# mttga/purejaxql

Measured on NVIDIA H100. Metric: MinAtar-Breakout env steps/sec @4096 envs x128 seeds, higher is better.
Workload: dtype f32

## Files before the change

### include/pqn_b200.h

```cpp
#ifndef PQN_B200_H
#define PQN_B200_H

#include <stdint.h>

#ifdef __cplusplus
extern "C" {
#endif

#define PQN_OK 0
#define PQN_E_INVALID (-1)
#define PQN_E_CUDA (-2)
#define PQN_E_UNSUPPORTED (-3)

#define PQN_ENV_BREAKOUT 0
#define PQN_ENV_ASTERIX 1
#define PQN_ENV_SPACE_INVADERS 2
#define PQN_ENV_FREEWAY 3
#define PQN_ENV_SEAQUEST 4
#define PQN_ENV_CARTPOLE 16
#define PQN_ENV_ACROBOT 17
#define PQN_ENV_MOUNTAIN_CAR 18
#define PQN_ENV_MEMORY_CHAIN 32
#define PQN_ENV_CATCH 33
#define PQN_ENV_DEEP_SEA 34
// ... 58 lines not shown
int pqn_rollout_act_step(int env_id, const uint32_t* step_keys, const float* q, const float* eps,
                         uint32_t* state, void* obs_next, int64_t obs_seed_stride, int32_t* action,
                         float* reward, uint8_t* done, float* maxq, int64_t tr_seed_stride, double* info_sums,
                         int info_done_only, int32_t S, int32_t E, int32_t env_total, int32_t env_offset, int max_steps,
                         float rew_scale, int rng_mode, void* stream);
int pqn_rollout_keys(uint32_t* rng_inout, uint32_t* keys_out, int32_t S, int32_t T, int rng_mode, void* stream);

int pqn_qlambda(const float* reward, const uint8_t* done, const float* maxq, const float* q_last,
                float* targets, int32_t T, int32_t S, int32_t E, int32_t A, float gamma, float lambda,
                void* stream);

#define PQN_NET_MINATAR_CNN 0
#define PQN_NET_MLP 1
#define PQN_NET_RNN 2
#define PQN_NET_MLP_BITS 3

typedef struct pqn_net_desc_t {
  int32_t kind;
  int32_t in_c;
  int32_t hidden;
  int32_t layers;
  int32_t num_actions;
  int32_t norm_type;
  int32_t norm_input;
} pqn_net_desc_t;
#define PQN_MAX_LAYERS 8
#define PQN_NORM_LAYER 0
#define PQN_NORM_BATCH 1
#define PQN_NORM_NONE 2

typedef struct pqn_net_layout_t {
  int64_t total;
  int64_t bn_scale, bn_bias;
  int64_t conv_w, conv_b;
  int64_t ln0_scale, ln0_bias;
  int64_t d0_w, d0_b;
  int64_t ln1_scale, ln1_bias;
  int64_t d1_w, d1_b;
  int64_t head_w, head_b;
  int64_t gru_ir_w, gru_ir_b, gru_iz_w, gru_iz_b, gru_in_w, gru_in_b, gru_hr_w, gru_hz_w, gru_hn_w, gru_hn_b;
} pqn_net_layout_t;

int pqn_net_layout(const pqn_net_desc_t* desc_host, pqn_net_layout_t* out_host);
int pqn_net_dense_layer(const pqn_net_desc_t* desc_host, int32_t layer, int64_t* offsets_host);
int64_t pqn_net_stats_floats(const pqn_net_desc_t* desc_host);
int64_t pqn_net_workspace_bytes(const pqn_net_desc_t* desc_host, int32_t S, int64_t rows);

int pqn_net_init(const pqn_net_desc_t* desc_host, const uint32_t* keys, float* params, int32_t S, void* stream);

int pqn_qnet_forward(const pqn_net_desc_t* desc_host, const float* params, const float* batch_stats, const void* obs,
                     const int32_t* gather, int64_t obs_rows_per_seed, float* q, int32_t S, int64_t rows,
                     void* workspace, void* stream);

int pqn_qnet_loss_grad(const pqn_net_desc_t* desc_host, const float* params, float* batch_stats, const void* obs,
                       const int32_t* gather, int64_t obs_rows_per_seed, const int32_t* action,
                       const float* target, int64_t tr_rows_per_seed, float* grads, float* loss_sum,
                       float* qsa_sum, float* bn_sums, int32_t S, int64_t rows, void* workspace, void* stream);

int pqn_rnn_step(const pqn_net_desc_t* desc_host, const float* params, float* hs, const float* obs,
                 int64_t obs_rows_per_seed, const uint8_t* last_done, const int32_t* last_action, float* q, int32_t S,
                 int32_t E, void* workspace, void* stream);
int pqn_rnn_loss_grad(const pqn_net_desc_t* desc_host, const float* params, const float* hs0, const float* obs,
                      const uint8_t* last_done, const int32_t* last_action, const int32_t* action, const float* reward,
                      const uint8_t* done, float* grads, float* loss_sum, float* qsa_sum, int32_t S, int32_t T, int32_t B,
                      float gamma, float lambda, void* workspace, void* stream);
int pqn_rnn_step_stats(const pqn_net_desc_t* desc_host, const float* params, const float* batch_stats, float* hs,
                       const float* obs, int64_t obs_rows_per_seed, const uint8_t* last_done, const int32_t* last_action,
                       float* q, int32_t S, int32_t E, void* workspace, void* stream);
int pqn_rnn_loss_grad_stats(const pqn_net_desc_t* desc_host, const float* params, float* batch_stats, const float* hs0,
                            const float* obs, const uint8_t* last_done, const int32_t* last_action,
                            const int32_t* action, const float* reward, const uint8_t* done, float* grads,
                            float* loss_sum, float* qsa_sum, int32_t S, int32_t T, int32_t B, float gamma, float lambda,
                            void* workspace, void* stream);

int pqn_radam_clip_step(float* params, const float* grads, float* mu, float* nu, const float* sched,
                        int32_t* step_counter, float* gnorm_scratch , int32_t S, int64_t P,
                        float max_norm, float b1, float b2, float eps, void* stream);

int pqn_bn_stats_update(float* batch_stats, float* bn_sums, int32_t S, int32_t F, int64_t stats_seed_stride,
                        float count, float momentum, void* stream);

int pqn_set_tensor_core_path(int on);
int pqn_set_conv_mma_path(int on);

int pqn_tc_split_lo(const float* x, float* lo, int64_t n, void* stream);
int pqn_tc_gemm_test(const float* a, const float* a_lo, const float* b, const float* b_lo, float* d, int32_t S,
                     int32_t M, int32_t N, int32_t K, int a_mn, int b_mn, int split3, void* stream);

int pqn_tc_split16(const float* x, void* hi, void* lo, int64_t n, float scale, void* stream);
int pqn_tc_gemm16_test(const void* a_hi, const void* a_lo, const void* b_hi, const void* b_lo, float* d, int32_t S,
                       int32_t M, int32_t N, int32_t K, int a_mn, int b_mn, float out_scale, void* stream);
int pqn_tc_dgrad16_test(const void* a_hi, const void* a_lo, const void* b_hi, const void* b_lo, const float* mask,
                        const uint32_t* relu_bits, float* d, int32_t S, int32_t M, int32_t N, int32_t K, int epi,
                        float out_scale, void* stream);

#ifdef __cplusplus
}
#endif
#endif
```

### purejaxql_b200/_lib.py

```python
from __future__ import annotations

import ctypes
import os
from ctypes import POINTER, Structure, c_char_p, c_double, c_float, c_int, c_int32, c_int64, c_longlong, c_void_p

HERE = os.path.dirname(os.path.abspath(__file__))
LIB_PATH = os.path.join(HERE, "libpqn_b200.so")


class EnvInfo(Structure):
    _fields_ = [("state_words", c_int32), ("obs_dim", c_int32), ("obs_shape", c_int32 * 3),
                ("num_actions", c_int32), ("max_steps", c_int32), ("binary_obs", c_int32),
                ("packed_obs_words", c_int32)]


class EnvParams(Structure):
    _fields_ = [("max_steps", c_int32), ("memory_length", c_int32)]


class NetDesc(Structure):
    _fields_ = [("kind", c_int32), ("in_c", c_int32), ("hidden", c_int32), ("layers", c_int32),
                ("num_actions", c_int32), ("norm_type", c_int32), ("norm_input", c_int32)]


NORM_TYPES = {"layer_norm": 0, "batch_norm": 1}


class NetLayout(Structure):
    _fields_ = [(n, c_int64) for n in (
        "total", "bn_scale", "bn_bias", "conv_w", "conv_b", "ln0_scale", "ln0_bias", "d0_w", "d0_b",
        "ln1_scale", "ln1_bias", "d1_w", "d1_b", "head_w", "head_b",
        "gru_ir_w", "gru_ir_b", "gru_iz_w", "gru_iz_b", "gru_in_w", "gru_in_b", "gru_hr_w", "gru_hz_w", "gru_hn_w",
        "gru_hn_b")]


class PqnError(RuntimeError):
    pass


_SIGS = {
    "pqn_last_error": (c_char_p, []),
    "pqn_version": (c_int, []),
    "pqn_launch_count": (c_longlong, []),
    "pqn_num_kernels": (c_int, []),
    "pqn_kernel_name": (c_char_p, [c_int]),
    "pqn_profile_enable": (c_int, [c_int]),
    "pqn_profile_read": (c_int, [POINTER(c_double), POINTER(c_longlong), c_int]),
    "pqn_env_info": (c_int, [c_int, POINTER(EnvInfo)]),
    "pqn_rng_split": (c_int, [c_void_p, c_int64, c_int32, c_void_p, c_int, c_void_p]),
    "pqn_threefry2x32": (c_int, [c_void_p, c_void_p, c_void_p, c_int64, c_void_p]),
    "pqn_rng_bits": (c_int, [c_void_p, c_int64, c_int64, c_void_p, c_int, c_void_p]),
    "pqn_random_normal": (c_int, [c_void_p, c_void_p, c_int64, c_int, c_void_p]),
    "pqn_normal_from_bits": (c_int, [c_void_p, c_void_p, c_int64, c_void_p]),
    "pqn_set_permutation_bucket_log2": (c_int, [c_int]),
    "pqn_permutation_workspace_bytes": (c_int64, [c_int64, c_int]),
    "pqn_permutation": (c_int, [c_void_p, c_int64, c_int, c_int, c_void_p, c_int64, c_void_p, c_void_p]),
    "pqn_env_reset": (c_int, [c_int, c_void_p, c_void_p, c_void_p, c_int64, c_int, c_int, c_void_p]),
    "pqn_env_reset_params": (c_int, [c_int, c_void_p, c_void_p, c_void_p, c_int64, POINTER(EnvParams), c_int, c_void_p]),
    "pqn_env_step": (c_int, [c_int, c_void_p, c_void_p, c_void_p, c_void_p, c_void_p, c_void_p, c_void_p,
                             c_void_p, c_void_p, c_void_p, c_int64, c_int, c_int, c_void_p]),
    "pqn_env_obs_packed": (c_int, [c_int, c_void_p, c_void_p, c_int64, c_void_p]),
    "pqn_env_obs": (c_int, [c_int, c_void_p, c_void_p, c_int64, c_void_p]),
    "pqn_eps_greedy": (c_int, [c_void_p, c_void_p, c_void_p, c_void_p, c_int64, c_int32, c_int, c_void_p]),
    "pqn_rollout_act_step": (c_int, [c_int, c_void_p, c_void_p, c_void_p, c_void_p, c_void_p, c_int64, c_void_p,
                                     c_void_p, c_void_p, c_void_p, c_int64, c_void_p, c_int, c_int32, c_int32,
                                     c_int32, c_int32, c_int, c_float, c_int, c_void_p]),
    "pqn_rollout_keys": (c_int, [c_void_p, c_void_p, c_int32, c_int32, c_int, c_void_p]),
    "pqn_qlambda": (c_int, [c_void_p, c_void_p, c_void_p, c_void_p, c_void_p, c_int32, c_int32, c_int32, c_int32,
                            c_float, c_float, c_void_p]),
    "pqn_net_layout": (c_int, [POINTER(NetDesc), POINTER(NetLayout)]),
    "pqn_net_dense_layer": (c_int, [POINTER(NetDesc), c_int32, POINTER(c_int64)]),
    "pqn_net_stats_floats": (c_int64, [POINTER(NetDesc)]),
    "pqn_net_workspace_bytes": (c_int64, [POINTER(NetDesc), c_int32, c_int64]),
    "pqn_net_init": (c_int, [POINTER(NetDesc), c_void_p, c_void_p, c_int32, c_void_p]),
    "pqn_qnet_forward": (c_int, [POINTER(NetDesc), c_void_p, c_void_p, c_void_p, c_void_p, c_int64, c_void_p, c_int32,
                                 c_int64, c_void_p, c_void_p]),
    "pqn_qnet_loss_grad": (c_int, [POINTER(NetDesc), c_void_p, c_void_p, c_void_p, c_void_p, c_int64, c_void_p,
                                   c_void_p, c_int64, c_void_p, c_void_p, c_void_p, c_void_p, c_int32, c_int64,
                                   c_void_p, c_void_p]),
    "pqn_rnn_step": (c_int, [POINTER(NetDesc), c_void_p, c_void_p, c_void_p, c_int64, c_void_p, c_void_p, c_void_p,
                             c_int32, c_int32, c_void_p, c_void_p]),
    "pqn_rnn_loss_grad": (c_int, [POINTER(NetDesc), c_void_p, c_void_p, c_void_p, c_void_p, c_void_p, c_void_p, c_void_p,
                                  c_void_p, c_void_p, c_void_p, c_void_p, c_int32, c_int32, c_int32, c_float, c_float,
                                  c_void_p, c_void_p]),
    "pqn_rnn_step_stats": (c_int, [POINTER(NetDesc), c_void_p, c_void_p, c_void_p, c_void_p, c_int64, c_void_p, c_void_p,
                                   c_void_p, c_int32, c_int32, c_void_p, c_void_p]),
    "pqn_rnn_loss_grad_stats": (c_int, [POINTER(NetDesc), c_void_p, c_void_p, c_void_p, c_void_p, c_void_p, c_void_p,
                                        c_void_p, c_void_p, c_void_p, c_void_p, c_void_p, c_void_p, c_int32, c_int32,
                                        c_int32, c_float, c_float, c_void_p, c_void_p]),
    "pqn_radam_clip_step": (c_int, [c_void_p, c_void_p, c_void_p, c_void_p, c_void_p, c_void_p, c_void_p, c_int32,
                                    c_int64, c_float, c_float, c_float, c_float, c_void_p]),
    "pqn_bn_stats_update": (c_int, [c_void_p, c_void_p, c_int32, c_int32, c_int64, c_float, c_float, c_void_p]),
    "pqn_set_tensor_core_path": (c_int, [c_int]),
    "pqn_set_conv_mma_path": (c_int, [c_int]),
    "pqn_tc_split_lo": (c_int, [c_void_p, c_void_p, c_int64, c_void_p]),
    "pqn_tc_split16": (c_int, [c_void_p, c_void_p, c_void_p, c_int64, c_float, c_void_p]),
    "pqn_tc_gemm_test": (c_int, [c_void_p, c_void_p, c_void_p, c_void_p, c_void_p, c_int32, c_int32, c_int32,
                                 c_int32, c_int, c_int, c_int, c_void_p]),
    "pqn_tc_gemm16_test": (c_int, [c_void_p, c_void_p, c_void_p, c_void_p, c_void_p, c_int32, c_int32, c_int32,
                                   c_int32, c_int, c_int, c_float, c_void_p]),
    "pqn_tc_dgrad16_test": (c_int, [c_void_p, c_void_p, c_void_p, c_void_p, c_void_p, c_void_p, c_void_p, c_int32,
                                    c_int32, c_int32, c_int32, c_int, c_float, c_void_p]),
}

EXPORTS = tuple(_SIGS)
_lib = None


def lib():
    global _lib
    if _lib is None:
        if not os.path.exists(LIB_PATH):
            raise PqnError(
                f"{LIB_PATH} is not built. Run `python -m purejaxql_b200.build` (needs nvcc). "
                "purejaxql_b200 has no CPU fallback.")
        l = ctypes.CDLL(LIB_PATH)
        for name, (res, args) in _SIGS.items():
            fn = getattr(l, name)
            fn.restype = res
            fn.argtypes = args
        _lib = l
    return _lib


def check(rc: int, what: str = ""):
    if rc != 0:
        msg = lib().pqn_last_error().decode("utf-8", "replace")
        raise PqnError(f"{what or 'libpqn_b200'} failed (rc={rc}): {msg}")


def p(t):
    if t is None:
        return None
    if not t.is_cuda:
        raise PqnError("libpqn_b200 takes CUDA tensors only (no CPU fallback); got a CPU tensor")
    if not t.is_contiguous():
        raise PqnError("libpqn_b200 takes contiguous tensors")
    return c_void_p(t.data_ptr())


def raw(t):
    if t is None:
        return None
    if not t.is_cuda:
        raise PqnError("libpqn_b200 takes CUDA tensors only (no CPU fallback); got a CPU tensor")
    return c_void_p(t.data_ptr())


def stream_ptr():
    import torch
    return c_void_p(torch.cuda.current_stream().cuda_stream)


def profile_read(reset=True):
    l = lib()
    n = l.pqn_num_kernels()
    ms = (c_double * n)()
    cnt = (c_longlong * n)()
    check(l.pqn_profile_read(ms, cnt, 1 if reset else 0), "pqn_profile_read")
    return {l.pqn_kernel_name(i).decode(): (ms[i], int(cnt[i])) for i in range(n) if cnt[i]}
```

### purejaxql_b200/csrc/pqn_net.cu

```cuda
#include <cuda_runtime.h>
#include <stdint.h>

#include "../../include/pqn_b200.h"
#include "api_common.h"
#include "tc_common.cuh"

namespace pqn {

constexpr int GT = 256;
constexpr int BK = 16;
constexpr float LN_EPS = 1e-6f;
constexpr int CONV_O = 16;
constexpr int CONV_PIX = 64;
constexpr int HID_CNN = 128;
constexpr int FLAT_CNN = CONV_PIX * CONV_O;

static int g_use_tc = 2;
static int g_conv_mma = 1;

__host__ __device__ static inline int64_t align4(int64_t x) { return (x + 3) & ~(int64_t)3; }

static int make_layout(const pqn_net_desc_t* d, pqn_net_layout_t* L) {
  int64_t off = 0;
  auto take = [&](int64_t n) { int64_t o = off; off += align4(n); return o; };
  L->d1_w = L->d1_b = L->ln1_scale = L->ln1_bias = L->conv_w = L->conv_b = -1;
  L->gru_ir_w = L->gru_ir_b = L->gru_iz_w = L->gru_iz_b = L->gru_in_w = L->gru_in_b = -1;
  L->gru_hr_w = L->gru_hz_w = L->gru_hn_w = L->gru_hn_b = -1;
  const int A = d->num_actions;
  const bool has_norm = d->norm_type != PQN_NORM_NONE;
  if (d->kind == PQN_NET_MINATAR_CNN) {
    const int C = d->in_c;
    L->bn_scale = take(C); L->bn_bias = take(C);
    L->conv_w = take(9 * C * CONV_O); L->conv_b = take(CONV_O);
    L->ln0_scale = L->ln0_bias = -1;
    if (has_norm) { L->ln0_scale = take(CONV_O); L->ln0_bias = take(CONV_O); }
    L->d0_w = take((int64_t)FLAT_CNN * HID_CNN); L->d0_b = take(HID_CNN);
    if (has_norm) { L->ln1_scale = take(HID_CNN); L->ln1_bias = take(HID_CNN); }
    L->head_w = take((int64_t)HID_CNN * A); L->head_b = take(A);
  } else if (d->kind == PQN_NET_MLP || d->kind == PQN_NET_RNN || d->kind == PQN_NET_MLP_BITS) {
    const int D = d->in_c, H = d->hidden;
    L->bn_scale = take(D); L->bn_bias = take(D);
    L->d0_w = take((int64_t)D * H); L->d0_b = take(H);
    L->ln0_scale = L->ln0_bias = -1;
    if (has_norm) { L->ln0_scale = take(H); L->ln0_bias = take(H); }
    for (int l = 1; l < d->layers; ++l) {
      const int64_t w = take((int64_t)H * H), b = take(H);
      const int64_t sc = has_norm ? take(H) : -1, bi = has_norm ? take(H) : -1;
      if (l == 1) { L->d1_w = w; L->d1_b = b; L->ln1_scale = sc; L->ln1_bias = bi; }
    }
    if (d->kind == PQN_NET_RNN) {
      L->gru_ir_w = take((int64_t)(H + A) * H); L->gru_ir_b = take(H);
      L->gru_iz_w = take((int64_t)(H + A) * H); L->gru_iz_b = take(H);
      L->gru_in_w = take((int64_t)(H + A) * H); L->gru_in_b = take(H);
      L->gru_hr_w = take((int64_t)H * H); L->gru_hz_w = take((int64_t)H * H);
      L->gru_hn_w = take((int64_t)H * H); L->gru_hn_b = take(H);
    }
    L->head_w = take((int64_t)H * A); L->head_b = take(A);
  } else {
    return -1;
  }
  L->total = off;
  return 0;
}

struct DenseOff { int64_t w, b, g, bi; };
__host__ __device__ inline DenseOff dense_off(const pqn_net_layout_t& L, int H, int l) {
  if (l == 0) return DenseOff{L.d0_w, L.d0_b, L.ln0_scale, L.ln0_bias};
  if (l == 1) return DenseOff{L.d1_w, L.d1_b, L.ln1_scale, L.ln1_bias};
  const bool norm = L.ln1_scale >= 0;
  const int64_t stride = align4((int64_t)H * H) + (norm ? 3 : 1) * align4(H);
  const int64_t w = (norm ? L.ln1_bias : L.d1_b) + align4(H) + (l - 2) * stride;
  const int64_t b = w + align4((int64_t)H * H);
  return DenseOff{w, b, norm ? b + align4(H) : -1, norm ? b + 2 * align4(H) : -1};
}

static int check_desc(const pqn_net_desc_t* d, const char* who) {
  if (!d) return set_error(PQN_E_INVALID, "%s: desc is NULL", who);
  if (d->num_actions < 1 || d->num_actions > 32) return set_error(PQN_E_INVALID, "%s: num_actions=%d out of [1,32]", who, d->num_actions);
  if (d->norm_type < 0 || d->norm_type > 2 || d->norm_input < 0 || d->norm_input > 1)
    return set_error(PQN_E_INVALID, "%s: norm_type=%d norm_input=%d", who, d->norm_type, d->norm_input);
  if (d->kind == PQN_NET_MLP || d->kind == PQN_NET_RNN || d->kind == PQN_NET_MLP_BITS) {
    const int H = d->hidden;
    if (H != 64 && H != 128 && H != 256 && H != 512)
      return set_error(PQN_E_UNSUPPORTED, "%s: hidden=%d (64, 128, 256 or 512 built)", who, H);
    if (d->layers < 1 || d->layers > PQN_MAX_LAYERS)
      return set_error(PQN_E_UNSUPPORTED, "%s: layers=%d (1 to %d built)", who, d->layers, PQN_MAX_LAYERS);
  }
  {
    const int Nh = d->kind == PQN_NET_MINATAR_CNN ? 128 : d->hidden;
    const size_t need = (size_t)(24 * Nh + 9 * d->num_actions * Nh + 8 * d->num_actions + 16) * sizeof(float);
    if (need > 227u * 1024u)
      return set_error(PQN_E_UNSUPPORTED, "%s: hidden=%d with num_actions=%d needs %zu B of shared memory for the head "
                       "backward (limit 227 KB)", who, Nh, d->num_actions, need);
  }
  if (d->kind == PQN_NET_MINATAR_CNN) {
    if (d->in_c != 4 && d->in_c != 6 && d->in_c != 7 && d->in_c != 10)
      return set_error(PQN_E_UNSUPPORTED, "%s: CNN in_c=%d (MinAtar uses 4/6/7/10)", who, d->in_c);
    return PQN_OK;
  }
  if (d->kind == PQN_NET_MLP_BITS) {
    if (d->in_c != 400 && d->in_c != 600 && d->in_c != 700)
// ... 494 lines not shown
      if (DZLO != nullptr) {
        float lo[V];
#pragma unroll
        for (int k = 0; k < V; ++k) lo[k] = tc::tf32_lo(dz[V * c + k]);
        st_feat<V>(DZLO + e, lo);
      }
    }
  }
#pragma unroll
  for (int j = 0; j < F; ++j) {
    const int f = (j / V) * CW + lane * V + (j % V);
    s_red3[warp * 3 * N + f] = a_dsc[j];
    s_red3[warp * 3 * N + N + f] = a_dbi[j];
    s_red3[warp * 3 * N + 2 * N + f] = a_db[j];
  }
  if (HEAD && lane == 0) { s_ls[warp * 2] = a_loss; s_ls[warp * 2 + 1] = a_qsa; }
  __syncthreads();
  const int stride = 3 * N + (HEAD ? A * N + A + 2 : 0);
  float* __restrict__ o = part + ((int64_t)seed * gridDim.x + blockIdx.x) * stride;
  for (int i = tid; i < 3 * N; i += 256) {
    float v = 0.f;
#pragma unroll
    for (int wv = 0; wv < 8; ++wv) v += s_red3[wv * 3 * N + i];
    o[i] = v;
  }
  if (HEAD) {
    for (int i = tid; i < A * N; i += 256) {
      float v = 0.f;
#pragma unroll
      for (int wv = 0; wv < 8; ++wv) v += s_dhw[wv * A * N + i];
      o[3 * N + i] = v;
    }
    if (tid < A + 2) {
      float v = 0.f;
      for (int wv = 0; wv < 8; ++wv) v += tid < A ? s_dhb[wv * A + tid] : s_ls[wv * 2 + (tid - A)];
      o[3 * N + A * N + tid] = v;
    }
  }
}

template <int SL>
__device__ __forceinline__ float ordered_partial_sum(const float* __restrict__ p, int count, int64_t stride, bool valid) {
  constexpr int COLS = 256 / SL;
  __shared__ float slice_sum[SL][COLS];
  const int col = threadIdx.x % COLS, sl = threadIdx.x / COLS;
  float v = 0.f;
  if (valid) {
#pragma unroll 4
    for (int c = sl; c < count; c += SL) v += p[(int64_t)c * stride];
  }
  slice_sum[sl][col] = v;
  __syncthreads();
  float r = 0.f;
  if (sl == 0) {
#pragma unroll
    for (int k = 0; k < SL; ++k) r += slice_sum[k][col];
  }
  return r;
}
static inline int final_slices(int count) { return count > 48 ? 32 : 8; }

template <int SL>
__global__ void row_bwd_final_kernel(const float* __restrict__ part, int nctas, int N, int A, int head,
                                     float* __restrict__ grads, int64_t P, int64_t off_dscale, int64_t off_dbias,
                                     int64_t off_db, int64_t off_hw, int64_t off_hb, float* __restrict__ loss_sum,
                                     float* __restrict__ qsa_sum) {
  const int seed = blockIdx.y;
  const int stride = 3 * N + (head ? A * N + A + 2 : 0);
  const int i = blockIdx.x * (256 / SL) + threadIdx.x % (256 / SL);
  const float v = ordered_partial_sum<SL>(part + (int64_t)seed * nctas * stride + i, nctas, stride, i < stride);
  if (i >= stride || threadIdx.x >= 256 / SL) return;
  float* __restrict__ g = grads + (int64_t)seed * P;
  if (i < N) g[off_dscale + i] = v;
  else if (i < 2 * N) g[off_dbias + (i - N)] = v;
  else if (i < 3 * N) g[off_db + (i - 2 * N)] = v;
  else if (i < 3 * N + A * N) {
    const int j = i - 3 * N, a = j / N, f = j - a * N;
    g[off_hw + (int64_t)f * A + a] = v;
  } else if (i < 3 * N + A * N + A) g[off_hb + (i - 3 * N - A * N)] = v;
  else if (i == 3 * N + A * N + A) loss_sum[seed] += v;
  else qsa_sum[seed] += v;
}

template <int C>
struct ConvCfg {
  static constexpr int TAPS = 9 * C;
  static constexpr int OBS_BITS = 100 * C;
  static constexpr int OBS_WORDS = (OBS_BITS + 31) / 32;
  static constexpr int PW = (OBS_WORDS + 3) / 4 * 4;
  static constexpr int SW = PW + 1;
};

template <int C>
__device__ __forceinline__ uint32_t pixel_bits(const uint32_t* __restrict__ so, int p) {
  const int f0 = p * C;
  const uint32_t lo = so[f0 >> 5], hi = so[(f0 >> 5) + 1];
  return __funnelshift_r(lo, hi, f0 & 31) & ((1u << C) - 1u);
}

template <int C>
__device__ __forceinline__ void conv_pixel(const uint32_t* __restrict__ so, const float* __restrict__ ws,
                                           const float* __restrict__ cb, int y, int x, float (&acc)[CONV_O]) {
#pragma unroll
  for (int o = 0; o < CONV_O; ++o) acc[o] = cb[o];
#pragma unroll
  for (int di = 0; di < 3; ++di)
#pragma unroll
    for (int dj = 0; dj < 3; ++dj) {
      const uint32_t nib = pixel_bits<C>(so, (y + di) * 10 + (x + dj));
      if (__ballot_sync(0xffffffffu, nib != 0u) == 0u) continue;
#pragma unroll
      for (int c = 0; c < C; ++c) {
        const bool bit = (nib >> c) & 1u;
        if (__ballot_sync(0xffffffffu, bit) == 0u) continue;
        const float* __restrict__ w = ws + ((di * 3 + dj) * C + c) * CONV_O;
#pragma unroll
        for (int o4 = 0; o4 < CONV_O / 4; ++o4) {
          const float4 wv = *reinterpret_cast<const float4*>(w + 4 * o4);
          if (bit) {
            acc[4 * o4] += wv.x; acc[4 * o4 + 1] += wv.y; acc[4 * o4 + 2] += wv.z; acc[4 * o4 + 3] += wv.w;
          }
        }
      }
    }
}

__device__ __forceinline__ void ln16(const float (&z)[CONV_O], float& mean, float& rstd) {
  float s1 = 0.f, s2 = 0.f;
#pragma unroll
  for (int o = 0; o < CONV_O; ++o) { s1 += z[o]; s2 = fmaf(z[o], z[o], s2); }
  mean = s1 * (1.0f / CONV_O);
  const float var = fmaxf(s2 * (1.0f / CONV_O) - mean * mean, 0.f);
  rstd = 1.0f / sqrtf(var + LN_EPS);
}

template <int C>
__device__ __forceinline__ void conv_load_consts(const float* __restrict__ prm, const pqn_net_layout_t& L, float* ws,
                                                 float* cb, float* sc, float* bi) {
  const float inv255 = 1.0f / 255.0f;
  for (int i = threadIdx.x; i < ConvCfg<C>::TAPS * CONV_O; i += blockDim.x) ws[i] = __ldg(prm + L.conv_w + i) * inv255;
  if (threadIdx.x < CONV_O) {
    cb[threadIdx.x] = __ldg(prm + L.conv_b + threadIdx.x);
    sc[threadIdx.x] = __ldg(prm + L.ln0_scale + threadIdx.x);
    bi[threadIdx.x] = __ldg(prm + L.ln0_bias + threadIdx.x);
  }
}

template <int C, bool TRAIN>
__global__ void __launch_bounds__(256) conv_fwd_kernel(const uint32_t* __restrict__ obs, int64_t obs_rows_per_seed,
                                                       const int32_t* __restrict__ gather,
                                                       const float* __restrict__ params, int64_t P,
                                                       pqn_net_layout_t L, float* __restrict__ H1,
                                                       float* __restrict__ H1LO, float* __restrict__ bn_sums,
                                                       int rows) {
  using Cfg = ConvCfg<C>;
  __shared__ __align__(16) float ws[Cfg::TAPS * CONV_O];
  __shared__ float cb[CONV_O], sc[CONV_O], bi[CONV_O];
  __shared__ uint32_t so[4][Cfg::SW];
  __shared__ float s_cnt[C];
  const int tid = threadIdx.x, sl = tid >> 6, pix = tid & 63;
  const int seed = blockIdx.y;
  const int row = blockIdx.x * 4 + sl;
  const bool valid = row < rows;
  conv_load_consts<C>(params + (int64_t)seed * P, L, ws, cb, sc, bi);
  if (TRAIN && tid < C) s_cnt[tid] = 0.f;
  if (pix < Cfg::SW) {
    uint32_t w = 0u;
    if (valid && pix < Cfg::PW) {
      const int64_t src = gather ? gather[(int64_t)seed * rows + row] : row;
      w = __ldg(obs + ((int64_t)seed * obs_rows_per_seed + src) * Cfg::PW + pix);
    }
    so[sl][pix] = w;
  }
  __syncthreads();
// ... 120 lines not shown
      for (int o4 = 0; o4 < CONV_O / 4; ++o4) {
        float4 dz;
        dz.x = rstd * (dy[4 * o4] - m1 - acc[4 * o4] * m2);
        dz.y = rstd * (dy[4 * o4 + 1] - m1 - acc[4 * o4 + 1] * m2);
        dz.z = rstd * (dy[4 * o4 + 2] - m1 - acc[4 * o4 + 2] * m2);
        dz.w = rstd * (dy[4 * o4 + 3] - m1 - acc[4 * o4 + 3] * m2);
        *reinterpret_cast<float4*>(&my_dz[pix * SDZ_LD + 4 * o4]) = dz;
      }
    }
    __syncwarp();
#pragma unroll 8
    for (int p = tpar; p < CONV_PIX; p += 2) a_dcb += my_dz[p * SDZ_LD + o_b];
#pragma unroll
    for (int c = 0; c < C; ++c) {
      for (int wi = 0; wi < Cfg::OBS_WORDS; ++wi) {
        uint32_t bits = my_so[wi];
        if (C == 4) bits &= 0x11111111u << c;
        if (bits == 0u) continue;
        while (bits) {
          const int b = __ffs(bits) - 1;
          bits &= bits - 1u;
          const int f = wi * 32 + b;
          const int q = f / C;
          if (f - q * C != c) continue;
          const int qy = q / 10, qx = q - qy * 10;
#pragma unroll
          for (int it = 0; it < 5; ++it) {
            const int py = qy - t_di[it], px = qx - t_dj[it];
            if ((unsigned)py < 8u && (unsigned)px < 8u) wacc[c][it] += my_dz[(py * 8 + px) * SDZ_LD + o_b];
          }
        }
      }
    }
  }
  __syncthreads();
  for (int i = tid; i < TAPS * CONV_O; i += blockDim.x) s_w[i] = 0.f;
  __syncthreads();
  const float inv255 = 1.0f / 255.0f;
#pragma unroll
  for (int c = 0; c < C; ++c)
#pragma unroll
    for (int it = 0; it < 5; ++it) {
      const int tap = it * 2 + tpar;
      if (tap < 9) atomicAdd(&s_w[(tap * C + c) * CONV_O + o_b], wacc[c][it] * inv255);
    }
  atomicAdd(&s_red[2 * CONV_O + o_b], a_dcb);
#pragma unroll
  for (int o = 0; o < CONV_O; ++o) {
    float v0 = a_dsc[o], v1 = a_dbi[o];
#pragma unroll
    for (int sft = 16; sft > 0; sft >>= 1) {
      v0 += __shfl_xor_sync(0xffffffffu, v0, sft);
      v1 += __shfl_xor_sync(0xffffffffu, v1, sft);
    }
    if (lane == 0) {
      atomicAdd(&s_red[o], v0);
      atomicAdd(&s_red[CONV_O + o], v1);
    }
  }
  __syncthreads();
  float* __restrict__ g = grads + (int64_t)seed * P;
  for (int i = tid; i < TAPS * CONV_O; i += blockDim.x) atomicAdd(g + L.conv_w + i, s_w[i]);
  if (tid < CONV_O) {
    atomicAdd(g + L.ln0_scale + tid, s_red[tid]);
    atomicAdd(g + L.ln0_bias + tid, s_red[CONV_O + tid]);
    atomicAdd(g + L.conv_b + tid, s_red[2 * CONV_O + tid]);
  }
}

__device__ __forceinline__ void mma_tf32_16n8k8(float (&d)[4], const uint32_t (&a)[4], uint32_t b0, uint32_t b1) {
  asm volatile(
      "mma.sync.aligned.m16n8k8.row.col.f32.tf32.tf32.f32 {%0,%1,%2,%3}, {%4,%5,%6,%7}, {%8,%9}, {%0,%1,%2,%3};"
      : "+f"(d[0]), "+f"(d[1]), "+f"(d[2]), "+f"(d[3])
      : "r"(a[0]), "r"(a[1]), "r"(a[2]), "r"(a[3]), "r"(b0), "r"(b1));
}

template <int C>
struct ConvMma {
  static constexpr int TAPS = 9 * C;
  static constexpr int KS = (TAPS + 7) / 8;
  static constexpr int MT = (TAPS + 15) / 16;
};

template <int C>
struct PatchCfg {
  static constexpr int WORDS = (9 * C + 31) / 32;
};

template <int C>
__device__ __forceinline__ void patch_bits(const uint32_t* __restrict__ so, int pix, uint32_t (&w)[PatchCfg<C>::WORDS]) {
  constexpr int W = PatchCfg<C>::WORDS;
#pragma unroll
  for (int k = 0; k < W; ++k) w[k] = 0u;
  const int y = pix >> 3, x = pix & 7;
#pragma unroll
  for (int di = 0; di < 3; ++di) {
    const int f0 = ((y + di) * 10 + x) * C;
    const uint32_t r = __funnelshift_r(so[f0 >> 5], so[(f0 >> 5) + 1], f0 & 31) & ((1u << (3 * C)) - 1u);
    const int o = 3 * C * di;
    w[o >> 5] |= r << (o & 31);
    if ((o & 31) + 3 * C > 32) w[min((o >> 5) + 1, W - 1)] |= r >> (32 - (o & 31));
  }
}

template <int C>
__device__ __forceinline__ void build_patch(const uint32_t* __restrict__ so, int pix, uint32_t* __restrict__ out) {
  constexpr int W = PatchCfg<C>::WORDS;
  uint32_t w[W];
  patch_bits<C>(so, pix, w);
#pragma unroll
  for (int k = 0; k < W; ++k) out[k] = w[k];
}

template <int C>
__device__ __forceinline__ void build_patches(const uint32_t* __restrict__ so, uint32_t* __restrict__ patch, int lane) {
  build_patch<C>(so, lane, patch + lane * PatchCfg<C>::WORDS);
  build_patch<C>(so, lane + 32, patch + (lane + 32) * PatchCfg<C>::WORDS);
}

__device__ __forceinline__ uint32_t bit_f32(uint32_t word, int shift) {
  return ((word >> shift) & 1u) ? 0x3F800000u : 0u;
}

template <int C, bool EXPC = false>
__device__ __forceinline__ void conv_mma_load_weights(const float* __restrict__ prm, const pqn_net_layout_t& L,
                                                      float2* wb_hi, float2* wb_lo, float* cb, float* sc, float* bi) {
  using M = ConvMma<C>;
  const float inv255 = 1.0f / 255.0f;
  for (int i = threadIdx.x; i < M::KS * 2 * 32; i += blockDim.x) {
    const int ln = i & 31, h = (i >> 5) & 1, ks = i >> 6;
    const int o = h * 8 + (ln >> 2);
    const int t0 = ks * 8 + (ln & 3), t1 = t0 + 4;
    float w0 = t0 < M::TAPS ? __ldg(prm + L.conv_w + t0 * CONV_O + o) * inv255 : 0.f;
    float w1 = t1 < M::TAPS ? __ldg(prm + L.conv_w + t1 * CONV_O + o) * inv255 : 0.f;
    if (EXPC) {
      w0 *= __uint_as_float((254u - (1u << (t0 & 7))) << 23);
      w1 *= __uint_as_float((254u - (1u << (t1 & 7))) << 23);
    }
    const float h0 = __uint_as_float(__float_as_uint(w0) & 0xFFFFE000u), h1 = __uint_as_float(__float_as_uint(w1) & 0xFFFFE000u);
    wb_hi[i] = make_float2(h0, h1);
    wb_lo[i] = make_float2(w0 - h0, w1 - h1);
  }
  if (threadIdx.x < CONV_O) {
    cb[threadIdx.x] = __ldg(prm + L.conv_b + threadIdx.x);
    sc[threadIdx.x] = __ldg(prm + L.ln0_scale + threadIdx.x);
    bi[threadIdx.x] = __ldg(prm + L.ln0_bias + threadIdx.x);
  }
}

template <int C>
struct ExpPatch {
  static constexpr int KS = ConvMma<C>::KS;
  static constexpr int LD = KS | 1;
};

template <int C>
__device__ __forceinline__ void build_exp_patch(const uint32_t* __restrict__ so, int pix, uint32_t* __restrict__ out) {
  constexpr int W = PatchCfg<C>::WORDS;
  uint32_t w[W];
  patch_bits<C>(so, pix, w);
#pragma unroll
  for (int ks = 0; ks < ExpPatch<C>::KS; ++ks)
    out[ks] = ((w[(8 * ks) >> 5] >> ((8 * ks) & 31)) & 0xFFu) << 23;
}

template <int C>
__device__ __forceinline__ void conv_mma_block2_exp(const uint32_t* __restrict__ xp, const float2* __restrict__ wb_hi,
                                                    const float2* __restrict__ wb_lo, const float* __restrict__ cb,
                                                    int mbp, int lane, float (&z)[2][2][4]) {
  using E = ExpPatch<C>;
  const int g = lane >> 2, t = lane & 3;
  const uint32_t m_lo = 1u << (23 + t), m_hi = 1u << (27 + t);
#pragma unroll
  for (int i = 0; i < 2; ++i)
#pragma unroll
    for (int h = 0; h < 2; ++h) {
      z[i][h][0] = z[i][h][2] = cb[8 * h + 2 * t];
      z[i][h][1] = z[i][h][3] = cb[8 * h + 2 * t + 1];
    }
  const uint32_t* r00 = xp + (32 * mbp + g) * E::LD;
#pragma unroll
  for (int ks = 0; ks < E::KS; ++ks) {
    uint32_t a[2][4];
#pragma unroll
    for (int i = 0; i < 2; ++i) {
      const uint32_t w0 = r00[(16 * i) * E::LD + ks], w1 = r00[(16 * i + 8) * E::LD + ks];
      a[i][0] = w0 & m_lo; a[i][1] = w1 & m_lo; a[i][2] = w0 & m_hi; a[i][3] = w1 & m_hi;
    }
    float2 bl[2], bh[2];
#pragma unroll
    for (int h = 0; h < 2; ++h) {
      bl[h] = wb_lo[(ks * 2 + h) * 32 + lane];
      bh[h] = wb_hi[(ks * 2 + h) * 32 + lane];
    }
#pragma unroll
    for (int h = 0; h < 2; ++h)
#pragma unroll
      for (int i = 0; i < 2; ++i) mma_tf32_16n8k8(z[i][h], a[i], __float_as_uint(bl[h].x), __float_as_uint(bl[h].y));
#pragma unroll
    for (int h = 0; h < 2; ++h)
#pragma unroll
      for (int i = 0; i < 2; ++i) mma_tf32_16n8k8(z[i][h], a[i], __float_as_uint(bh[h].x), __float_as_uint(bh[h].y));
  }
}

__device__ __forceinline__ void ln16_quad(const float (&z)[2][4], float& mean0, float& rstd0, float& mean1,
                                          float& rstd1) {
  float s0 = z[0][0] + z[0][1] + z[1][0] + z[1][1];
  float q0 = fmaf(z[1][1], z[1][1], fmaf(z[1][0], z[1][0], fmaf(z[0][0], z[0][0], __fmul_rn(z[0][1], z[0][1]))));
  float s1 = z[0][2] + z[0][3] + z[1][2] + z[1][3];
  float q1 = fmaf(z[1][3], z[1][3], fmaf(z[1][2], z[1][2], fmaf(z[0][2], z[0][2], __fmul_rn(z[0][3], z[0][3]))));
#pragma unroll
  for (int o = 1; o <= 2; o <<= 1) {
    s0 += __shfl_xor_sync(0xffffffffu, s0, o); q0 += __shfl_xor_sync(0xffffffffu, q0, o);
    s1 += __shfl_xor_sync(0xffffffffu, s1, o); q1 += __shfl_xor_sync(0xffffffffu, q1, o);
  }
  mean0 = __fmul_rn(s0, 1.0f / CONV_O); mean1 = __fmul_rn(s1, 1.0f / CONV_O);
  rstd0 = rsqrtf(fmaxf(fmaf(q0, 1.0f / CONV_O, -__fmul_rn(mean0, mean0)), 0.f) + LN_EPS);
  rstd1 = rsqrtf(fmaxf(fmaf(q1, 1.0f / CONV_O, -__fmul_rn(mean1, mean1)), 0.f) + LN_EPS);
}

constexpr int CONV_MMA_WARPS = 8;

template <int C, bool TRAIN, bool H16 = false>
__global__ void __launch_bounds__(CONV_MMA_WARPS * 32, 3)
    conv_fwd_mma_kernel(const uint32_t* __restrict__ obs, int64_t obs_rows_per_seed, const int32_t* __restrict__ gather,
                        const float* __restrict__ params, int64_t P, pqn_net_layout_t L, float* __restrict__ H1,
                        float* __restrict__ H1LO, float* __restrict__ XH1, float* __restrict__ RS1,
                        uint32_t* __restrict__ RB, float* __restrict__ bn_sums, int rows) {
  using Cfg = ConvCfg<C>;
  using M = ConvMma<C>;
  __shared__ float2 wb_hi[M::KS * 2 * 32], wb_lo[M::KS * 2 * 32];
  __shared__ float cb[CONV_O], sc[CONV_O], bi[CONV_O];
  __shared__ uint32_t so[CONV_MMA_WARPS][Cfg::SW];
  __shared__ uint32_t sxp[CONV_MMA_WARPS][CONV_PIX * ExpPatch<C>::LD];
  __shared__ float s_cnt[C];
  const int tid = threadIdx.x, warp = tid >> 5, lane = tid & 31;
  const int g = lane >> 2, t = lane & 3;
  const int seed = blockIdx.y;
  conv_mma_load_weights<C, true>(params + (int64_t)seed * P, L, wb_hi, wb_lo, cb, sc, bi);
  if (TRAIN && tid < C) s_cnt[tid] = 0.f;
  __syncthreads();
  int cnt[C];
  uint32_t cmask[C];
#pragma unroll
  for (int c = 0; c < C; ++c) {
    cnt[c] = 0;
    cmask[c] = 0u;
    if (TRAIN) {
      for (int b = 0; b < 32; ++b) {
        const int f = lane * 32 + b;
        if (f < Cfg::OBS_BITS && f % C == c) cmask[c] |= 1u << b;
      }
    }
  }
  uint32_t* __restrict__ my_so = so[warp];
  static_assert(Cfg::PW <= 32, "one packed observation word per lane");
  if (lane == 0) my_so[Cfg::PW] = 0u;
  const int row_stride = gridDim.x * CONV_MMA_WARPS;
  auto fetch = [&](int r) -> uint32_t {
    if (r >= rows || lane >= Cfg::PW) return 0u;
    const int64_t src = gather ? gather[(int64_t)seed * rows + r] : r;
    return __ldg(obs + ((int64_t)seed * obs_rows_per_seed + src) * Cfg::PW + lane);
  };
  uint32_t pre = fetch(blockIdx.x * CONV_MMA_WARPS + warp);
  for (int row = blockIdx.x * CONV_MMA_WARPS + warp; row < rows; row += row_stride) {
    __syncwarp();
    if (lane < Cfg::PW) my_so[lane] = pre;
    if (TRAIN && bn_sums != nullptr) {
#pragma unroll
      for (int c = 0; c < C; ++c) cnt[c] += __popc(pre & cmask[c]);
    }
    __syncwarp();
    pre = fetch(row + row_stride);
    build_exp_patch<C>(my_so, lane, sxp[warp] + lane * ExpPatch<C>::LD);
    build_exp_patch<C>(my_so, lane + 32, sxp[warp] + (lane + 32) * ExpPatch<C>::LD);
    __syncwarp();
    float* __restrict__ hrow = H16 ? nullptr : H1 + ((int64_t)seed * rows + row) * FLAT_CNN;
    float* __restrict__ lrow = (!H16 && H1LO) ? H1LO + ((int64_t)seed * rows + row) * FLAT_CNN : nullptr;
    __half* __restrict__ hrow16 = H16 ? reinterpret_cast<__half*>(H1) + ((int64_t)seed * rows + row) * FLAT_CNN : nullptr;
    __half* __restrict__ lrow16 = H16 ? reinterpret_cast<__half*>(H1LO) + ((int64_t)seed * rows + row) * FLAT_CNN : nullptr;
    float* __restrict__ xrow = (TRAIN && XH1) ? XH1 + ((int64_t)seed * rows + row) * FLAT_CNN : nullptr;
    float* __restrict__ rrow = (TRAIN && RS1) ? RS1 + ((int64_t)seed * rows + row) * CONV_PIX : nullptr;
    uint16_t* __restrict__ brow =
        (TRAIN && RB) ? reinterpret_cast<uint16_t*>(RB + ((int64_t)seed * rows + row) * (FLAT_CNN / 32)) : nullptr;
#pragma unroll 1
    for (int mbp = 0; mbp < 2; ++mbp) {
     float z2[2][2][4];
     conv_mma_block2_exp<C>(sxp[warp], wb_hi, wb_lo, cb, mbp, lane, z2);
#pragma unroll
     for (int mi = 0; mi < 2; ++mi) {
      const int mb = 2 * mbp + mi;
      float (&z)[2][4] = z2[mi];
      float mean0, rstd0, mean1, rstd1;
      ln16_quad(z, mean0, rstd0, mean1, rstd1);
      uint32_t rb0 = 0u, rb1 = 0u;
#pragma unroll
      for (int h = 0; h < 2; ++h) {
        const int o = 8 * h + 2 * t;
        float2 v0, v1;
        v0.x = fmaxf((z[h][0] - mean0) * rstd0 * sc[o] + bi[o], 0.f);
        v0.y = fmaxf((z[h][1] - mean0) * rstd0 * sc[o + 1] + bi[o + 1], 0.f);
        v1.x = fmaxf((z[h][2] - mean1) * rstd1 * sc[o] + bi[o], 0.f);
        v1.y = fmaxf((z[h][3] - mean1) * rstd1 * sc[o + 1] + bi[o + 1], 0.f);
        const int p0 = 16 * mb + g, p1 = p0 + 8;
        if (H16) {
          __half2 h0, l0, h1v, l1;
          tc::split16x2<false>(fminf(v0.x, 65000.f), fminf(v0.y, 65000.f), h0, l0);
          tc::split16x2<false>(fminf(v1.x, 65000.f), fminf(v1.y, 65000.f), h1v, l1);
          *reinterpret_cast<__half2*>(hrow16 + p0 * CONV_O + o) = h0;
          *reinterpret_cast<__half2*>(lrow16 + p0 * CONV_O + o) = l0;
          *reinterpret_cast<__half2*>(hrow16 + p1 * CONV_O + o) = h1v;
          *reinterpret_cast<__half2*>(lrow16 + p1 * CONV_O + o) = l1;
        } else {
          *reinterpret_cast<float2*>(hrow + p0 * CONV_O + o) = v0;
          *reinterpret_cast<float2*>(hrow + p1 * CONV_O + o) = v1;
        }
        if (TRAIN) {
          rb0 |= ((v0.x > 0.f ? 1u : 0u) | (v0.y > 0.f ? 2u : 0u)) << o;
          rb1 |= ((v1.x > 0.f ? 1u : 0u) | (v1.y > 0.f ? 2u : 0u)) << o;
        }
        if (xrow) {
          *reinterpret_cast<float2*>(xrow + p0 * CONV_O + o) =
              make_float2((z[h][0] - mean0) * rstd0, (z[h][1] - mean0) * rstd0);
          *reinterpret_cast<float2*>(xrow + p1 * CONV_O + o) =
              make_float2((z[h][2] - mean1) * rstd1, (z[h][3] - mean1) * rstd1);
          if (h == 0 && t == 0) { rrow[p0] = rstd0; rrow[p1] = rstd1; }
        }
        if (lrow) {
          *reinterpret_cast<float2*>(lrow + p0 * CONV_O + o) = make_float2(tc::tf32_lo(v0.x), tc::tf32_lo(v0.y));
          *reinterpret_cast<float2*>(lrow + p1 * CONV_O + o) = make_float2(tc::tf32_lo(v1.x), tc::tf32_lo(v1.y));
        }
      }
      if (TRAIN && brow) {
        rb0 |= __shfl_xor_sync(0xffffffffu, rb0, 1); rb1 |= __shfl_xor_sync(0xffffffffu, rb1, 1);
        rb0 |= __shfl_xor_sync(0xffffffffu, rb0, 2); rb1 |= __shfl_xor_sync(0xffffffffu, rb1, 2);
        if (t == 0) { brow[16 * mb + g] = (uint16_t)rb0; brow[16 * mb + g + 8] = (uint16_t)rb1; }
      }
     }
    }
  }
  if (TRAIN && bn_sums != nullptr) {
#pragma unroll
    for (int c = 0; c < C; ++c) {
      int v = cnt[c];
#pragma unroll
      for (int o = 16; o > 0; o >>= 1) v += __shfl_xor_sync(0xffffffffu, v, o);
      if (lane == 0 && v) atomicAdd(&s_cnt[c], (float)v);
    }
    __syncthreads();
    if (tid < C && s_cnt[tid] != 0.f) {
      atomicAdd(bn_sums + (int64_t)seed * 2 * C + tid, s_cnt[tid]);
      atomicAdd(bn_sums + (int64_t)seed * 2 * C + C + tid, s_cnt[tid]);
    }
  }
}

__device__ __forceinline__ void mma_f16_16n8k16(float (&d)[4], const uint32_t (&a)[4], uint32_t b0, uint32_t b1) {
  asm volatile(
      "mma.sync.aligned.m16n8k16.row.col.f32.f16.f16.f32 {%0,%1,%2,%3}, {%4,%5,%6,%7}, {%8,%9}, {%0,%1,%2,%3};"
      : "+f"(d[0]), "+f"(d[1]), "+f"(d[2]), "+f"(d[3])
      : "r"(a[0]), "r"(a[1]), "r"(a[2]), "r"(a[3]), "r"(b0), "r"(b1));
}

template <int C>
struct Conv16 {
  static constexpr int TAPS = 9 * C;
  static constexpr int KS = (TAPS + 15) / 16;
  static constexpr int ROW = 2 * KS < 8 ? 8 : 2 * KS;
};

__host__ __device__ constexpr int conv16_channel(int h, int n) { return 4 * (n >> 1) + 2 * h + (n & 1); }

__host__ __device__ constexpr int conv16_tap(int s, int kk) {
  return 16 * s + (kk < 8 ? 0 : 8) + ((kk & 1) ? 4 : 0) + ((kk & 7) >> 1);
}

template <int C>
__device__ __forceinline__ void conv16_load_weights(const float* __restrict__ prm, const pqn_net_layout_t& L, uint4* wb,
                                                    float* cb, float* sc, float* bi) {
  using M = Conv16<C>;
  const float inv255 = 1.0f / 255.0f;
  for (int i = threadIdx.x; i < M::KS * 2 * 32; i += blockDim.x) {
    const int ln = i & 31, h = (i >> 5) & 1, s = i >> 6;
    const int gg = ln >> 2, tt = ln & 3;
    const int o = conv16_channel(h, gg);
    const float scale = __uint_as_float((uint32_t)(127 + 15 - (1 << tt)) << 23);
    float v[4];
#pragma unroll
    for (int q = 0; q < 4; ++q) {
      const int tap = conv16_tap(s, 2 * tt + (q & 1) + (q >> 1) * 8);
      v[q] = tap < M::TAPS ? __ldg(prm + L.conv_w + tap * CONV_O + o) * inv255 * scale : 0.f;
      v[q] = fminf(fmaxf(v[q], -65000.f), 65000.f);
    }
    const __half2 h0 = __floats2half2_rn(v[0], v[1]), h1 = __floats2half2_rn(v[2], v[3]);
    const float2 f0 = __half22float2(h0), f1 = __half22float2(h1);
    const __half2 l0 = __floats2half2_rn(v[0] - f0.x, v[1] - f0.y), l1 = __floats2half2_rn(v[2] - f1.x, v[3] - f1.y);
    wb[i] = make_uint4(*reinterpret_cast<const uint32_t*>(&h0), *reinterpret_cast<const uint32_t*>(&h1),
                       *reinterpret_cast<const uint32_t*>(&l0), *reinterpret_cast<const uint32_t*>(&l1));
  }
  if (threadIdx.x < CONV_O) {
    cb[threadIdx.x] = __ldg(prm + L.conv_b + threadIdx.x);
    sc[threadIdx.x] = __ldg(prm + L.ln0_scale + threadIdx.x);
    bi[threadIdx.x] = __ldg(prm + L.ln0_bias + threadIdx.x);
  }
}

template <int C>
__device__ __forceinline__ void build_patch16(const uint32_t* __restrict__ so, int pix, uint32_t* __restrict__ out) {
  constexpr int W = PatchCfg<C>::WORDS;
  uint32_t w[W];
  patch_bits<C>(so, pix, w);
#pragma unroll
  for (int b = 0; b < 2 * Conv16<C>::KS; ++b) {
    const int o = 8 * b;
    uint32_t v = (o >> 5) < W ? w[(o >> 5) < W ? (o >> 5) : 0] : 0u;
    const int sh = o & 31;
    const uint32_t lo = sh >= 10 ? v >> (sh - 10) : v << (10 - sh);
    const uint32_t hi = sh + 4 <= 26 ? v << (26 - sh - 4) : v >> (sh + 4 - 26);
    out[b] = __byte_perm(lo, hi, 0x7610);
  }
}

template <int C>
__device__ __forceinline__ void store_patch16(const uint32_t* __restrict__ so, int pix, uint32_t* __restrict__ row) {
  using M = Conv16<C>;
  uint32_t w[M::ROW];
#pragma unroll
  for (int k = 0; k < M::ROW; ++k) w[k] = 0u;
  build_patch16<C>(so, pix, w);
#pragma unroll
  for (int q = 0; q < M::ROW / 4; ++q)
    *reinterpret_cast<uint4*>(row + 4 * q) = make_uint4(w[4 * q], w[4 * q + 1], w[4 * q + 2], w[4 * q + 3]);
}

template <int C, int NB>
__device__ __forceinline__ void conv16_blocks(const uint32_t* __restrict__ xp, const uint4* __restrict__ wb,
                                              const float* __restrict__ cb, int mb0, int lane, float (&z)[NB][2][4]) {
  using M = Conv16<C>;
  const int g = lane >> 2, t = lane & 3;
  const uint32_t mask = (1u << (10 + t)) | (1u << (26 + t));
#pragma unroll
  for (int i = 0; i < NB; ++i)
#pragma unroll
    for (int h = 0; h < 2; ++h) {
      z[i][h][0] = z[i][h][2] = cb[4 * t + 2 * h];
      z[i][h][1] = z[i][h][3] = cb[4 * t + 2 * h + 1];
    }
  const uint32_t* r00 = xp + (16 * mb0 + g) * M::ROW;
#pragma unroll
  for (int s = 0; s < M::KS; ++s) {
    uint32_t a[NB][4];
#pragma unroll
    for (int i = 0; i < NB; ++i) {
      const uint2 w0 = *reinterpret_cast<const uint2*>(r00 + (16 * i) * M::ROW + 2 * s);
      const uint2 w1 = *reinterpret_cast<const uint2*>(r00 + (16 * i + 8) * M::ROW + 2 * s);
      a[i][0] = w0.x & mask; a[i][1] = w1.x & mask; a[i][2] = w0.y & mask; a[i][3] = w1.y & mask;
    }
    uint4 b[2];
#pragma unroll
    for (int h = 0; h < 2; ++h) b[h] = wb[(s * 2 + h) * 32 + lane];
#pragma unroll
    for (int h = 0; h < 2; ++h)
#pragma unroll
      for (int i = 0; i < NB; ++i) mma_f16_16n8k16(z[i][h], a[i], b[h].z, b[h].w);
#pragma unroll
    for (int h = 0; h < 2; ++h)
#pragma unroll
      for (int i = 0; i < NB; ++i) mma_f16_16n8k16(z[i][h], a[i], b[h].x, b[h].y);
  }
}

__device__ __forceinline__ void conv16_xhat(const float (&z)[2][4], float (&x0)[4], float (&x1)[4], float& rstd0,
                                            float& rstd1) {
  float mean0, mean1;
  ln16_quad(z, mean0, rstd0, mean1, rstd1);
  const float nm0 = -__fmul_rn(mean0, rstd0), nm1 = -__fmul_rn(mean1, rstd1);
#pragma unroll
  for (int h = 0; h < 2; ++h)
#pragma unroll
    for (int c = 0; c < 2; ++c) {
      x0[2 * h + c] = fmaf(z[h][c], rstd0, nm0);
      x1[2 * h + c] = fmaf(z[h][2 + c], rstd1, nm1);
    }
}

__device__ __forceinline__ uint32_t cvt_f16x2_satfinite(float lo, float hi) {
  uint32_t r;
  asm("cvt.rn.satfinite.f16x2.f32 %0, %1, %2;" : "=r"(r) : "f"(hi), "f"(lo));
  return r;
}

constexpr int CONV16_WARPS = 4;
constexpr int CONV16_CTAS_PER_SM = 5;

template <int C, bool TRAIN, bool H16>
__global__ void __launch_bounds__(CONV16_WARPS * 32, CONV16_CTAS_PER_SM)
    conv_fwd_mma16_kernel(const uint32_t* __restrict__ obs, int64_t obs_rows_per_seed, const int32_t* __restrict__ gather,
                          const float* __restrict__ params, int64_t P, pqn_net_layout_t L, float* __restrict__ H1,
                          float* __restrict__ H1LO, uint32_t* __restrict__ RB, float* __restrict__ bn_sums, int rows) {
  using Cfg = ConvCfg<C>;
  using M = Conv16<C>;
  __shared__ __align__(16) uint4 wb[M::KS * 2 * 32];
  __shared__ float cb[CONV_O], sc[CONV_O], bi[CONV_O];
  __shared__ uint32_t so[CONV16_WARPS][Cfg::SW];
  __shared__ __align__(16) uint32_t sxp[CONV16_WARPS][CONV_PIX * M::ROW];
  __shared__ float s_cnt[C];
  const int tid = threadIdx.x, warp = tid >> 5, lane = tid & 31;
  const int g = lane >> 2, t = lane & 3;
  const int seed = blockIdx.y;
  conv16_load_weights<C>(params + (int64_t)seed * P, L, wb, cb, sc, bi);
  if (TRAIN && tid < C) s_cnt[tid] = 0.f;
  __syncthreads();
  int cnt[C];
  uint32_t cmask[C];
#pragma unroll
  for (int c = 0; c < C; ++c) {
    cnt[c] = 0;
    cmask[c] = 0u;
    if (TRAIN) {
      for (int b = 0; b < 32; ++b) {
        const int f = lane * 32 + b;
        if (f < Cfg::OBS_BITS && f % C == c) cmask[c] |= 1u << b;
      }
    }
  }
  uint32_t* __restrict__ my_so = so[warp];
  static_assert(Cfg::PW <= 32, "one packed observation word per lane");
  if (lane == 0) my_so[Cfg::PW] = 0u;
  const int row_stride = gridDim.x * CONV16_WARPS;
  auto fetch_index = [&](int r) -> int {
    const int rc = r < rows ? r : rows - 1;
    return gather ? __ldg(gather + (int64_t)seed * rows + rc) : rc;
  };
  auto fetch_obs = [&](int src) -> uint32_t {
    return __ldg(obs + ((int64_t)seed * obs_rows_per_seed + src) * Cfg::PW + (lane < Cfg::PW ? lane : 0));
  };
  const int row0 = blockIdx.x * CONV16_WARPS + warp;
  uint32_t pre = fetch_obs(fetch_index(row0));
  int src_next = fetch_index(row0 + row_stride);
  for (int row = row0; row < rows; row += row_stride) {
    __syncwarp();
    if (lane < Cfg::PW) my_so[lane] = pre;
    if (TRAIN && bn_sums != nullptr) {
#pragma unroll
      for (int c = 0; c < C; ++c) cnt[c] += __popc(pre & cmask[c]);
    }
    __syncwarp();
    pre = fetch_obs(src_next);
    src_next = fetch_index(row + 2 * row_stride);
    store_patch16<C>(my_so, lane, sxp[warp] + lane * M::ROW);
    store_patch16<C>(my_so, lane + 32, sxp[warp] + (lane + 32) * M::ROW);
    __syncwarp();
    const int64_t grow = (int64_t)seed * rows + row;
    float* __restrict__ hrow = H16 ? nullptr : H1 + grow * FLAT_CNN;
    __half* __restrict__ hrow16 = H16 ? reinterpret_cast<__half*>(H1) + grow * FLAT_CNN : nullptr;
    __half* __restrict__ lrow16 = H16 ? reinterpret_cast<__half*>(H1LO) + grow * FLAT_CNN : nullptr;
    uint16_t* __restrict__ brow = (TRAIN && RB) ? reinterpret_cast<uint16_t*>(RB + grow * (FLAT_CNN / 32)) : nullptr;
    uint32_t keep_rb = 0u;
#pragma unroll 1
    for (int mbp = 0; mbp < 2; ++mbp) {
      float z2[2][2][4];
      conv16_blocks<C, 2>(sxp[warp], wb, cb, 2 * mbp, lane, z2);
#pragma unroll
      for (int mi = 0; mi < 2; ++mi) {
        const int mb = 2 * mbp + mi;
        float x0[4], x1[4], rstd0, rstd1;
        conv16_xhat(z2[mi], x0, x1, rstd0, rstd1);
        uint32_t rb0 = 0u, rb1 = 0u;
        const int p0 = 16 * mb + g, p1 = p0 + 8, o4 = 4 * t;
        float v0[4], v1[4];
#pragma unroll
        for (int c = 0; c < 4; ++c) {
          v0[c] = fmaxf(fmaf(x0[c], sc[o4 + c], bi[o4 + c]), 0.f);
          v1[c] = fmaxf(fmaf(x1[c], sc[o4 + c], bi[o4 + c]), 0.f);
        }
        if (H16) {
          uint32_t hw0[2], hw1[2], lw0[2], lw1[2];
#pragma unroll
          for (int h = 0; h < 2; ++h) {
            hw0[h] = cvt_f16x2_satfinite(v0[2 * h], v0[2 * h + 1]);
            hw1[h] = cvt_f16x2_satfinite(v1[2 * h], v1[2 * h + 1]);
            const float2 f0 = __half22float2(*reinterpret_cast<const __half2*>(&hw0[h]));
            const float2 f1 = __half22float2(*reinterpret_cast<const __half2*>(&hw1[h]));
            const __half2 l0 = __floats2half2_rn((v0[2 * h] - f0.x) * tc::TC_LO_SCALE, (v0[2 * h + 1] - f0.y) * tc::TC_LO_SCALE);
            const __half2 l1 = __floats2half2_rn((v1[2 * h] - f1.x) * tc::TC_LO_SCALE, (v1[2 * h + 1] - f1.y) * tc::TC_LO_SCALE);
            lw0[h] = *reinterpret_cast<const uint32_t*>(&l0); lw1[h] = *reinterpret_cast<const uint32_t*>(&l1);
          }
          *reinterpret_cast<uint2*>(hrow16 + p0 * CONV_O + o4) = make_uint2(hw0[0], hw0[1]);
          *reinterpret_cast<uint2*>(lrow16 + p0 * CONV_O + o4) = make_uint2(lw0[0], lw0[1]);
          *reinterpret_cast<uint2*>(hrow16 + p1 * CONV_O + o4) = make_uint2(hw1[0], hw1[1]);
          *reinterpret_cast<uint2*>(lrow16 + p1 * CONV_O + o4) = make_uint2(lw1[0], lw1[1]);
        } else {
          *reinterpret_cast<float4*>(hrow + p0 * CONV_O + o4) = make_float4(v0[0], v0[1], v0[2], v0[3]);
          *reinterpret_cast<float4*>(hrow + p1 * CONV_O + o4) = make_float4(v1[0], v1[1], v1[2], v1[3]);
        }
        if (TRAIN) {
#pragma unroll
          for (int c = 0; c < 4; ++c) {
            rb0 |= (v0[c] > 0.f ? 1u : 0u) << (o4 + c);
            rb1 |= (v1[c] > 0.f ? 1u : 0u) << (o4 + c);
          }
        }
        if (TRAIN && brow) {
          uint32_t rb = rb0 | (rb1 << 16);
          rb |= __shfl_xor_sync(0xffffffffu, rb, 1);
          rb |= __shfl_xor_sync(0xffffffffu, rb, 2);
          if (t == mb) keep_rb = rb;
        }
      }
    }
    if (TRAIN && brow) { brow[16 * t + g] = (uint16_t)keep_rb; brow[16 * t + g + 8] = (uint16_t)(keep_rb >> 16); }
  }
  if (TRAIN && bn_sums != nullptr) {
#pragma unroll
    for (int c = 0; c < C; ++c) {
      int v = cnt[c];
#pragma unroll
      for (int o = 16; o > 0; o >>= 1) v += __shfl_xor_sync(0xffffffffu, v, o);
      if (lane == 0 && v) atomicAdd(&s_cnt[c], (float)v);
    }
    __syncthreads();
    if (tid < C && s_cnt[tid] != 0.f) {
      atomicAdd(bn_sums + (int64_t)seed * 2 * C + tid, s_cnt[tid]);
      atomicAdd(bn_sums + (int64_t)seed * 2 * C + C + tid, s_cnt[tid]);
    }
  }
}

constexpr int CDZ_LD = 16;
__device__ __forceinline__ int cswz(int p, int col) { return col ^ (((p >> 1) & 1) << 3); }

__device__ __forceinline__ void cp_async16(void* smem_dst, const void* gsrc) {
  asm volatile("cp.async.cg.shared.global [%0], [%1], 16;" ::"r"((uint32_t)__cvta_generic_to_shared(smem_dst)), "l"(gsrc)
               : "memory");
}
__device__ __forceinline__ void cp_async_commit() { asm volatile("cp.async.commit_group;" ::: "memory"); }
__device__ __forceinline__ void cp_async_wait_all() { asm volatile("cp.async.wait_group 0;" ::: "memory"); }

template <int C>
struct ConvBwdSmem {
  static constexpr int DY = 0;
  static constexpr int XH = DY + FLAT_CNN;
  static constexpr int RS = XH + FLAT_CNN;
  static constexpr int DZ = RS + CONV_PIX;
  static constexpr int PATCH = DZ + CONV_PIX * CDZ_LD;
  static constexpr int WARP_FLOATS = (PATCH + CONV_PIX * PatchCfg<C>::WORDS + 3) / 4 * 4;
  static constexpr int WARPS = 8;
  static constexpr int BYTES = (WARPS * WARP_FLOATS + 4 * CONV_O) * 4;
};

template <int C>
__global__ void __launch_bounds__(ConvBwdSmem<C>::WARPS * 32, 2)
    conv_bwd_mma_kernel(const uint32_t* __restrict__ obs, int64_t obs_rows_per_seed, const int32_t* __restrict__ gather,
                        const float* __restrict__ params, int64_t P, pqn_net_layout_t L, const float* __restrict__ DY1,
                        const float* __restrict__ XH1, const float* __restrict__ RS1, float* __restrict__ part,
                        int rows) {
  using Cfg = ConvCfg<C>;
  using M = ConvMma<C>;
  using SM = ConvBwdSmem<C>;
  constexpr int PWD = PatchCfg<C>::WORDS;
  extern __shared__ __align__(16) float smem_bwd[];
  const int tid = threadIdx.x, warp = tid >> 5, lane = tid & 31;
  const int g = lane >> 2, t = lane & 3;
  const int seed = blockIdx.y;
  float* my = smem_bwd + warp * SM::WARP_FLOATS;
  float* my_dy = my + SM::DY;
  float* my_xh = my + SM::XH;
  float* my_rs = my + SM::RS;
  float* my_dz = my + SM::DZ;
  uint32_t* my_so = reinterpret_cast<uint32_t*>(my + SM::DZ);
// ... 164 lines not shown
  for (int col = 0; col < 4; ++col) {
    float v0 = a_dsc[col], v1 = a_dbi[col], v2 = a_dcb[col];
#pragma unroll
    for (int sft = 4; sft <= 16; sft <<= 1) {
      v0 += __shfl_xor_sync(0xffffffffu, v0, sft);
      v1 += __shfl_xor_sync(0xffffffffu, v1, sft);
      v2 += __shfl_xor_sync(0xffffffffu, v2, sft);
    }
    a_dsc[col] = v0; a_dbi[col] = v1; a_dcb[col] = v2;
  }
  for (int w = 0; w < SM::WARPS; ++w) {
    if (warp == w && g == 0) {
#pragma unroll
      for (int col = 0; col < 4; ++col) {
        const int o = 8 * (col >> 1) + 2 * t + (col & 1);
        s_red[o] = (w == 0 ? 0.f : s_red[o]) + a_dsc[col];
        s_red[CONV_O + o] = (w == 0 ? 0.f : s_red[CONV_O + o]) + a_dbi[col];
        s_red[2 * CONV_O + o] = (w == 0 ? 0.f : s_red[2 * CONV_O + o]) + a_dcb[col];
      }
    }
    __syncthreads();
  }
  float* __restrict__ o = part + ((int64_t)seed * gridDim.x + blockIdx.x) * (M::TAPS * CONV_O + 3 * CONV_O);
  for (int i = tid; i < M::TAPS * CONV_O; i += blockDim.x) o[i] = s_w[i] * (1.0f / 255.0f);
  if (tid < 3 * CONV_O) o[M::TAPS * CONV_O + tid] = s_red[tid];
}

template <int C>
struct ConvBwd16 {
  static constexpr int MT = ConvMma<C>::MT;
  static constexpr int NG = 4 * MT;
  static constexpr int NGP = (NG % 8 == 4) ? NG : NG + 4;
  static constexpr int DY = 0;
  static constexpr int XH = DY + FLAT_CNN;
  static constexpr int RS = XH + 16 * CONV_O;
  static constexpr int DZT = RS + 16;
  static constexpr int PW = DZT + 2 * CONV_O * 32;
  static constexpr int XP = PW + 32 * NGP;
  static constexpr int WARP_FLOATS = (XP + CONV_PIX * Conv16<C>::ROW + 3) / 4 * 4;
  static constexpr int WARPS = (C == 4) ? 8 : 6;
  static constexpr int WB = WARPS * WARP_FLOATS;
  static constexpr int BYTES = (WB + Conv16<C>::KS * 2 * 32 * 4 + 6 * CONV_O) * 4;
};

__device__ __forceinline__ int cswz16(int p, int col) {
  return ((p ^ ((p >> 2) & 1)) << 4) + (col ^ (((p >> 1) & 1) << 3));
}
__device__ __forceinline__ int dzt_word(int ch, int ks, int pos) {
  const int c7 = ch & 7;
  return (ch << 5) + ((ks ^ ((c7 + (c7 >> 2)) & 3)) << 3) + pos;
}

template <int C>
__global__ void __launch_bounds__(ConvBwd16<C>::WARPS * 32, 2)
    conv_bwd_mma16_kernel(const uint32_t* __restrict__ obs, int64_t obs_rows_per_seed, const int32_t* __restrict__ gather,
                          const float* __restrict__ params, int64_t P, pqn_net_layout_t L, const float* __restrict__ DY1,
                          float* __restrict__ part, int rows, float gs) {
  using Cfg = ConvCfg<C>;
  using M = ConvMma<C>;
  using SM = ConvBwd16<C>;
  constexpr int PWD = PatchCfg<C>::WORDS;
  extern __shared__ __align__(16) float smem_bwd[];
  const int tid = threadIdx.x, warp = tid >> 5, lane = tid & 31;
  const int g = lane >> 2, t = lane & 3;
  const int seed = blockIdx.y;
  float* my = smem_bwd + warp * SM::WARP_FLOATS;
  float* my_dy = my + SM::DY;
  float* my_xh = my + SM::XH;
  float* my_rs = my + SM::RS;
  uint32_t* my_dzt = reinterpret_cast<uint32_t*>(my + SM::DZT);
  uint32_t* my_so = reinterpret_cast<uint32_t*>(my + SM::DZT);
  uint32_t* my_pw = reinterpret_cast<uint32_t*>(my + SM::PW);
  uint32_t* my_xp = reinterpret_cast<uint32_t*>(my + SM::XP);
  uint4* wb = reinterpret_cast<uint4*>(smem_bwd + SM::WB);
  float* cb = smem_bwd + SM::WB + Conv16<C>::KS * 2 * 32 * 4;
  float* sc = cb + CONV_O;
  float* bi = sc + CONV_O;
  float* s_red = bi + CONV_O;
  float* s_w = smem_bwd;
  static_assert(Cfg::SW <= 2 * CONV_O * 32, "obs staging aliases the dz planes");
  static_assert(M::MT * 16 * CONV_O <= SM::WARP_FLOATS * SM::WARPS, "dW reduction buffer aliases the warp slices");
  static_assert(Cfg::PW <= 32, "one packed observation word per lane");
  static_assert(SM::XP % 4 == 0 && SM::WB % 4 == 0, "16-byte aligned patch rows and weight fragments");
  conv16_load_weights<C>(params + (int64_t)seed * P, L, wb, cb, sc, bi);
  if (tid < 3 * CONV_O) s_red[tid] = 0.f;
  __syncthreads();
  float a_dsc[4] = {0.f, 0.f, 0.f, 0.f}, a_dbi[4] = {0.f, 0.f, 0.f, 0.f}, a_dcb[4] = {0.f, 0.f, 0.f, 0.f};
  float wrun[M::MT][2][4];
#pragma unroll
  for (int mt = 0; mt < M::MT; ++mt)
#pragma unroll
    for (int h = 0; h < 2; ++h)
#pragma unroll
      for (int j = 0; j < 4; ++j) wrun[mt][h][j] = 0.f;
  const uint32_t amask = (1u << (10 + (g & 3))) | (1u << (26 + (g & 3)));
  const int pos_g = g < 4 ? 2 * g : 2 * (g - 4) + 1;

  const int row_stride = gridDim.x * SM::WARPS;
  auto fetch_index = [&](int r) -> int {
    const int rc = r < rows ? r : rows - 1;
    return gather ? __ldg(gather + (int64_t)seed * rows + rc) : rc;
  };
  auto fetch_obs = [&](int src) -> uint32_t {
    return __ldg(obs + ((int64_t)seed * obs_rows_per_seed + src) * Cfg::PW + (lane < Cfg::PW ? lane : 0));
  };
  auto fetch_dy = [&](int r) {
    if (r < rows) {
      const float* dsrc = DY1 + ((int64_t)seed * rows + r) * FLAT_CNN;
#pragma unroll
      for (int i = 0; i < FLAT_CNN / 4 / 32; ++i) {
        const int q = i * 32 + lane, prow = q >> 2;
        cp_async16(my_dy + cswz16(prow, (q & 3) * 4), dsrc + q * 4);
      }
    }
    cp_async_commit();
  };
  int row = blockIdx.x * SM::WARPS + warp;
  uint32_t pre = fetch_obs(fetch_index(row));
  int src_next = fetch_index(row + row_stride);
  fetch_dy(row);
  for (; row < rows; row += row_stride) {
    __syncwarp();
    if (lane < Cfg::PW) my_so[lane] = pre;
    if (lane == 0) my_so[Cfg::PW] = 0u;
    __syncwarp();
    pre = fetch_obs(src_next);
    src_next = fetch_index(row + 2 * row_stride);
    store_patch16<C>(my_so, lane, my_xp + lane * Conv16<C>::ROW);
    store_patch16<C>(my_so, lane + 32, my_xp + (lane + 32) * Conv16<C>::ROW);
    {
      uint32_t w0[PWD], w1[PWD];
      patch_bits<C>(my_so, 2 * lane, w0);
      patch_bits<C>(my_so, 2 * lane + 1, w1);
      uint32_t pw[SM::NGP];
#pragma unroll
      for (int k = 0; k < SM::NGP; ++k) pw[k] = 0u;
#pragma unroll
      for (int q = 0; q < SM::NG; ++q) {
        const int ql = q & 3, slot = (q & ~3) + (ql == 1 ? 2 : (ql == 2 ? 1 : ql));
        const int bit = 4 * q, wi = bit >> 5, sh = bit & 31;
        if (wi < PWD) {
          const uint32_t v0 = w0[wi < PWD ? wi : 0], v1 = w1[wi < PWD ? wi : 0];
          const uint32_t lo = sh >= 10 ? v0 >> (sh >= 10 ? sh - 10 : 0) : v0 << (sh < 10 ? 10 - sh : 0);
          const uint32_t hi = sh <= 26 ? v1 << (sh <= 26 ? 26 - sh : 0) : v1 >> (sh > 26 ? sh - 26 : 0);
          pw[slot] = __byte_perm(lo, hi, 0x7610);
        }
      }
      uint32_t* dstw = my_pw + lane * SM::NGP;
#pragma unroll
      for (int k = 0; k < SM::NGP / 4; ++k)
        *reinterpret_cast<uint4*>(dstw + 4 * k) = make_uint4(pw[4 * k], pw[4 * k + 1], pw[4 * k + 2], pw[4 * k + 3]);
    }
    cp_async_wait_all();
    __syncwarp();
#pragma unroll 1
    for (int mb = 0; mb < 4; ++mb) {
      {
        float zc[1][2][4], x0[4], x1[4], rs0, rs1;
        conv16_blocks<C, 1>(my_xp, wb, cb, mb, lane, zc);
        conv16_xhat(zc[0], x0, x1, rs0, rs1);
        __syncwarp();
        *reinterpret_cast<float4*>(my_xh + cswz16(g, 4 * t)) = make_float4(x0[0], x0[1], x0[2], x0[3]);
        *reinterpret_cast<float4*>(my_xh + cswz16(g + 8, 4 * t)) = make_float4(x1[0], x1[1], x1[2], x1[3]);
        if (t == 0) { my_rs[g] = rs0; my_rs[g + 8] = rs1; }
        __syncwarp();
      }
      const int p0 = 16 * mb + 2 * g, p1 = p0 + 1;
// ... 521 lines not shown
  if (per_seed < 1) per_seed = 1;
  return (unsigned)per_seed;
}

static int wgrad_splits(int tiles, int S, int rows) {
  int s = (2 * device_sm_count() + tiles * S - 1) / (tiles * S);
  const int maxs = (rows + 255) / 256;
  if (s > maxs) s = maxs;
  if (s < 1) s = 1;
  return s;
}

__global__ void split_lo_strided_kernel(const float* __restrict__ src, int64_t src_seed_stride, float* __restrict__ lo,
                                        int64_t n_per_seed) {
  const int seed = blockIdx.y;
  const int64_t i4 = (int64_t)blockIdx.x * blockDim.x + threadIdx.x;
  if (i4 * 4 >= n_per_seed) return;
  const float4 v = __ldg(reinterpret_cast<const float4*>(src + (int64_t)seed * src_seed_stride) + i4);
  reinterpret_cast<float4*>(lo + (int64_t)seed * n_per_seed)[i4] =
      make_float4(tc::tf32_lo(v.x), tc::tf32_lo(v.y), tc::tf32_lo(v.z), tc::tf32_lo(v.w));
}

static void launch_split_w1(const float* params, int64_t P, int64_t off_w, float* w1_lo, int S, cudaStream_t st) {
  const int64_t n = (int64_t)FLAT_CNN * HID_CNN;
  LaunchScope _ls(K_TC_SPLIT, st);
  split_lo_strided_kernel<<<dim3(cdiv(n / 4, 256), S), 256, 0, st>>>(params + off_w, P, w1_lo, n);
}

struct Planes16 { __half *h1_hi, *h1_lo, *dz_hi, *dz_lo, *w1_hi, *w1_lo; };
static Planes16 planes16(const Workspace& w, int S, int64_t rows) {
  const int64_t R = (int64_t)S * rows;
  Planes16 p;
  p.h1_hi = reinterpret_cast<__half*>(w.h1_lo); p.h1_lo = p.h1_hi + R * FLAT_CNN;
  p.dz_hi = reinterpret_cast<__half*>(w.dz2_lo); p.dz_lo = p.dz_hi + R * HID_CNN;
  p.w1_hi = reinterpret_cast<__half*>(w.w1_lo); p.w1_lo = p.w1_hi + (int64_t)S * FLAT_CNN * HID_CNN;
  return p;
}
static float grad_scale(int64_t rows) {
  float s = 16.f;
  while (rows > 1) { s *= 2.f; rows = (rows + 1) >> 1; }
  return s;
}

__global__ void split16_strided_kernel(const float* __restrict__ src, int64_t src_seed_stride, __half* __restrict__ hi,
                                       __half* __restrict__ lo, int64_t n_per_seed) {
  const int seed = blockIdx.y;
  const int64_t i4 = (int64_t)blockIdx.x * blockDim.x + threadIdx.x;
  if (i4 * 4 >= n_per_seed) return;
  const float4 v = __ldg(reinterpret_cast<const float4*>(src + (int64_t)seed * src_seed_stride) + i4);
  __half2 h0, h1, l0, l1;
  tc::split16x2(v.x, v.y, h0, l0);
  tc::split16x2(v.z, v.w, h1, l1);
  reinterpret_cast<uint2*>(hi + (int64_t)seed * n_per_seed)[i4] =
      make_uint2(*reinterpret_cast<uint32_t*>(&h0), *reinterpret_cast<uint32_t*>(&h1));
  reinterpret_cast<uint2*>(lo + (int64_t)seed * n_per_seed)[i4] =
      make_uint2(*reinterpret_cast<uint32_t*>(&l0), *reinterpret_cast<uint32_t*>(&l1));
}

static void launch_split16_w1(const float* params, int64_t P, int64_t off_w, const Planes16& pl, int S, cudaStream_t st) {
  const int64_t n = (int64_t)FLAT_CNN * HID_CNN;
  LaunchScope _ls(K_TC_SPLIT, st);
  split16_strided_kernel<<<dim3(cdiv(n / 4, 256), S), 256, 0, st>>>(params + off_w, P, pl.w1_hi, pl.w1_lo, n);
}
static void launch_split16_h1(const float* h1, const Planes16& pl, int64_t n, cudaStream_t st) {
  LaunchScope _ls(K_TC_SPLIT, st);
  split16_strided_kernel<<<dim3(cdiv(n / 4, 256), 1), 256, 0, st>>>(h1, 0, pl.h1_hi, pl.h1_lo, n);
}

static int tc16_dense_fwd(int epi, const float* params, int64_t P, const pqn_net_layout_t& L, const Workspace& w,
                          const Planes16& pl, int A, float* q, int S, int rows, cudaStream_t st) {
  CUtensorMap t[4];
  int rc;
  if ((rc = tc::make_tmap16(&t[0], pl.h1_hi, FLAT_CNN, rows, S, FLAT_CNN, (uint64_t)rows * FLAT_CNN, 128))) return rc;
  if ((rc = tc::make_tmap16(&t[1], pl.h1_lo, FLAT_CNN, rows, S, FLAT_CNN, (uint64_t)rows * FLAT_CNN, 128))) return rc;
  if ((rc = tc::make_tmap16(&t[2], pl.w1_hi, HID_CNN, FLAT_CNN, S, HID_CNN, (uint64_t)FLAT_CNN * HID_CNN, 64))) return rc;
  if ((rc = tc::make_tmap16(&t[3], pl.w1_lo, HID_CNN, FLAT_CNN, S, HID_CNN, (uint64_t)FLAT_CNN * HID_CNN, 64))) return rc;
  tc::GemmShape gs = {};
  gs.S = S; gs.M = rows; gs.m_tiles = (rows + 127) / 128; gs.n_tiles = 1; gs.k_blocks = FLAT_CNN / tc::TC_BK16;
  tc::EpiParams ep = {};
  ep.params = params; ep.P = P; ep.off_b = L.d0_b; ep.off_scale = L.ln1_scale; ep.off_bias = L.ln1_bias;
  ep.off_hw = L.head_w; ep.off_hb = L.head_b; ep.A = A; ep.rows = rows;
  ep.H = w.h2; ep.XHAT = w.xhat2; ep.RSTD = w.rstd2; ep.Q = q;
  return tc::launch_gemm16(0, 1, epi, t, gs, ep, st, epi == tc::EPI_LN_HEAD ? K_TC_FWD_HEAD : K_TC_FWD);
}

static int tc16_wgrad(float* grads, int64_t P, const pqn_net_layout_t& L, const Planes16& pl, int S, int rows,
                      float gscale, float* wg_part, cudaStream_t st) {
  CUtensorMap t[4];
  int rc;
  if ((rc = tc::make_tmap16(&t[0], pl.h1_hi, FLAT_CNN, rows, S, FLAT_CNN, (uint64_t)rows * FLAT_CNN, 64))) return rc;
  if ((rc = tc::make_tmap16(&t[1], pl.h1_lo, FLAT_CNN, rows, S, FLAT_CNN, (uint64_t)rows * FLAT_CNN, 64))) return rc;
  if ((rc = tc::make_tmap16(&t[2], pl.dz_hi, HID_CNN, rows, S, HID_CNN, (uint64_t)rows * HID_CNN, 64))) return rc;
  if ((rc = tc::make_tmap16(&t[3], pl.dz_lo, HID_CNN, rows, S, HID_CNN, (uint64_t)rows * HID_CNN, 64))) return rc;
  tc::GemmShape gs = {};
  gs.S = S; gs.M = FLAT_CNN; gs.m_tiles = FLAT_CNN / 128; gs.n_tiles = 1;
  gs.k_blocks = (rows + tc::TC_BK16 - 1) / tc::TC_BK16;
  gs.k_split = wgrad_ksplit(S * gs.m_tiles * gs.n_tiles, gs.k_blocks);
  tc::EpiParams ep = {};
  ep.ld_out = HID_CNN; ep.out_scale = 1.0f / gscale;
  const int64_t n = (int64_t)FLAT_CNN * HID_CNN;
  if (gs.k_split > 1) { ep.out = wg_part; ep.out_seed_stride = n; ep.split_stride = (int64_t)S * n; }
  else { ep.out = grads + L.d0_w; ep.out_seed_stride = P; }
  if ((rc = tc::launch_gemm16(1, 1, tc::EPI_STORE, t, gs, ep, st, K_TC_WGRAD))) return rc;
  if (gs.k_split > 1) {
    launch_split_reduce(wg_part, gs.k_split, (int64_t)S * n, n, S, grads + L.d0_w, P, st);
  }
  return 0;
}

static int tc16_dgrad(const Workspace& w, const Planes16& pl, int S, int rows, bool have_bits, float gscale,
                      cudaStream_t st) {
  CUtensorMap t[4];
  int rc;
  if ((rc = tc::make_tmap16(&t[0], pl.dz_hi, HID_CNN, rows, S, HID_CNN, (uint64_t)rows * HID_CNN, 128))) return rc;
  if ((rc = tc::make_tmap16(&t[1], pl.dz_lo, HID_CNN, rows, S, HID_CNN, (uint64_t)rows * HID_CNN, 128))) return rc;
  if ((rc = tc::make_tmap16(&t[2], pl.w1_hi, HID_CNN, FLAT_CNN, S, HID_CNN, (uint64_t)FLAT_CNN * HID_CNN, 128))) return rc;
  if ((rc = tc::make_tmap16(&t[3], pl.w1_lo, HID_CNN, FLAT_CNN, S, HID_CNN, (uint64_t)FLAT_CNN * HID_CNN, 128))) return rc;
  tc::GemmShape gs = {};
  gs.S = S; gs.M = rows; gs.m_tiles = (rows + 127) / 128; gs.n_tiles = FLAT_CNN / 128; gs.k_blocks = HID_CNN / tc::TC_BK16;
 
  tc::EpiParams ep = {};
  ep.out = w.h1; ep.mask = w.h1; ep.ld_out = FLAT_CNN; ep.out_seed_stride = (int64_t)rows * FLAT_CNN;
  ep.relu_bits = w.relu_bits; ep.rows = rows; ep.out_scale = 1.0f / gscale;
  return tc::launch_gemm16(0, 0, have_bits ? tc::EPI_RELU_BITS : tc::EPI_RELU_MASK, t, gs, ep, st, K_TC_DGRAD);
}

static int tc16_mm_store(const __half* a, int64_t a_plane, const __half* b, int64_t b_plane, float* out, int S, int rows, int K,
                         int N, cudaStream_t st, int kid) {
  CUtensorMap t[4];
  int rc;
  if ((rc = tc::make_tmap16(&t[0], a, K, rows, S, K, (uint64_t)rows * K, 128))) return rc;
  if ((rc = tc::make_tmap16(&t[1], a + a_plane, K, rows, S, K, (uint64_t)rows * K, 128))) return rc;
  if ((rc = tc::make_tmap16(&t[2], b, N, K, S, N, (uint64_t)K * N, 64))) return rc;
  if ((rc = tc::make_tmap16(&t[3], b + b_plane, N, K, S, N, (uint64_t)K * N, 64))) return rc;
  tc::GemmShape gs = {};
  gs.S = S; gs.M = rows; gs.m_tiles = (rows + 127) / 128; gs.n_tiles = N / 128; gs.k_blocks = (K + tc::TC_BK16 - 1) / tc::TC_BK16;
 
  tc::EpiParams ep = {};
  ep.out = out; ep.ld_out = N; ep.out_seed_stride = (int64_t)rows * N;
  return tc::launch_gemm16(0, 1, tc::EPI_STORE, t, gs, ep, st, kid);
}
static int tc16_mm_wgrad(const __half* a, int64_t a_plane, const __half* dz, int64_t dz_plane, float* out, int64_t out_seed_stride,
                         int S, int rows, int M, int N, float out_scale, float* wg_part, cudaStream_t st) {
  CUtensorMap t[4];
  int rc;
  if ((rc = tc::make_tmap16(&t[0], a, M, rows, S, M, (uint64_t)rows * M, 64))) return rc;
  if ((rc = tc::make_tmap16(&t[1], a + a_plane, M, rows, S, M, (uint64_t)rows * M, 64))) return rc;
  if ((rc = tc::make_tmap16(&t[2], dz, N, rows, S, N, (uint64_t)rows * N, 64))) return rc;
  if ((rc = tc::make_tmap16(&t[3], dz + dz_plane, N, rows, S, N, (uint64_t)rows * N, 64))) return rc;
  tc::GemmShape gs = {};
  gs.S = S; gs.M = M; gs.m_tiles = M / 128; gs.n_tiles = N / 128; gs.k_blocks = (rows + tc::TC_BK16 - 1) / tc::TC_BK16;
  gs.k_split = wgrad_ksplit(S * gs.m_tiles * gs.n_tiles, gs.k_blocks);
  tc::EpiParams ep = {};
  ep.ld_out = N; ep.out_scale = out_scale;
  const int64_t n = (int64_t)M * N;
  if (gs.k_split > 1) { ep.out = wg_part; ep.out_seed_stride = n; ep.split_stride = (int64_t)S * n; }
  else { ep.out = out; ep.out_seed_stride = out_seed_stride; }
  if ((rc = tc::launch_gemm16(1, 1, tc::EPI_STORE, t, gs, ep, st, K_TC_WGRAD))) return rc;
  if (gs.k_split > 1) {
    launch_split_reduce(wg_part, gs.k_split, (int64_t)S * n, n, S, out, out_seed_stride, st);
  }
  return 0;
}
static int tc16_mm_dgrad(const __half* dz, int64_t dz_plane, const __half* wgt, int64_t w_plane, const float* mask, float* out,
                         int S, int rows, int N, int Kp, float out_scale, cudaStream_t st) {
  CUtensorMap t[4];
// ... 223 lines not shown
  if (rnn::modular_rnn(d)) {
    if ((rc = rnn::rnn_trunk_bwd_modular(d, L, params, obs, grads, S, rows, w, st))) return rc;
    return check_launch(who);
  }
  const dim3 rbg(conv_mma_ctas(S, rows, 4), S);
  float* dcur = w.dx;
  for (int l = d->layers - 1; l >= 0; --l) {
    const DenseOff o = dense_off(L, H, l);
    if ((rc = run_row_bwd(H, false, rbg, A, st, nullptr, w.xh[l], w.rs[l], dcur, dcur, nullptr, nullptr, nullptr, 1.0f, params,
                          grads, P, o.g, o.bi, o.b, 0, 0, nullptr, nullptr, nullptr, 0, nullptr, nullptr, w.rbp,
                          rows))) return rc;
    const float* xprev = l == 0 ? obs : w.h[l - 1];
    const int kin = l == 0 ? D : H;
    const int spl = wgrad_splits(ffma_tiles(kin, H), S, rows);
    run_wgrad_ffma(xprev, (int64_t)rows * kin, kin, dcur, (int64_t)rows * H, H, grads, P, o.w, rows, kin, S, spl, w.wgp, st);
    if (l > 0) {
      float* dnext = dcur == w.dhl ? w.dx : w.dhl;
      launch_dgrad(dcur, (int64_t)rows * H, H, params, P, o.w, w.h[l - 1], dnext, (int64_t)rows * H, rows, H, 0, S, st);
      dcur = dnext;
    }
  }
  return check_launch(who);
}

}

using namespace pqn;

extern "C" {

int64_t pqn_net_stats_floats(const pqn_net_desc_t* d) {
  if (check_desc(d, "pqn_net_stats_floats")) return -1;
  return nrm::stats_floats(d);
}

int pqn_rnn_step(const pqn_net_desc_t* d, const float* params, float* hs, const float* obs, int64_t obs_rows_per_seed,
                 const uint8_t* last_done, const int32_t* last_action, float* q, int32_t S, int32_t E, void* workspace,
                 void* stream) {
  int rc = check_desc(d, "pqn_rnn_step");
  if (rc) return rc;
  if ((rc = rnn::check_rnn(d, "pqn_rnn_step"))) return rc;
  return rnn_step(d, params, nullptr, hs, obs, obs_rows_per_seed, last_done, last_action, q, S, E, workspace, stream,
                  "pqn_rnn_step");
}

int pqn_rnn_step_stats(const pqn_net_desc_t* d, const float* params, const float* batch_stats, float* hs, const float* obs,
                       int64_t obs_rows_per_seed, const uint8_t* last_done, const int32_t* last_action, float* q, int32_t S,
                       int32_t E, void* workspace, void* stream) {
  int rc = check_desc(d, "pqn_rnn_step_stats");
  if (rc) return rc;
  if ((rc = rnn::check_rnn_stats(d, batch_stats, "pqn_rnn_step_stats"))) return rc;
  return rnn_step(d, params, batch_stats, hs, obs, obs_rows_per_seed, last_done, last_action, q, S, E, workspace, stream,
                  "pqn_rnn_step_stats");
}

int pqn_rnn_loss_grad(const pqn_net_desc_t* d, const float* params, const float* hs0, const float* obs,
                      const uint8_t* last_done, const int32_t* last_action, const int32_t* action, const float* reward,
                      const uint8_t* done, float* grads, float* loss_sum, float* qsa_sum, int32_t S, int32_t T, int32_t B,
                      float gamma, float lambda, void* workspace, void* stream) {
  int rc = check_desc(d, "pqn_rnn_loss_grad");
  if (rc) return rc;
  if ((rc = rnn::check_rnn(d, "pqn_rnn_loss_grad"))) return rc;
  return rnn_loss_grad(d, params, nullptr, hs0, obs, last_done, last_action, action, reward, done, grads, loss_sum, qsa_sum,
                       S, T, B, gamma, lambda, workspace, stream, "pqn_rnn_loss_grad");
}

int pqn_rnn_loss_grad_stats(const pqn_net_desc_t* d, const float* params, float* batch_stats, const float* hs0,
                            const float* obs, const uint8_t* last_done, const int32_t* last_action, const int32_t* action,
                            const float* reward, const uint8_t* done, float* grads, float* loss_sum, float* qsa_sum,
                            int32_t S, int32_t T, int32_t B, float gamma, float lambda, void* workspace, void* stream) {
  int rc = check_desc(d, "pqn_rnn_loss_grad_stats");
  if (rc) return rc;
  if ((rc = rnn::check_rnn_stats(d, batch_stats, "pqn_rnn_loss_grad_stats"))) return rc;
  return rnn_loss_grad(d, params, batch_stats, hs0, obs, last_done, last_action, action, reward, done, grads, loss_sum,
                       qsa_sum, S, T, B, gamma, lambda, workspace, stream, "pqn_rnn_loss_grad_stats");
}

int pqn_set_conv_mma_path(int on) {
  if (on != 0 && on != 1 && on != 3) return set_error(PQN_E_UNSUPPORTED, "pqn_set_conv_mma_path: no conv path %d", on);
  g_conv_mma = on;
  return PQN_OK;
}

int pqn_set_tensor_core_path(int on) {
  if (on < 0 || on > 2) return set_error(PQN_E_UNSUPPORTED, "pqn_set_tensor_core_path: no tensor-core path %d", on);
  g_use_tc = on;
  return PQN_OK;
}

int pqn_net_layout(const pqn_net_desc_t* d, pqn_net_layout_t* out) {
  int rc = check_desc(d, "pqn_net_layout");
  if (rc) return rc;
  if (!out) return set_error(PQN_E_INVALID, "pqn_net_layout: out is NULL");
  make_layout(d, out);
  return PQN_OK;
}

int pqn_net_dense_layer(const pqn_net_desc_t* d, int32_t layer, int64_t* offsets_host) {
  int rc = check_desc(d, "pqn_net_dense_layer");
  if (rc) return rc;
  if (d->kind != PQN_NET_MLP && d->kind != PQN_NET_RNN && d->kind != PQN_NET_MLP_BITS)
    return set_error(PQN_E_INVALID, "pqn_net_dense_layer: only the MLP and GRU networks have hidden dense layers");
  if (!offsets_host || layer < 0 || layer >= d->layers)
    return set_error(PQN_E_INVALID, "pqn_net_dense_layer: layer=%d out of [0,%d) or offsets NULL", layer, d->layers);
  pqn_net_layout_t L;
  make_layout(d, &L);
  const DenseOff o = dense_off(L, d->hidden, layer);
  offsets_host[0] = o.w; offsets_host[1] = o.b; offsets_host[2] = o.g; offsets_host[3] = o.bi;
  return PQN_OK;
}

int64_t pqn_net_workspace_bytes(const pqn_net_desc_t* d, int32_t S, int64_t rows) {
  if (check_desc(d, "pqn_net_workspace_bytes")) return -1;
  if (d->kind == PQN_NET_RNN) return rnn::carve_rnn(d, S, rows, nullptr, nullptr);
  if (modular_net(d)) return nrm::carve_norm(d, S, rows, nullptr, nullptr);
  return carve(d, S, rows, nullptr, nullptr) +
         (d->kind == PQN_NET_MLP_BITS ? bits::carve_bits(d, S, rows, nullptr, nullptr) : 0);
}

int pqn_qnet_forward(const pqn_net_desc_t* d, const float* params, const float* batch_stats, const void* obs,
                     const int32_t* gather, int64_t obs_rows_per_seed, float* q, int32_t S, int64_t rows, void* workspace,
                     void* stream) {
  int rc = check_desc(d, "pqn_qnet_forward");
  if (rc) return rc;
  if (!params || !obs || !q || !workspace || S <= 0 || rows <= 0 || S > 65535)
    return set_error(PQN_E_INVALID, "pqn_qnet_forward: bad argument");
  cudaStream_t st = (cudaStream_t)stream;
  pqn_net_layout_t L;
  make_layout(d, &L);
  if (modular_net(d)) {
    nrm::NormWs nw;
    nrm::carve_norm(d, S, rows, (char*)workspace, &nw);
    return nrm::norm_forward(d, L, params, const_cast<float*>(batch_stats), obs, gather, obs_rows_per_seed, q, S, (int)rows,
                            0, nullptr, nw, st);
  }
  Workspace w;
  carve(d, S, rows, (char*)workspace, &w);
  const int A = d->num_actions;
  if (d->kind == PQN_NET_MINATAR_CNN) {
    const bool use_tc = g_use_tc && A <= PQN_TC_MAX_A;
    const bool f16 = use_tc && g_use_tc == 2;
    const Planes16 pl = planes16(w, S, rows);
    const bool conv16 = f16 && g_conv_mma == 1;
    launch_conv_fwd<false>(d->in_c, dim3(cdiv(rows, 4), S), st, (const uint32_t*)obs, obs_rows_per_seed, gather, params,
                           L.total, L, conv16 ? (float*)pl.h1_hi : w.h1, conv16 ? (float*)pl.h1_lo : nullptr, nullptr,
                           (int)rows, nullptr, nullptr, nullptr, conv16);
    if (f16) {
      if (!conv16) launch_split16_h1(w.h1, pl, (int64_t)S * rows * FLAT_CNN, st);
      launch_split16_w1(params, L.total, L.d0_w, pl, S, st);
      if ((rc = tc16_dense_fwd(tc::EPI_LN_HEAD, params, L.total, L, w, pl, A, q, S, (int)rows, st))) return rc;
    } else if (use_tc) {
      launch_split_w1(params, L.total, L.d0_w, w.w1_lo, S, st);
      if ((rc = tc_dense_fwd(tc::EPI_LN_HEAD, params, L.total, L, w, A, q, S, (int)rows, st))) return rc;
    } else {
      if ((rc = launch_dense<2>(128, dim3(cdiv(rows, 128), S), st, w.h1, rows * FLAT_CNN, FLAT_CNN, params, L.total, L.d0_w,
                      L.d0_b, L.ln1_scale, L.ln1_bias, L.head_w, L.head_b, A, nullptr, nullptr, nullptr, q, (int)rows,
                      FLAT_CNN))) return rc;
    }
  } else {
    const int D = d->in_c, H = d->hidden;
    const bool bits = d->kind == PQN_NET_MLP_BITS, bits_tc = bits && g_use_tc == 2;
    const float* x = (const float*)obs;
    int64_t xss = obs_rows_per_seed * D;
    if (bits && !bits_tc) {
      bits::launch_expand((const uint32_t*)obs, obs_rows_per_seed, gather, (int)rows, D, w.xg, S, st);
      x = w.xg;
      xss = rows * D;
    } else if (gather && !bits) {
      { LaunchScope _ls(K_GATHER_ROWS, st); gather_rows_kernel<<<dim3(cdiv(rows * D, 256), S), 256, 0, st>>>(x, obs_rows_per_seed, gather, w.xg,
                                                                      (int)rows, D); }
      x = w.xg;
      xss = rows * D;
    }
    const int BM = (H == 128) ? 128 : 64;
    const dim3 grid(cdiv(rows, BM), S);
    const int last = d->layers - 1;
    if (bits_tc) {
      bits::BitsWs bw;
      bits::carve_bits(d, S, rows, (char*)workspace + carve(d, S, rows, nullptr, nullptr), &bw);
      if ((rc = bits_layer0_ln(d, L, params, (const uint32_t*)obs, obs_rows_per_seed, gather, S, (int)rows, w, bw, nullptr,
                               nullptr, st))) return rc;
      if (last == 0) {
        LaunchScope _ls(K_NORM_FWD, st);
        nrm::head_fwd_kernel<<<dim3(cdiv(rows, 8), S), 256, 0, st>>>(w.h[0], (int)rows, H, params, L.total, L.head_w, L.head_b, A, q);
      }
    } else if (last == 0) {
      if ((rc = dense_ln_fwd<2>(H, grid, st, x, xss, D, params, L.total, dense_off(L, H, 0), L.head_w, L.head_b, A, w.h[0], nullptr,
                      nullptr, q, (int)rows, D))) return rc;
    } else {
      if ((rc = dense_ln_fwd<0>(H, grid, st, x, xss, D, params, L.total, dense_off(L, H, 0), 0, 0, A, w.h[0], nullptr, nullptr, nullptr,
                      (int)rows, D))) return rc;
    }
    {
      for (int l = 1; l <= last; ++l) {
        if (mlp_hidden_tc(H)) {
          if ((rc = mlp_hidden_tc_fwd(w, L, params, L.total, H, l, S, (int)rows, nullptr, nullptr,
                                      l == last ? K_TC_FWD_HEAD : K_TC_FWD, st))) return rc;
          if (l == last) {
            LaunchScope _ls(K_NORM_FWD, st);
            nrm::head_fwd_kernel<<<dim3(cdiv(rows, 8), S), 256, 0, st>>>(w.h[l], (int)rows, H, params, L.total, L.head_w, L.head_b, A, q);
          }
        } else if (l == last) {
          if ((rc = dense_ln_fwd<2>(H, grid, st, w.h[l - 1], rows * H, H, params, L.total, dense_off(L, H, l), L.head_w, L.head_b, A,
                          w.h[l], nullptr, nullptr, q, (int)rows, H))) return rc;
        } else {
          if ((rc = dense_ln_fwd<0>(H, grid, st, w.h[l - 1], rows * H, H, params, L.total, dense_off(L, H, l), 0, 0, A, w.h[l], nullptr,
                          nullptr, nullptr, (int)rows, H))) return rc;
        }
      }
    }
  }
  return check_launch("pqn_qnet_forward");
}

int pqn_qnet_loss_grad(const pqn_net_desc_t* d, const float* params, float* batch_stats, const void* obs,
                       const int32_t* gather, int64_t obs_rows_per_seed, const int32_t* action, const float* target,
                       int64_t tr_rows_per_seed, float* grads, float* loss_sum, float* qsa_sum, float* bn_sums,
                       int32_t S, int64_t rows, void* workspace, void* stream) {
  int rc = check_desc(d, "pqn_qnet_loss_grad");
  if (rc) return rc;
  if (!params || !obs || !action || !target || !grads || !loss_sum || !qsa_sum || !workspace || S <= 0 || rows <= 0 ||
      S > 65535)
    return set_error(PQN_E_INVALID, "pqn_qnet_loss_grad: bad argument");
  cudaStream_t st = (cudaStream_t)stream;
  pqn_net_layout_t L;
  make_layout(d, &L);
  const int64_t P = L.total;
  Workspace w;
  carve(d, S, rows, (char*)workspace, &w);
  const int A = d->num_actions;
// ... 148 lines not shown
```

### purejaxql_b200/csrc/pqn_tc.cu

```cuda
#include <cuda.h>
#include <cuda_runtime.h>
#include <stdint.h>

#include "../../include/pqn_b200.h"
#include "api_common.h"
#include "tc_common.cuh"

namespace pqn {
namespace tc {

constexpr int STG_LD = 36;

__device__ __forceinline__ void store_chunk_coalesced(float* stage, const float (&vals)[32], int lane, float* dst,
                                                      int64_t ld, int m_base, int M) {
#pragma unroll
  for (int j = 0; j < 8; ++j)
    *reinterpret_cast<float4*>(stage + lane * STG_LD + 4 * j) =
        make_float4(vals[4 * j], vals[4 * j + 1], vals[4 * j + 2], vals[4 * j + 3]);
  __syncwarp();
  const int r_in = lane >> 3, c4 = lane & 7;
#pragma unroll
  for (int it = 0; it < 8; ++it) {
    const int r = it * 4 + r_in;
    if (m_base + r < M)
      *reinterpret_cast<float4*>(dst + (int64_t)r * ld + 4 * c4) = *reinterpret_cast<const float4*>(stage + r * STG_LD + 4 * c4);
  }
  __syncwarp();
}

constexpr int SP_B = 0, SP_SC = 128, SP_BI = 256, SP_HW = 384 ,
              SP_HB = SP_HW + PQN_TC_MAX_A * 128, SP_FLOATS = SP_HB + PQN_TC_MAX_A;
static_assert(SP_FLOATS == TC_SP_FLOATS, "matches the TC_SMEM_BYTES budget in tc_common.cuh");

__device__ __forceinline__ void epi_bar_sync() { asm volatile("bar.sync 1, 128;" ::: "memory"); }
__device__ __forceinline__ void consumer_bar_sync() { asm volatile("bar.sync 2, 256;" ::: "memory"); }

template <int EPI>
__device__ __forceinline__ void stage_epi_params(const EpiParams& ep, float* sp, int seed, int et ) {
  const float* __restrict__ prm = ep.params + (int64_t)seed * ep.P;
  epi_bar_sync();
  sp[SP_B + et] = __ldg(prm + ep.off_b + et);
  sp[SP_SC + et] = __ldg(prm + ep.off_scale + et);
  sp[SP_BI + et] = __ldg(prm + ep.off_bias + et);
  if constexpr (EPI == EPI_LN_HEAD) {
    for (int a = 0; a < ep.A; ++a) sp[SP_HW + a * 128 + et] = __ldg(prm + ep.off_hw + (int64_t)et * ep.A + a);
    if (et < ep.A) sp[SP_HB + et] = __ldg(prm + ep.off_hb + et);
  }
  epi_bar_sync();
}

template <int EPI>
__device__ __forceinline__ void epilogue_ln_row(const EpiParams& ep, float (&acc)[128], float* stage, const float* sp,
                                                int lane, int seed, int m_base, int M) {
  const int m = m_base + lane;
  const bool row_ok = m < M;
  float s1 = 0.f, s2 = 0.f;
#pragma unroll
  for (int j4 = 0; j4 < 32; ++j4) {
    const float4 b = *reinterpret_cast<const float4*>(sp + SP_B + 4 * j4);
    const float bb[4] = {b.x, b.y, b.z, b.w};
#pragma unroll
    for (int e = 0; e < 4; ++e) {
      const int j = 4 * j4 + e;
      acc[j] += bb[e];
      s1 += acc[j];
      s2 = fmaf(acc[j], acc[j], s2);
    }
  }
  const float mean = s1 * (1.0f / 128.f);
  const float var = fmaxf(s2 * (1.0f / 128.f) - mean * mean, 0.f);
  const float rstd = 1.0f / sqrtf(var + 1e-6f);
  const int64_t grow = (int64_t)seed * ep.rows + m;
  if constexpr (EPI == EPI_LN_TRAIN) {
    float* hbase = ep.H + ((int64_t)seed * ep.rows + m_base) * 128;
    float* xbase = ep.XHAT + ((int64_t)seed * ep.rows + m_base) * 128;
#pragma unroll
    for (int c = 0; c < 4; ++c) {
      float xh[32], h[32];
#pragma unroll
      for (int j4 = 0; j4 < 8; ++j4) {
        const float4 s4 = *reinterpret_cast<const float4*>(sp + SP_SC + c * 32 + 4 * j4);
        const float4 b4 = *reinterpret_cast<const float4*>(sp + SP_BI + c * 32 + 4 * j4);
        const float ss[4] = {s4.x, s4.y, s4.z, s4.w}, bb[4] = {b4.x, b4.y, b4.z, b4.w};
#pragma unroll
        for (int e = 0; e < 4; ++e) {
          const int j = 4 * j4 + e;
          xh[j] = (acc[c * 32 + j] - mean) * rstd;
          h[j] = fmaxf(xh[j] * ss[e] + bb[e], 0.f);
        }
// ... 53 lines not shown
  const int wr = (warp & 3) * 32, wc = (warp >> 2) * 64;
  float mainacc[2][8][4], corr[2][8][4];
#pragma unroll
  for (int mi = 0; mi < 2; ++mi)
#pragma unroll
    for (int ni = 0; ni < 8; ++ni)
#pragma unroll
      for (int e = 0; e < 4; ++e) { mainacc[mi][ni][e] = 0.f; corr[mi][ni][e] = 0.f; }
  for (int kb = 0; kb < kbn; ++kb) {
    mbar_wait(&full[stage], phase);
    const uint8_t* sb = smem_al + stage * TC_STAGE_BYTES;
    if (kb % TC_PROMOTE == 0) {
#pragma unroll
      for (int mi = 0; mi < 2; ++mi)
#pragma unroll
        for (int ni = 0; ni < 8; ++ni)
#pragma unroll
          for (int e = 0; e < 4; ++e) mainacc[mi][ni][e] = 0.f;
    }
#pragma unroll
    for (int ks = 0; ks < TC_BK / 8; ++ks) {
      const int k = ks * 8 + tq;
      uint32_t ahi[2][4], alo[2][4];
#pragma unroll
      for (int mi = 0; mi < 2; ++mi) {
        const int r0 = wr + mi * 16 + g;
        const int rr[4] = {r0, r0 + 8, r0, r0 + 8}, kk[4] = {k, k, k + 4, k + 4};
#pragma unroll
        for (int e = 0; e < 4; ++e) {
          const float x = lds_tf32<A_MN>(sb + TC_A_HI, rr[e], kk[e]);
          ahi[mi][e] = tf32_trunc_bits(x);
          const float lo = split3 == 1 ? lds_tf32<A_MN>(sb + TC_A_LO, rr[e], kk[e]) : x - __uint_as_float(ahi[mi][e]);
          alo[mi][e] = tf32_trunc_bits(lo);
        }
      }
#pragma unroll
      for (int ni = 0; ni < 8; ++ni) {
        const int n = wc + ni * 8 + g;
        const uint32_t bh0 = tf32_trunc_bits(lds_tf32<B_MN>(sb + TC_B_HI, n, k));
        const uint32_t bh1 = tf32_trunc_bits(lds_tf32<B_MN>(sb + TC_B_HI, n, k + 4));
        if (split3) {
          const uint32_t bl0 = tf32_trunc_bits(lds_tf32<B_MN>(sb + TC_B_LO, n, k));
          const uint32_t bl1 = tf32_trunc_bits(lds_tf32<B_MN>(sb + TC_B_LO, n, k + 4));
#pragma unroll
          for (int mi = 0; mi < 2; ++mi) {
            mma_tf32_16x8x8(corr[mi][ni], alo[mi], bh0, bh1);
            mma_tf32_16x8x8(corr[mi][ni], ahi[mi], bl0, bl1);
          }
        }
#pragma unroll
        for (int mi = 0; mi < 2; ++mi) mma_tf32_16x8x8(mainacc[mi][ni], ahi[mi], bh0, bh1);
      }
    }
    __syncwarp();
    if (lane == 0) mbar_arrive(&empty[stage]);
    if (++stage == TC_STAGES) { stage = 0; phase ^= 1u; }
    if ((kb + 1) % TC_PROMOTE == 0 || kb == kbn - 1) {
      const bool first = kb < TC_PROMOTE;
#pragma unroll
      for (int mi = 0; mi < 2; ++mi)
#pragma unroll
        for (int ni = 0; ni < 8; ++ni)
#pragma unroll
          for (int h = 0; h < 2; ++h) {
            float2* p = reinterpret_cast<float2*>(tile_s + (wr + mi * 16 + g + 8 * h) * TC_ACC_LD + wc + ni * 8 + 2 * tq);
            const float2 v = make_float2(mainacc[mi][ni][2 * h], mainacc[mi][ni][2 * h + 1]);
            if (first) *p = v;
            else { const float2 o = *p; *p = make_float2(o.x + v.x, o.y + v.y); }
          }
    }
  }
#pragma unroll
  for (int mi = 0; mi < 2; ++mi)
#pragma unroll
    for (int ni = 0; ni < 8; ++ni)
#pragma unroll
      for (int h = 0; h < 2; ++h) {
        float2* p = reinterpret_cast<float2*>(tile_s + (wr + mi * 16 + g + 8 * h) * TC_ACC_LD + wc + ni * 8 + 2 * tq);
        float2 o = kbn > 0 ? *p : make_float2(0.f, 0.f);
        o.x += corr[mi][ni][2 * h];
        o.y += corr[mi][ni][2 * h + 1];
        *p = make_float2(o.x * osc, o.y * osc);
      }
}

template <int EPI, bool F16>
__host__ __device__ constexpr bool tma_store_epilogue() { return F16 && (EPI == EPI_RELU_MASK || EPI == EPI_RELU_BITS); }

__device__ __forceinline__ void wg_bar_sync(int wg) { asm volatile("bar.sync %0, 128;" ::"r"(3 + wg) : "memory"); }

template <int A_MN, int B_MN, int EPI, bool F16 = true>
__global__ void __launch_bounds__(TC_THREADS, 1)
    tc_gemm_kernel(const __grid_constant__ CUtensorMap tm_a_hi, const __grid_constant__ CUtensorMap tm_a_lo,
                   const __grid_constant__ CUtensorMap tm_b_hi, const __grid_constant__ CUtensorMap tm_b_lo,
                   const __grid_constant__ CUtensorMap tm_out, const GemmShape gs, const EpiParams ep) {
  constexpr bool TMA_EPI = tma_store_epilogue<EPI, F16>();
  extern __shared__ __align__(1024) uint8_t smem_raw[];
  const uint32_t smem_base = (smem_u32(smem_raw) + 1023u) & ~1023u;
  uint8_t* smem_al = smem_raw + (smem_base - smem_u32(smem_raw));
  float* tile_s = reinterpret_cast<float*>(smem_al + TC_STAGES * TC_STAGE_BYTES);
  float* sp_all = tile_s + 128 * TC_ACC_LD;
  uint64_t* full = reinterpret_cast<uint64_t*>(sp_all + TC_SP_FLOATS);
  uint64_t* empty = full + TC_STAGES;

  const int warp = threadIdx.x >> 5, lane = threadIdx.x & 31;

  if (warp == 8 && lane == 0) {
    prefetch_tmap(&tm_a_hi); prefetch_tmap(&tm_a_lo); prefetch_tmap(&tm_b_hi); prefetch_tmap(&tm_b_lo);
    if (TMA_EPI) prefetch_tmap(&tm_out);
    for (int i = 0; i < TC_STAGES; ++i) { mbar_init(&full[i], 1); mbar_init(&empty[i], TC_CONSUMERS / 32); }
    fence_barrier_init();
  }
  __syncthreads();

  const int ksplit = gs.k_split > 1 ? gs.k_split : 1;
  const int kb_per = (gs.k_blocks + ksplit - 1) / ksplit;
  const int tiles_per_seed = gs.m_tiles * gs.n_tiles * ksplit;
  const int num_tiles = tiles_per_seed * gs.S;
  auto decode = [&](int tile, int& seed, int& m0, int& n0, int& kb0, int& kbn) {
    seed = tile / tiles_per_seed;
    const int rem = tile - seed * tiles_per_seed;
    const int ks = rem % ksplit, mn = rem / ksplit;
    m0 = (mn / gs.n_tiles) * 128; n0 = (mn % gs.n_tiles) * 128;
    kb0 = ks * kb_per;
    kbn = min(kb_per, gs.k_blocks - kb0);
    if (kbn < 0) kbn = 0;
    return ks;
  };

  constexpr int BKE = F16 ? TC_BK16 : TC_BK;
  constexpr int MNB = F16 ? 2 : 4;
  constexpr int MNB_ELEMS = F16 ? 64 : 32, MNB_BYTES = F16 ? 8192 : 4096;
  const bool a_lo_tma = F16 || gs.split3 == 1, b_lo_tma = F16 || gs.split3 != 0;
  if (warp == 8) {
    if (lane == 0) {
      int stage = 0;
      uint32_t phase = 0;
      for (int tile = blockIdx.x; tile < num_tiles; tile += gridDim.x) {
        int seed, m0, n0, kb0, kbn;
        decode(tile, seed, m0, n0, kb0, kbn);
        for (int kb = kb0; kb < kb0 + kbn; ++kb) {
          mbar_wait(&empty[stage], phase ^ 1u);
          const uint32_t sb = smem_base + stage * TC_STAGE_BYTES;
          mbar_expect_tx(&full[stage], (2 + (a_lo_tma ? 1 : 0) + (b_lo_tma ? 1 : 0)) * TC_TILE_BYTES);
          const int k0 = kb * BKE;
          if (A_MN) {
#pragma unroll
            for (int j = 0; j < MNB; ++j) {
              tma_load_3d(sb + TC_A_HI + j * MNB_BYTES, &tm_a_hi, &full[stage], m0 + MNB_ELEMS * j, k0, seed);
              if (a_lo_tma) tma_load_3d(sb + TC_A_LO + j * MNB_BYTES, &tm_a_lo, &full[stage], m0 + MNB_ELEMS * j, k0, seed);
            }
          } else {
            tma_load_3d(sb + TC_A_HI, &tm_a_hi, &full[stage], k0, m0, seed);
            if (a_lo_tma) tma_load_3d(sb + TC_A_LO, &tm_a_lo, &full[stage], k0, m0, seed);
          }
          if (B_MN) {
#pragma unroll
            for (int j = 0; j < MNB; ++j) {
              tma_load_3d(sb + TC_B_HI + j * MNB_BYTES, &tm_b_hi, &full[stage], n0 + MNB_ELEMS * j, k0, seed);
              if (b_lo_tma) tma_load_3d(sb + TC_B_LO + j * MNB_BYTES, &tm_b_lo, &full[stage], n0 + MNB_ELEMS * j, k0, seed);
            }
          } else {
            tma_load_3d(sb + TC_B_HI, &tm_b_hi, &full[stage], k0, n0, seed);
            if (b_lo_tma) tma_load_3d(sb + TC_B_LO, &tm_b_lo, &full[stage], k0, n0, seed);
          }
          if (++stage == TC_STAGES) { stage = 0; phase ^= 1u; }
// ... 114 lines not shown
              x = mk.x > 0.f ? x : 0.f; y = mk.y > 0.f ? y : 0.f;
            }
          }
        }
      if (et == 0) bulk_wait_read_all();
      wg_bar_sync(wg);
      const int rl = fr - 64 * wg;
#pragma unroll
      for (int j = 0; j < 16; ++j)
#pragma unroll
        for (int h = 0; h < 2; ++h) {
          const int chunk = 2 * (j & 3) + (fc >> 2);
          const int off = (j >> 2) * TC_OUT_BOX_BYTES + (rl + 8 * h) * 128 + ((chunk ^ (lane >> 2)) << 4) + (fc & 3) * 4;
          *reinterpret_cast<float2*>(out_stage + off) = make_float2(mainacc[4 * j + 2 * h], mainacc[4 * j + 2 * h + 1]);
        }
      fence_proxy_async_smem();
      wg_bar_sync(wg);
      if (et == 0) {
#pragma unroll
        for (int b = 0; b < 4; ++b)
          tma_store_3d(&tm_out, smem_u32(out_stage + b * TC_OUT_BOX_BYTES), n0 + 32 * b, m0 + 64 * wg, seed);
        bulk_commit();
      }
      continue;
    }
    {
      const float osc = ep.out_scale != 0.f ? ep.out_scale : 1.0f;
#pragma unroll
      for (int j = 0; j < 16; ++j)
#pragma unroll
        for (int h = 0; h < 2; ++h) {
          float2* p = reinterpret_cast<float2*>(tile_s + (fr + 8 * h) * TC_ACC_LD + 8 * j + fc);
          float2 o = kbn > 0 ? *p : make_float2(0.f, 0.f);
          if (kbn > 0) {
            o.x = fmaf(corr[4 * j + 2 * h], TC_LO_INV, o.x);
            o.y = fmaf(corr[4 * j + 2 * h + 1], TC_LO_INV, o.y);
          }
          *p = make_float2(o.x * osc, o.y * osc);
        }
    }
    }
    consumer_bar_sync();

    if constexpr (EPI == EPI_LN_TRAIN || EPI == EPI_LN_HEAD) {
      if (t < 128) {
        stage_epi_params<EPI>(ep, sp_all, seed, t);
        float acc[128];
        const float* row = tile_s + t * TC_ACC_LD;
#pragma unroll
        for (int j = 0; j < 32; ++j) {
          const float4 v = *reinterpret_cast<const float4*>(row + 4 * j);
          acc[4 * j] = v.x; acc[4 * j + 1] = v.y; acc[4 * j + 2] = v.z; acc[4 * j + 3] = v.w;
        }
        __syncwarp();
        epilogue_ln_row<EPI>(ep, acc, tile_s + warp * 32 * TC_ACC_LD, sp_all, lane, seed, m0 + warp * 32, gs.M);
      }
    } else {
      const int64_t base = (int64_t)seed * ep.out_seed_stride + n0;
      float* out = ep.out + (EPI == EPI_STORE ? (int64_t)ks_idx * ep.split_stride : 0) + base;
      for (int i = t; i < 128 * 32; i += TC_CONSUMERS) {
        const int r = i >> 5, c4 = i & 31, m = m0 + r;
        if (m >= gs.M) break;
        float4 v = *reinterpret_cast<const float4*>(tile_s + r * TC_ACC_LD + 4 * c4);
        if constexpr (EPI == EPI_RELU_MASK) {
          const float4 mk = *reinterpret_cast<const float4*>(ep.mask + base + (int64_t)m * ep.ld_out + 4 * c4);
          v.x = mk.x > 0.f ? v.x : 0.f; v.y = mk.y > 0.f ? v.y : 0.f;
          v.z = mk.z > 0.f ? v.z : 0.f; v.w = mk.w > 0.f ? v.w : 0.f;
        }
        if constexpr (EPI == EPI_RELU_BITS) {
          const uint32_t wd = __ldg(ep.relu_bits + ((int64_t)seed * ep.rows + m) * (ep.ld_out >> 5) + ((n0 >> 5) + (c4 >> 3)));
          const uint32_t b = wd >> (4 * (c4 & 7));
          v.x = (b & 1u) ? v.x : 0.f; v.y = (b & 2u) ? v.y : 0.f;
          v.z = (b & 4u) ? v.z : 0.f; v.w = (b & 8u) ? v.w : 0.f;
        }
        *reinterpret_cast<float4*>(out + (int64_t)m * ep.ld_out + 4 * c4) = v;
      }
    }
  }
  if constexpr (TMA_EPI) {
    if (et == 0) bulk_wait_all();
  }
}

typedef CUresult (*EncodeTiledFn)(CUtensorMap*, CUtensorMapDataType, cuuint32_t, void*, const cuuint64_t*,
                                  const cuuint64_t*, const cuuint32_t*, const cuuint32_t*, CUtensorMapInterleave,
                                  CUtensorMapSwizzle, CUtensorMapL2promotion, CUtensorMapFloatOOBfill);

static EncodeTiledFn get_encode() {
  static EncodeTiledFn fn = nullptr;
  if (!fn) {
    void* p = nullptr;
    cudaDriverEntryPointQueryResult qres;
    if (cudaGetDriverEntryPoint("cuTensorMapEncodeTiled", &p, cudaEnableDefault, &qres) != cudaSuccess || !p) return nullptr;
    fn = reinterpret_cast<EncodeTiledFn>(p);
  }
  return fn;
}

static int num_sms() { return device_sm_count(); }

int make_tmap(CUtensorMap* tm, const float* base, uint64_t inner, uint64_t mid, uint64_t seeds, uint64_t mid_stride_elems,
              uint64_t seed_stride_elems, uint32_t box_mid) {
  EncodeTiledFn enc = get_encode();
  if (!enc) return set_error(PQN_E_CUDA, "cuTensorMapEncodeTiled entry point unavailable");
  cuuint64_t dims[3] = {inner, mid, seeds};
  cuuint64_t strides[2] = {mid_stride_elems * 4, seed_stride_elems * 4};
  cuuint32_t box[3] = {32, box_mid, 1};
  cuuint32_t estr[3] = {1, 1, 1};
  CUresult r = enc(tm, CU_TENSOR_MAP_DATA_TYPE_FLOAT32, 3, const_cast<float*>(base), dims, strides, box, estr,
                   CU_TENSOR_MAP_INTERLEAVE_NONE, CU_TENSOR_MAP_SWIZZLE_128B, CU_TENSOR_MAP_L2_PROMOTION_L2_256B,
                   CU_TENSOR_MAP_FLOAT_OOB_FILL_NONE);
  if (r != CUDA_SUCCESS) return set_error(PQN_E_CUDA, "cuTensorMapEncodeTiled failed (%d)", (int)r);
  return PQN_OK;
}

template <int A_MN, int B_MN, int EPI, bool F16>
static int launch_t(const CUtensorMap* t, const GemmShape& gs, const EpiParams& ep, cudaStream_t st, int kid) {
  auto kfn = tc_gemm_kernel<A_MN, B_MN, EPI, F16>;
  static_assert(TC_SMEM_BYTES <= 227 * 1024, "dynamic shared memory of the GEMM kernel exceeds the per-CTA limit");
  if (cudaFuncSetAttribute(kfn, cudaFuncAttributeMaxDynamicSharedMemorySize, TC_SMEM_BYTES) != cudaSuccess)
    return check_launch("tc_gemm(cudaFuncSetAttribute)");
  CUtensorMap tm_out = t[0];
  if (tma_store_epilogue<EPI, F16>()) {
    if (ep.ld_out != (int64_t)gs.n_tiles * 128 || gs.k_split > 1)
      return set_error(PQN_E_INVALID, "tc_gemm16: ReLU-mask epilogues need ld_out == N and no split-K");
    int rc = make_tmap(&tm_out, ep.out, (uint64_t)ep.ld_out, (uint64_t)gs.M, (uint64_t)gs.S, (uint64_t)ep.ld_out,
                       (uint64_t)ep.out_seed_stride, 64);
    if (rc) return rc;
  }
  const int tiles = gs.m_tiles * gs.n_tiles * gs.S * (gs.k_split > 1 ? gs.k_split : 1);
  const int grid = tiles < num_sms() ? tiles : num_sms();
  {
    LaunchScope _ls(kid < 0 ? (int)K_TC_GEMM : kid, st);
    kfn<<<grid, TC_THREADS, TC_SMEM_BYTES, st>>>(t[0], t[1], t[2], t[3], tm_out, gs, ep);
  }
  return check_launch("tc_gemm");
}

int launch_gemm(int a_mn, int b_mn, int epi, const CUtensorMap* t, const GemmShape& gs, const EpiParams& ep,
                cudaStream_t st, int kernel_id) {
#define PQN_TC_CASE(A, B, E) \
  if (a_mn == A && b_mn == B && epi == E) return launch_t<A, B, E, false>(t, gs, ep, st, kernel_id);
  PQN_TC_CASE(0, 1, EPI_STORE)
  PQN_TC_CASE(0, 1, EPI_LN_TRAIN)
  PQN_TC_CASE(0, 1, EPI_LN_HEAD)
  PQN_TC_CASE(1, 1, EPI_STORE)
  PQN_TC_CASE(0, 0, EPI_STORE)
  PQN_TC_CASE(0, 0, EPI_RELU_MASK)
  PQN_TC_CASE(0, 0, EPI_RELU_BITS)
#undef PQN_TC_CASE
  return set_error(PQN_E_UNSUPPORTED, "tc_gemm: combination a_mn=%d b_mn=%d epi=%d not instantiated", a_mn, b_mn, epi);
}

int launch_gemm16(int a_mn, int b_mn, int epi, const CUtensorMap* t, const GemmShape& gs, const EpiParams& ep,
                  cudaStream_t st, int kernel_id) {
#define PQN_TC_CASE(A, B, E) \
  if (a_mn == A && b_mn == B && epi == E) return launch_t<A, B, E, true>(t, gs, ep, st, kernel_id);
  PQN_TC_CASE(0, 1, EPI_STORE)
  PQN_TC_CASE(0, 1, EPI_LN_TRAIN)
  PQN_TC_CASE(0, 1, EPI_LN_HEAD)
  PQN_TC_CASE(1, 1, EPI_STORE)
  PQN_TC_CASE(0, 0, EPI_STORE)
  PQN_TC_CASE(0, 0, EPI_RELU_MASK)
  PQN_TC_CASE(0, 0, EPI_RELU_BITS)
#undef PQN_TC_CASE
  return set_error(PQN_E_UNSUPPORTED, "tc_gemm16: combination a_mn=%d b_mn=%d epi=%d not instantiated", a_mn, b_mn, epi);
}

int make_tmap16(CUtensorMap* tm, const void* base, uint64_t inner, uint64_t mid, uint64_t seeds, uint64_t mid_stride_elems,
                uint64_t seed_stride_elems, uint32_t box_mid) {
  EncodeTiledFn enc = get_encode();
  if (!enc) return set_error(PQN_E_CUDA, "cuTensorMapEncodeTiled entry point unavailable");
  cuuint64_t dims[3] = {inner, mid, seeds};
  cuuint64_t strides[2] = {mid_stride_elems * 2, seed_stride_elems * 2};
  cuuint32_t box[3] = {64, box_mid, 1};
  cuuint32_t estr[3] = {1, 1, 1};
  CUresult r = enc(tm, CU_TENSOR_MAP_DATA_TYPE_FLOAT16, 3, const_cast<void*>(base), dims, strides, box, estr,
                   CU_TENSOR_MAP_INTERLEAVE_NONE, CU_TENSOR_MAP_SWIZZLE_128B, CU_TENSOR_MAP_L2_PROMOTION_L2_256B,
                   CU_TENSOR_MAP_FLOAT_OOB_FILL_NONE);
  if (r != CUDA_SUCCESS) return set_error(PQN_E_CUDA, "cuTensorMapEncodeTiled(fp16) failed (%d)", (int)r);
  return PQN_OK;
}

__global__ void split_lo_kernel(const float* __restrict__ x, float* __restrict__ lo, int64_t n4) {
  const int64_t i = (int64_t)blockIdx.x * blockDim.x + threadIdx.x;
  if (i >= n4) return;
  const float4 v = __ldg(reinterpret_cast<const float4*>(x) + i);
  float4 o;
  o.x = tf32_lo(v.x); o.y = tf32_lo(v.y); o.z = tf32_lo(v.z); o.w = tf32_lo(v.w);
  reinterpret_cast<float4*>(lo)[i] = o;
}

__global__ void split16_kernel(const float* __restrict__ x, __half* __restrict__ hi, __half* __restrict__ lo, int64_t n4,
                               float scale) {
  const int64_t i = (int64_t)blockIdx.x * blockDim.x + threadIdx.x;
  if (i >= n4) return;
  const float4 v = __ldg(reinterpret_cast<const float4*>(x) + i);
  __half2 h0, h1, l0, l1;
  split16x2(v.x * scale, v.y * scale, h0, l0);
  split16x2(v.z * scale, v.w * scale, h1, l1);
  reinterpret_cast<uint2*>(hi)[i] = make_uint2(*reinterpret_cast<uint32_t*>(&h0), *reinterpret_cast<uint32_t*>(&h1));
  reinterpret_cast<uint2*>(lo)[i] = make_uint2(*reinterpret_cast<uint32_t*>(&l0), *reinterpret_cast<uint32_t*>(&l1));
}

}
}

using namespace pqn;
using namespace pqn::tc;

extern "C" {

int pqn_tc_split_lo(const float* x, float* lo, int64_t n, void* stream) {
  if (!x || !lo || n < 0 || (n & 3)) return set_error(PQN_E_INVALID, "pqn_tc_split_lo: bad argument (n %% 4 == 0)");
  if (n == 0) return PQN_OK;
  {
    LaunchScope _ls(K_TC_SPLIT, (cudaStream_t)stream);
    split_lo_kernel<<<(unsigned)((n / 4 + 255) / 256), 256, 0, (cudaStream_t)stream>>>(x, lo, n / 4);
  }
// ... 84 lines not shown
```

### purejaxql_b200/csrc/tc_common.cuh

```cuda
#pragma once
#include <cuda.h>
#include <cuda_fp16.h>
#include <stdint.h>

namespace pqn {
namespace tc {

constexpr int TC_CONSUMERS = 256;
constexpr int TC_THREADS = TC_CONSUMERS + 32;
constexpr int TC_BK16 = 64;
constexpr int TC_BK = 32;
constexpr int TC_STAGES = 2;
constexpr int TC_PROMOTE = 4;
constexpr int TC_TILE_BYTES = 128 * TC_BK16 * 2;
constexpr float TC_LO_SCALE = 2048.0f, TC_LO_INV = 1.0f / 2048.0f;
constexpr int TC_A_HI = 0, TC_A_LO = TC_TILE_BYTES, TC_B_HI = 2 * TC_TILE_BYTES, TC_B_LO = 3 * TC_TILE_BYTES;
constexpr int TC_STAGE_BYTES = 4 * TC_TILE_BYTES;
constexpr int TC_ACC_LD = 132;
constexpr int TC_SP_FLOATS = 384 + 8 * 128 + 8;
constexpr int TC_SMEM_BYTES = TC_STAGES * TC_STAGE_BYTES + 128 * TC_ACC_LD * 4 + TC_SP_FLOATS * 4 + 256  +
                              1024 ;
constexpr int TC_OUT_BOX_BYTES = 64 * 32 * 4;
constexpr int TC_OUT_STAGE_WG = 34 * 1024;
static_assert(TC_OUT_STAGE_WG >= 64 * TC_ACC_LD * 4 && TC_OUT_STAGE_WG + 4 * TC_OUT_BOX_BYTES <= 128 * TC_ACC_LD * 4,
// ... 23 lines not shown
  float *H, *XHAT, *RSTD, *Q;
};

__device__ __forceinline__ uint32_t smem_u32(const void* p) { return (uint32_t)__cvta_generic_to_shared(p); }

__device__ __forceinline__ float tf32_lo(float x) {
  const float hi = __uint_as_float(__float_as_uint(x) & 0xFFFFE000u);
  return x - hi;
}

__device__ __forceinline__ void mbar_init(uint64_t* bar, int count) {
  asm volatile("mbarrier.init.shared::cta.b64 [%0], %1;" ::"r"(smem_u32(bar)), "r"(count) : "memory");
}
__device__ __forceinline__ void fence_barrier_init() { asm volatile("fence.mbarrier_init.release.cluster;" ::: "memory"); }
__device__ __forceinline__ void mbar_expect_tx(uint64_t* bar, uint32_t bytes) {
  asm volatile("mbarrier.arrive.expect_tx.shared::cta.b64 _, [%0], %1;" ::"r"(smem_u32(bar)), "r"(bytes) : "memory");
}
__device__ __forceinline__ void mbar_arrive(uint64_t* bar) {
  asm volatile("mbarrier.arrive.shared::cta.b64 _, [%0];" ::"r"(smem_u32(bar)) : "memory");
}
__device__ __forceinline__ void mbar_wait(uint64_t* bar, uint32_t parity) {
  const uint32_t addr = smem_u32(bar);
  uint32_t ok;
  do {
    asm volatile(
        "{\n\t.reg .pred p;\n\t"
        "mbarrier.try_wait.parity.shared::cta.b64 p, [%1], %2;\n\t"
        "selp.u32 %0, 1, 0, p;\n\t}"
        : "=r"(ok)
        : "r"(addr), "r"(parity)
        : "memory");
  } while (!ok);
}

__device__ __forceinline__ void prefetch_tmap(const CUtensorMap* tm) {
  asm volatile("prefetch.tensormap [%0];" ::"l"(reinterpret_cast<uint64_t>(tm)) : "memory");
}
__device__ __forceinline__ void tma_load_3d(uint32_t smem_dst, const CUtensorMap* tm, uint64_t* bar, int c0, int c1, int c2) {
  asm volatile(
      "cp.async.bulk.tensor.3d.shared::cluster.global.mbarrier::complete_tx::bytes [%0], [%1, {%3, %4, %5}], [%2];"
      ::"r"(smem_dst), "l"(reinterpret_cast<uint64_t>(tm)), "r"(smem_u32(bar)), "r"(c0), "r"(c1), "r"(c2)
      : "memory");
}
__device__ __forceinline__ void tma_store_3d(const CUtensorMap* tm, uint32_t smem_src, int c0, int c1, int c2) {
  asm volatile("cp.async.bulk.tensor.3d.global.shared::cta.bulk_group [%0, {%2, %3, %4}], [%1];"
               ::"l"(reinterpret_cast<uint64_t>(tm)), "r"(smem_src), "r"(c0), "r"(c1), "r"(c2)
               : "memory");
}
__device__ __forceinline__ void bulk_commit() { asm volatile("cp.async.bulk.commit_group;" ::: "memory"); }
__device__ __forceinline__ void bulk_wait_read_all() { asm volatile("cp.async.bulk.wait_group.read 0;" ::: "memory"); }
__device__ __forceinline__ void bulk_wait_all() { asm volatile("cp.async.bulk.wait_group 0;" ::: "memory"); }
__device__ __forceinline__ void fence_proxy_async_smem() { asm volatile("fence.proxy.async.shared::cta;" ::: "memory"); }

__device__ __forceinline__ void wgmma_fence() { asm volatile("wgmma.fence.sync.aligned;" ::: "memory"); }
__device__ __forceinline__ void wgmma_commit() { asm volatile("wgmma.commit_group.sync.aligned;" ::: "memory"); }
template <int N>
__device__ __forceinline__ void wgmma_wait() { asm volatile("wgmma.wait_group.sync.aligned %0;" ::"n"(N) : "memory"); }
__device__ __forceinline__ void fence_operands(float (&d)[64]) {
#pragma unroll
  for (int i = 0; i < 64; ++i) asm volatile("" : "+f"(d[i])::"memory");
}

template <int TA, int TB>
__device__ __forceinline__ void wgmma_f16_m64n128(float (&d)[64], uint64_t desc_a, uint64_t desc_b, uint32_t scale_d) {
  asm volatile(
      "{\n\t.reg .pred p;\n\t"
      "setp.ne.b32 p, %66, 0;\n\t"
      "wgmma.mma_async.sync.aligned.m64n128k16.f32.f16.f16 "
      "{%0, %1, %2, %3, %4, %5, %6, %7, %8, %9, %10, %11, %12, %13, %14, %15, %16, %17, %18, %19, %20, %21, %22, %23, "
      "%24, %25, %26, %27, %28, %29, %30, %31, %32, %33, %34, %35, %36, %37, %38, %39, %40, %41, %42, %43, %44, %45, "
      "%46, %47, %48, %49, %50, %51, %52, %53, %54, %55, %56, %57, %58, %59, %60, %61, %62, %63}, "
      "%64, %65, p, 1, 1, %67, %68;\n\t}"
      : "+f"(d[0]), "+f"(d[1]), "+f"(d[2]), "+f"(d[3]), "+f"(d[4]), "+f"(d[5]), "+f"(d[6]), "+f"(d[7]), "+f"(d[8]),
        "+f"(d[9]), "+f"(d[10]), "+f"(d[11]), "+f"(d[12]), "+f"(d[13]), "+f"(d[14]), "+f"(d[15]), "+f"(d[16]),
        "+f"(d[17]), "+f"(d[18]), "+f"(d[19]), "+f"(d[20]), "+f"(d[21]), "+f"(d[22]), "+f"(d[23]), "+f"(d[24]),
        "+f"(d[25]), "+f"(d[26]), "+f"(d[27]), "+f"(d[28]), "+f"(d[29]), "+f"(d[30]), "+f"(d[31]), "+f"(d[32]),
        "+f"(d[33]), "+f"(d[34]), "+f"(d[35]), "+f"(d[36]), "+f"(d[37]), "+f"(d[38]), "+f"(d[39]), "+f"(d[40]),
        "+f"(d[41]), "+f"(d[42]), "+f"(d[43]), "+f"(d[44]), "+f"(d[45]), "+f"(d[46]), "+f"(d[47]), "+f"(d[48]),
        "+f"(d[49]), "+f"(d[50]), "+f"(d[51]), "+f"(d[52]), "+f"(d[53]), "+f"(d[54]), "+f"(d[55]), "+f"(d[56]),
        "+f"(d[57]), "+f"(d[58]), "+f"(d[59]), "+f"(d[60]), "+f"(d[61]), "+f"(d[62]), "+f"(d[63])
      : "l"(desc_a), "l"(desc_b), "r"(scale_d), "n"(TA), "n"(TB));
}

template <int MN>
__device__ __forceinline__ uint64_t make_gdesc16(uint32_t tile_addr, int ks) {
  const uint32_t addr = MN ? tile_addr + ks * 2048 : tile_addr + ks * 32;
  const uint64_t lbo = MN ? (8192u >> 4) : 1u;
  const uint64_t sbo = 1024u >> 4;
  return (uint64_t)((addr >> 4) & 0x3FFFu) | (lbo << 16) | (sbo << 32) | (1ull << 62);
}

__device__ __forceinline__ void split16(float x, __half& hi, __half& lo) {
  x = fminf(fmaxf(x, -65000.0f), 65000.0f);
  hi = __float2half_rn(x);
  lo = __float2half_rn((x - __half2float(hi)) * TC_LO_SCALE);
}
template <bool SAT = true>
__device__ __forceinline__ void split16x2(float x0, float x1, __half2& hi, __half2& lo) {
  if (SAT) {
    x0 = fminf(fmaxf(x0, -65000.0f), 65000.0f);
    x1 = fminf(fmaxf(x1, -65000.0f), 65000.0f);
  }
  hi = __floats2half2_rn(x0, x1);
  const float2 hf = __half22float2(hi);
  lo = __floats2half2_rn((x0 - hf.x) * TC_LO_SCALE, (x1 - hf.y) * TC_LO_SCALE);
}

int make_tmap(CUtensorMap* tm, const float* base, uint64_t inner, uint64_t mid, uint64_t seeds, uint64_t mid_stride_elems,
              uint64_t seed_stride_elems, uint32_t box_mid);
int launch_gemm(int a_mn, int b_mn, int epi, const CUtensorMap* t, const GemmShape& gs, const EpiParams& ep, cudaStream_t st,
                int kernel_id = -1);
int make_tmap16(CUtensorMap* tm, const void* base, uint64_t inner, uint64_t mid, uint64_t seeds, uint64_t mid_stride_elems,
                uint64_t seed_stride_elems, uint32_t box_mid);
int launch_gemm16(int a_mn, int b_mn, int epi, const CUtensorMap* t, const GemmShape& gs, const EpiParams& ep,
                  cudaStream_t st, int kernel_id = -1);

}
}
```

Measured before the change: 35.34 million.

## Fuse conv+LayerNorm into dense-layer WGMMA GEMM with register A operands

Adds a fused kernel that computes the bit-packed observation conv with mma.sync, applies LayerNorm and ReLU, splits the result into fp16 hi/lo, and feeds it straight into the dense-layer wgmma as register-sourced A fragments. This avoids writing and re-reading the conv activation tensor in global memory and drops the separate conv kernel launch. Observation tiles are prefetched with cp.async into double buffers, and weights are reloaded per seed. The cost is a more complex warp-specialised pipeline, extra register pressure and conv work repeated inside the GEMM, with a global toggle to fall back to the old path.

```diff
diff --git a/include/pqn_b200.h b/include/pqn_b200.h
--- a/include/pqn_b200.h
+++ b/include/pqn_b200.h
@@ -164,6 +164,7 @@
 
 int pqn_set_tensor_core_path(int on);
 int pqn_set_conv_mma_path(int on);
+int pqn_set_conv_fusion(int on);
 
 int pqn_tc_split_lo(const float* x, float* lo, int64_t n, void* stream);
 int pqn_tc_gemm_test(const float* a, const float* a_lo, const float* b, const float* b_lo, float* d, int32_t S,
diff --git a/purejaxql_b200/_lib.py b/purejaxql_b200/_lib.py
--- a/purejaxql_b200/_lib.py
+++ b/purejaxql_b200/_lib.py
@@ -93,6 +93,7 @@
     "pqn_bn_stats_update": (c_int, [c_void_p, c_void_p, c_int32, c_int32, c_int64, c_float, c_float, c_void_p]),
     "pqn_set_tensor_core_path": (c_int, [c_int]),
     "pqn_set_conv_mma_path": (c_int, [c_int]),
+    "pqn_set_conv_fusion": (c_int, [c_int]),
     "pqn_tc_split_lo": (c_int, [c_void_p, c_void_p, c_int64, c_void_p]),
     "pqn_tc_split16": (c_int, [c_void_p, c_void_p, c_void_p, c_int64, c_float, c_void_p]),
     "pqn_tc_gemm_test": (c_int, [c_void_p, c_void_p, c_void_p, c_void_p, c_void_p, c_int32, c_int32, c_int32,
diff --git a/purejaxql_b200/csrc/conv16.cuh b/purejaxql_b200/csrc/conv16.cuh
--- /dev/null
+++ b/purejaxql_b200/csrc/conv16.cuh
@@ -0,0 +1,231 @@
+#pragma once
+#include <cuda_fp16.h>
+#include <cuda_runtime.h>
+#include <stdint.h>
+
+#include "../../include/pqn_b200.h"
+#include "tc_common.cuh"
+
+namespace pqn {
+
+constexpr float LN_EPS = 1e-6f;
+constexpr int CONV_O = 16;
+constexpr int CONV_PIX = 64;
+constexpr int HID_CNN = 128;
+constexpr int FLAT_CNN = CONV_PIX * CONV_O;
+
+template <int C>
+struct ConvCfg {
+  static constexpr int TAPS = 9 * C;
+  static constexpr int OBS_BITS = 100 * C;
+  static constexpr int OBS_WORDS = (OBS_BITS + 31) / 32;
+  static constexpr int PW = (OBS_WORDS + 3) / 4 * 4;
+  static constexpr int SW = PW + 1;
+};
+
+template <int C>
+struct PatchCfg {
+  static constexpr int WORDS = (9 * C + 31) / 32;
+};
+
+template <int C>
+__device__ __forceinline__ void patch_bits(const uint32_t* __restrict__ so, int pix, uint32_t (&w)[PatchCfg<C>::WORDS]) {
+  constexpr int W = PatchCfg<C>::WORDS;
+#pragma unroll
+  for (int k = 0; k < W; ++k) w[k] = 0u;
+  const int y = pix >> 3, x = pix & 7;
+#pragma unroll
+  for (int di = 0; di < 3; ++di) {
+    const int f0 = ((y + di) * 10 + x) * C;
+    const uint32_t r = __funnelshift_r(so[f0 >> 5], so[(f0 >> 5) + 1], f0 & 31) & ((1u << (3 * C)) - 1u);
+    const int o = 3 * C * di;
+    w[o >> 5] |= r << (o & 31);
+    if ((o & 31) + 3 * C > 32) w[min((o >> 5) + 1, W - 1)] |= r >> (32 - (o & 31));
+  }
+}
+
+__device__ __forceinline__ void ln16_quad(const float (&z)[2][4], float& mean0, float& rstd0, float& mean1,
+                                          float& rstd1) {
+  float s0 = z[0][0] + z[0][1] + z[1][0] + z[1][1];
+  float q0 = fmaf(z[1][1], z[1][1], fmaf(z[1][0], z[1][0], fmaf(z[0][0], z[0][0], __fmul_rn(z[0][1], z[0][1]))));
+  float s1 = z[0][2] + z[0][3] + z[1][2] + z[1][3];
+  float q1 = fmaf(z[1][3], z[1][3], fmaf(z[1][2], z[1][2], fmaf(z[0][2], z[0][2], __fmul_rn(z[0][3], z[0][3]))));
+#pragma unroll
+  for (int o = 1; o <= 2; o <<= 1) {
+    s0 += __shfl_xor_sync(0xffffffffu, s0, o); q0 += __shfl_xor_sync(0xffffffffu, q0, o);
+    s1 += __shfl_xor_sync(0xffffffffu, s1, o); q1 += __shfl_xor_sync(0xffffffffu, q1, o);
+  }
+  mean0 = __fmul_rn(s0, 1.0f / CONV_O); mean1 = __fmul_rn(s1, 1.0f / CONV_O);
+  rstd0 = rsqrtf(fmaxf(fmaf(q0, 1.0f / CONV_O, -__fmul_rn(mean0, mean0)), 0.f) + LN_EPS);
+  rstd1 = rsqrtf(fmaxf(fmaf(q1, 1.0f / CONV_O, -__fmul_rn(mean1, mean1)), 0.f) + LN_EPS);
+}
+
+__device__ __forceinline__ void mma_f16_16n8k16(float (&d)[4], const uint32_t (&a)[4], uint32_t b0, uint32_t b1) {
+  asm volatile(
+      "mma.sync.aligned.m16n8k16.row.col.f32.f16.f16.f32 {%0,%1,%2,%3}, {%4,%5,%6,%7}, {%8,%9}, {%0,%1,%2,%3};"
+      : "+f"(d[0]), "+f"(d[1]), "+f"(d[2]), "+f"(d[3])
+      : "r"(a[0]), "r"(a[1]), "r"(a[2]), "r"(a[3]), "r"(b0), "r"(b1));
+}
+
+template <int C>
+struct Conv16 {
+  static constexpr int TAPS = 9 * C;
+  static constexpr int KS = (TAPS + 15) / 16;
+  static constexpr int ROW = 2 * KS < 8 ? 8 : 2 * KS;
+};
+
+__host__ __device__ constexpr int conv16_channel(int h, int n) { return 4 * (n >> 1) + 2 * h + (n & 1); }
+
+__host__ __device__ constexpr int conv16_tap(int s, int kk) {
+  return 16 * s + (kk < 8 ? 0 : 8) + ((kk & 1) ? 4 : 0) + ((kk & 7) >> 1);
+}
+
+template <int C>
+__device__ __forceinline__ void conv16_load_weights(const float* __restrict__ prm, const pqn_net_layout_t& L, uint4* wb,
+                                                    float* cb, float* sc, float* bi, int tid, int nt) {
+  using M = Conv16<C>;
+  const float inv255 = 1.0f / 255.0f;
+  for (int i = tid; i < M::KS * 2 * 32; i += nt) {
+    const int ln = i & 31, h = (i >> 5) & 1, s = i >> 6;
+    const int gg = ln >> 2, tt = ln & 3;
+    const int o = conv16_channel(h, gg);
+    const float scale = __uint_as_float((uint32_t)(127 + 15 - (1 << tt)) << 23);
+    float v[4];
+#pragma unroll
+    for (int q = 0; q < 4; ++q) {
+      const int tap = conv16_tap(s, 2 * tt + (q & 1) + (q >> 1) * 8);
+      v[q] = tap < M::TAPS ? __ldg(prm + L.conv_w + tap * CONV_O + o) * inv255 * scale : 0.f;
+      v[q] = fminf(fmaxf(v[q], -65000.f), 65000.f);
+    }
+    const __half2 h0 = __floats2half2_rn(v[0], v[1]), h1 = __floats2half2_rn(v[2], v[3]);
+    const float2 f0 = __half22float2(h0), f1 = __half22float2(h1);
+    const __half2 l0 = __floats2half2_rn(v[0] - f0.x, v[1] - f0.y), l1 = __floats2half2_rn(v[2] - f1.x, v[3] - f1.y);
+    wb[i] = make_uint4(*reinterpret_cast<const uint32_t*>(&h0), *reinterpret_cast<const uint32_t*>(&h1),
+                       *reinterpret_cast<const uint32_t*>(&l0), *reinterpret_cast<const uint32_t*>(&l1));
+  }
+  if (tid < CONV_O) {
+    cb[tid] = __ldg(prm + L.conv_b + tid);
+    sc[tid] = __ldg(prm + L.ln0_scale + tid);
+    bi[tid] = __ldg(prm + L.ln0_bias + tid);
+  }
+}
+
+template <int C>
+__device__ __forceinline__ void build_patch16(const uint32_t* __restrict__ so, int pix, uint32_t* __restrict__ out) {
+  constexpr int W = PatchCfg<C>::WORDS;
+  uint32_t w[W];
+  patch_bits<C>(so, pix, w);
+#pragma unroll
+  for (int b = 0; b < 2 * Conv16<C>::KS; ++b) {
+    const int o = 8 * b;
+    uint32_t v = (o >> 5) < W ? w[(o >> 5) < W ? (o >> 5) : 0] : 0u;
+    const int sh = o & 31;
+    const uint32_t lo = sh >= 10 ? v >> (sh - 10) : v << (10 - sh);
+    const uint32_t hi = sh + 4 <= 26 ? v << (26 - sh - 4) : v >> (sh + 4 - 26);
+    out[b] = __byte_perm(lo, hi, 0x7610);
+  }
+}
+
+template <int C>
+__device__ __forceinline__ void store_patch16(const uint32_t* __restrict__ so, int pix, uint32_t* __restrict__ row) {
+  using M = Conv16<C>;
+  uint32_t w[M::ROW];
+#pragma unroll
+  for (int k = 0; k < M::ROW; ++k) w[k] = 0u;
+  build_patch16<C>(so, pix, w);
+#pragma unroll
+  for (int q = 0; q < M::ROW / 4; ++q)
+    *reinterpret_cast<uint4*>(row + 4 * q) = make_uint4(w[4 * q], w[4 * q + 1], w[4 * q + 2], w[4 * q + 3]);
+}
+
+template <int C, int NB>
+__device__ __forceinline__ void conv16_blocks(const uint32_t* __restrict__ xp, const uint4* __restrict__ wb,
+                                              const float* __restrict__ cb, int mb0, int lane, float (&z)[NB][2][4]) {
+  using M = Conv16<C>;
+  const int g = lane >> 2, t = lane & 3;
+  const uint32_t mask = (1u << (10 + t)) | (1u << (26 + t));
+#pragma unroll
+  for (int i = 0; i < NB; ++i)
+#pragma unroll
+    for (int h = 0; h < 2; ++h) {
+      z[i][h][0] = z[i][h][2] = cb[4 * t + 2 * h];
+      z[i][h][1] = z[i][h][3] = cb[4 * t + 2 * h + 1];
+    }
+  const uint32_t* r00 = xp + (16 * mb0 + g) * M::ROW;
+#pragma unroll
+  for (int s = 0; s < M::KS; ++s) {
+    uint32_t a[NB][4];
+#pragma unroll
+    for (int i = 0; i < NB; ++i) {
+      const uint2 w0 = *reinterpret_cast<const uint2*>(r00 + (16 * i) * M::ROW + 2 * s);
+      const uint2 w1 = *reinterpret_cast<const uint2*>(r00 + (16 * i + 8) * M::ROW + 2 * s);
+      a[i][0] = w0.x & mask; a[i][1] = w1.x & mask; a[i][2] = w0.y & mask; a[i][3] = w1.y & mask;
+    }
+    uint4 b[2];
+#pragma unroll
+    for (int h = 0; h < 2; ++h) b[h] = wb[(s * 2 + h) * 32 + lane];
+#pragma unroll
+    for (int h = 0; h < 2; ++h)
+#pragma unroll
+      for (int i = 0; i < NB; ++i) mma_f16_16n8k16(z[i][h], a[i], b[h].z, b[h].w);
+#pragma unroll
+    for (int h = 0; h < 2; ++h)
+#pragma unroll
+      for (int i = 0; i < NB; ++i) mma_f16_16n8k16(z[i][h], a[i], b[h].x, b[h].y);
+  }
+}
+
+__device__ __forceinline__ void conv16_xhat(const float (&z)[2][4], float (&x0)[4], float (&x1)[4], float& rstd0,
+                                            float& rstd1) {
+  float mean0, mean1;
+  ln16_quad(z, mean0, rstd0, mean1, rstd1);
+  const float nm0 = -__fmul_rn(mean0, rstd0), nm1 = -__fmul_rn(mean1, rstd1);
+#pragma unroll
+  for (int h = 0; h < 2; ++h)
+#pragma unroll
+    for (int c = 0; c < 2; ++c) {
+      x0[2 * h + c] = fmaf(z[h][c], rstd0, nm0);
+      x1[2 * h + c] = fmaf(z[h][2 + c], rstd1, nm1);
+    }
+}
+
+__device__ __forceinline__ uint32_t cvt_f16x2_satfinite(float lo, float hi) {
+  uint32_t r;
+  asm("cvt.rn.satfinite.f16x2.f32 %0, %1, %2;" : "=r"(r) : "f"(hi), "f"(lo));
+  return r;
+}
+
+__device__ __forceinline__ void conv16_act(const float (&z)[2][4], const float (&sc4)[4], const float (&bi4)[4],
+                                           float (&v0)[4], float (&v1)[4]) {
+  float x0[4], x1[4], rstd0, rstd1;
+  conv16_xhat(z, x0, x1, rstd0, rstd1);
+#pragma unroll
+  for (int c = 0; c < 4; ++c) {
+    v0[c] = fmaxf(fmaf(x0[c], sc4[c], bi4[c]), 0.f);
+    v1[c] = fmaxf(fmaf(x1[c], sc4[c], bi4[c]), 0.f);
+  }
+}
+
+__device__ __forceinline__ void conv16_split(const float (&v)[4], uint32_t (&hw)[2], uint32_t (&lw)[2]) {
+#pragma unroll
+  for (int h = 0; h < 2; ++h) {
+    hw[h] = cvt_f16x2_satfinite(v[2 * h], v[2 * h + 1]);
+    const float2 f = __half22float2(*reinterpret_cast<const __half2*>(&hw[h]));
+    const __half2 l = __floats2half2_rn((v[2 * h] - f.x) * tc::TC_LO_SCALE, (v[2 * h + 1] - f.y) * tc::TC_LO_SCALE);
+    lw[h] = *reinterpret_cast<const uint32_t*>(&l);
+  }
+}
+
+namespace tc {
+struct ConvIn {
+  const uint32_t* obs;
+  int64_t obs_rows_per_seed;
+  const int32_t* gather;
+  pqn_net_layout_t L;
+};
+int launch_conv_gemm16(int C, int epi, const CUtensorMap* tb, const GemmShape& gs, const EpiParams& ep, const ConvIn& ci,
+                       cudaStream_t st, int kernel_id);
+}
+
+
+}
diff --git a/purejaxql_b200/csrc/pqn_net.cu b/purejaxql_b200/csrc/pqn_net.cu
--- a/purejaxql_b200/csrc/pqn_net.cu
+++ b/purejaxql_b200/csrc/pqn_net.cu
@@ -4,19 +4,16 @@
 #include "../../include/pqn_b200.h"
 #include "api_common.h"
 #include "tc_common.cuh"
+#include "conv16.cuh"
 
 namespace pqn {
 
 constexpr int GT = 256;
 constexpr int BK = 16;
-constexpr float LN_EPS = 1e-6f;
-constexpr int CONV_O = 16;
-constexpr int CONV_PIX = 64;
-constexpr int HID_CNN = 128;
-constexpr int FLAT_CNN = CONV_PIX * CONV_O;
 
 static int g_use_tc = 2;
 static int g_conv_mma = 1;
+static int g_conv_fuse = 1;
 
 __host__ __device__ static inline int64_t align4(int64_t x) { return (x + 3) & ~(int64_t)3; }
 
@@ -677,14 +674,6 @@
   else qsa_sum[seed] += v;
 }
 
-template <int C>
-struct ConvCfg {
-  static constexpr int TAPS = 9 * C;
-  static constexpr int OBS_BITS = 100 * C;
-  static constexpr int OBS_WORDS = (OBS_BITS + 31) / 32;
-  static constexpr int PW = (OBS_WORDS + 3) / 4 * 4;
-  static constexpr int SW = PW + 1;
-};
 
 template <int C>
 __device__ __forceinline__ uint32_t pixel_bits(const uint32_t* __restrict__ so, int p) {
@@ -971,26 +960,6 @@
   static constexpr int MT = (TAPS + 15) / 16;
 };
 
-template <int C>
-struct PatchCfg {
-  static constexpr int WORDS = (9 * C + 31) / 32;
-};
-
-template <int C>
-__device__ __forceinline__ void patch_bits(const uint32_t* __restrict__ so, int pix, uint32_t (&w)[PatchCfg<C>::WORDS]) {
-  constexpr int W = PatchCfg<C>::WORDS;
-#pragma unroll
-  for (int k = 0; k < W; ++k) w[k] = 0u;
-  const int y = pix >> 3, x = pix & 7;
-#pragma unroll
-  for (int di = 0; di < 3; ++di) {
-    const int f0 = ((y + di) * 10 + x) * C;
-    const uint32_t r = __funnelshift_r(so[f0 >> 5], so[(f0 >> 5) + 1], f0 & 31) & ((1u << (3 * C)) - 1u);
-    const int o = 3 * C * di;
-    w[o >> 5] |= r << (o & 31);
-    if ((o & 31) + 3 * C > 32) w[min((o >> 5) + 1, W - 1)] |= r >> (32 - (o & 31));
-  }
-}
 
 template <int C>
 __device__ __forceinline__ void build_patch(const uint32_t* __restrict__ so, int pix, uint32_t* __restrict__ out) {
@@ -1093,21 +1062,6 @@
   }
 }
 
-__device__ __forceinline__ void ln16_quad(const float (&z)[2][4], float& mean0, float& rstd0, float& mean1,
-                                          float& rstd1) {
-  float s0 = z[0][0] + z[0][1] + z[1][0] + z[1][1];
-  float q0 = fmaf(z[1][1], z[1][1], fmaf(z[1][0], z[1][0], fmaf(z[0][0], z[0][0], __fmul_rn(z[0][1], z[0][1]))));
-  float s1 = z[0][2] + z[0][3] + z[1][2] + z[1][3];
-  float q1 = fmaf(z[1][3], z[1][3], fmaf(z[1][2], z[1][2], fmaf(z[0][2], z[0][2], __fmul_rn(z[0][3], z[0][3]))));
-#pragma unroll
-  for (int o = 1; o <= 2; o <<= 1) {
-    s0 += __shfl_xor_sync(0xffffffffu, s0, o); q0 += __shfl_xor_sync(0xffffffffu, q0, o);
-    s1 += __shfl_xor_sync(0xffffffffu, s1, o); q1 += __shfl_xor_sync(0xffffffffu, q1, o);
-  }
-  mean0 = __fmul_rn(s0, 1.0f / CONV_O); mean1 = __fmul_rn(s1, 1.0f / CONV_O);
-  rstd0 = rsqrtf(fmaxf(fmaf(q0, 1.0f / CONV_O, -__fmul_rn(mean0, mean0)), 0.f) + LN_EPS);
-  rstd1 = rsqrtf(fmaxf(fmaf(q1, 1.0f / CONV_O, -__fmul_rn(mean1, mean1)), 0.f) + LN_EPS);
-}
 
 constexpr int CONV_MMA_WARPS = 8;
 
@@ -1245,140 +1199,6 @@
   }
 }
 
-__device__ __forceinline__ void mma_f16_16n8k16(float (&d)[4], const uint32_t (&a)[4], uint32_t b0, uint32_t b1) {
-  asm volatile(
-      "mma.sync.aligned.m16n8k16.row.col.f32.f16.f16.f32 {%0,%1,%2,%3}, {%4,%5,%6,%7}, {%8,%9}, {%0,%1,%2,%3};"
-      : "+f"(d[0]), "+f"(d[1]), "+f"(d[2]), "+f"(d[3])
-      : "r"(a[0]), "r"(a[1]), "r"(a[2]), "r"(a[3]), "r"(b0), "r"(b1));
-}
-
-template <int C>
-struct Conv16 {
-  static constexpr int TAPS = 9 * C;
-  static constexpr int KS = (TAPS + 15) / 16;
-  static constexpr int ROW = 2 * KS < 8 ? 8 : 2 * KS;
-};
-
-__host__ __device__ constexpr int conv16_channel(int h, int n) { return 4 * (n >> 1) + 2 * h + (n & 1); }
-
-__host__ __device__ constexpr int conv16_tap(int s, int kk) {
-  return 16 * s + (kk < 8 ? 0 : 8) + ((kk & 1) ? 4 : 0) + ((kk & 7) >> 1);
-}
-
-template <int C>
-__device__ __forceinline__ void conv16_load_weights(const float* __restrict__ prm, const pqn_net_layout_t& L, uint4* wb,
-                                                    float* cb, float* sc, float* bi) {
-  using M = Conv16<C>;
-  const float inv255 = 1.0f / 255.0f;
-  for (int i = threadIdx.x; i < M::KS * 2 * 32; i += blockDim.x) {
-    const int ln = i & 31, h = (i >> 5) & 1, s = i >> 6;
-    const int gg = ln >> 2, tt = ln & 3;
-    const int o = conv16_channel(h, gg);
-    const float scale = __uint_as_float((uint32_t)(127 + 15 - (1 << tt)) << 23);
-    float v[4];
-#pragma unroll
-    for (int q = 0; q < 4; ++q) {
-      const int tap = conv16_tap(s, 2 * tt + (q & 1) + (q >> 1) * 8);
-      v[q] = tap < M::TAPS ? __ldg(prm + L.conv_w + tap * CONV_O + o) * inv255 * scale : 0.f;
-      v[q] = fminf(fmaxf(v[q], -65000.f), 65000.f);
-    }
-    const __half2 h0 = __floats2half2_rn(v[0], v[1]), h1 = __floats2half2_rn(v[2], v[3]);
-    const float2 f0 = __half22float2(h0), f1 = __half22float2(h1);
-    const __half2 l0 = __floats2half2_rn(v[0] - f0.x, v[1] - f0.y), l1 = __floats2half2_rn(v[2] - f1.x, v[3] - f1.y);
-    wb[i] = make_uint4(*reinterpret_cast<const uint32_t*>(&h0), *reinterpret_cast<const uint32_t*>(&h1),
-                       *reinterpret_cast<const uint32_t*>(&l0), *reinterpret_cast<const uint32_t*>(&l1));
-  }
-  if (threadIdx.x < CONV_O) {
-    cb[threadIdx.x] = __ldg(prm + L.conv_b + threadIdx.x);
-    sc[threadIdx.x] = __ldg(prm + L.ln0_scale + threadIdx.x);
-    bi[threadIdx.x] = __ldg(prm + L.ln0_bias + threadIdx.x);
-  }
-}
-
-template <int C>
-__device__ __forceinline__ void build_patch16(const uint32_t* __restrict__ so, int pix, uint32_t* __restrict__ out) {
-  constexpr int W = PatchCfg<C>::WORDS;
-  uint32_t w[W];
-  patch_bits<C>(so, pix, w);
-#pragma unroll
-  for (int b = 0; b < 2 * Conv16<C>::KS; ++b) {
-    const int o = 8 * b;
-    uint32_t v = (o >> 5) < W ? w[(o >> 5) < W ? (o >> 5) : 0] : 0u;
-    const int sh = o & 31;
-    const uint32_t lo = sh >= 10 ? v >> (sh - 10) : v << (10 - sh);
-    const uint32_t hi = sh + 4 <= 26 ? v << (26 - sh - 4) : v >> (sh + 4 - 26);
-    out[b] = __byte_perm(lo, hi, 0x7610);
-  }
-}
-
-template <int C>
-__device__ __forceinline__ void store_patch16(const uint32_t* __restrict__ so, int pix, uint32_t* __restrict__ row) {
-  using M = Conv16<C>;
-  uint32_t w[M::ROW];
-#pragma unroll
-  for (int k = 0; k < M::ROW; ++k) w[k] = 0u;
-  build_patch16<C>(so, pix, w);
-#pragma unroll
-  for (int q = 0; q < M::ROW / 4; ++q)
-    *reinterpret_cast<uint4*>(row + 4 * q) = make_uint4(w[4 * q], w[4 * q + 1], w[4 * q + 2], w[4 * q + 3]);
-}
-
-template <int C, int NB>
-__device__ __forceinline__ void conv16_blocks(const uint32_t* __restrict__ xp, const uint4* __restrict__ wb,
-                                              const float* __restrict__ cb, int mb0, int lane, float (&z)[NB][2][4]) {
-  using M = Conv16<C>;
-  const int g = lane >> 2, t = lane & 3;
-  const uint32_t mask = (1u << (10 + t)) | (1u << (26 + t));
-#pragma unroll
-  for (int i = 0; i < NB; ++i)
-#pragma unroll
-    for (int h = 0; h < 2; ++h) {
-      z[i][h][0] = z[i][h][2] = cb[4 * t + 2 * h];
-      z[i][h][1] = z[i][h][3] = cb[4 * t + 2 * h + 1];
-    }
-  const uint32_t* r00 = xp + (16 * mb0 + g) * M::ROW;
-#pragma unroll
-  for (int s = 0; s < M::KS; ++s) {
-    uint32_t a[NB][4];
-#pragma unroll
-    for (int i = 0; i < NB; ++i) {
-      const uint2 w0 = *reinterpret_cast<const uint2*>(r00 + (16 * i) * M::ROW + 2 * s);
-      const uint2 w1 = *reinterpret_cast<const uint2*>(r00 + (16 * i + 8) * M::ROW + 2 * s);
-      a[i][0] = w0.x & mask; a[i][1] = w1.x & mask; a[i][2] = w0.y & mask; a[i][3] = w1.y & mask;
-    }
-    uint4 b[2];
-#pragma unroll
-    for (int h = 0; h < 2; ++h) b[h] = wb[(s * 2 + h) * 32 + lane];
-#pragma unroll
-    for (int h = 0; h < 2; ++h)
-#pragma unroll
-      for (int i = 0; i < NB; ++i) mma_f16_16n8k16(z[i][h], a[i], b[h].z, b[h].w);
-#pragma unroll
-    for (int h = 0; h < 2; ++h)
-#pragma unroll
-      for (int i = 0; i < NB; ++i) mma_f16_16n8k16(z[i][h], a[i], b[h].x, b[h].y);
-  }
-}
-
-__device__ __forceinline__ void conv16_xhat(const float (&z)[2][4], float (&x0)[4], float (&x1)[4], float& rstd0,
-                                            float& rstd1) {
-  float mean0, mean1;
-  ln16_quad(z, mean0, rstd0, mean1, rstd1);
-  const float nm0 = -__fmul_rn(mean0, rstd0), nm1 = -__fmul_rn(mean1, rstd1);
-#pragma unroll
-  for (int h = 0; h < 2; ++h)
-#pragma unroll
-    for (int c = 0; c < 2; ++c) {
-      x0[2 * h + c] = fmaf(z[h][c], rstd0, nm0);
-      x1[2 * h + c] = fmaf(z[h][2 + c], rstd1, nm1);
-    }
-}
-
-__device__ __forceinline__ uint32_t cvt_f16x2_satfinite(float lo, float hi) {
-  uint32_t r;
-  asm("cvt.rn.satfinite.f16x2.f32 %0, %1, %2;" : "=r"(r) : "f"(hi), "f"(lo));
-  return r;
-}
 
 constexpr int CONV16_WARPS = 4;
 constexpr int CONV16_CTAS_PER_SM = 5;
@@ -1398,7 +1218,7 @@
   const int tid = threadIdx.x, warp = tid >> 5, lane = tid & 31;
   const int g = lane >> 2, t = lane & 3;
   const int seed = blockIdx.y;
-  conv16_load_weights<C>(params + (int64_t)seed * P, L, wb, cb, sc, bi);
+  conv16_load_weights<C>(params + (int64_t)seed * P, L, wb, cb, sc, bi, threadIdx.x, blockDim.x);
   if (TRAIN && tid < C) s_cnt[tid] = 0.f;
   __syncthreads();
   int cnt[C];
@@ -1454,28 +1274,16 @@
 #pragma unroll
       for (int mi = 0; mi < 2; ++mi) {
         const int mb = 2 * mbp + mi;
-        float x0[4], x1[4], rstd0, rstd1;
-        conv16_xhat(z2[mi], x0, x1, rstd0, rstd1);
         uint32_t rb0 = 0u, rb1 = 0u;
         const int p0 = 16 * mb + g, p1 = p0 + 8, o4 = 4 * t;
+        const float sc4[4] = {sc[o4], sc[o4 + 1], sc[o4 + 2], sc[o4 + 3]};
+        const float bi4[4] = {bi[o4], bi[o4 + 1], bi[o4 + 2], bi[o4 + 3]};
         float v0[4], v1[4];
-#pragma unroll
-        for (int c = 0; c < 4; ++c) {
-          v0[c] = fmaxf(fmaf(x0[c], sc[o4 + c], bi[o4 + c]), 0.f);
-          v1[c] = fmaxf(fmaf(x1[c], sc[o4 + c], bi[o4 + c]), 0.f);
-        }
+        conv16_act(z2[mi], sc4, bi4, v0, v1);
         if (H16) {
           uint32_t hw0[2], hw1[2], lw0[2], lw1[2];
-#pragma unroll
-          for (int h = 0; h < 2; ++h) {
-            hw0[h] = cvt_f16x2_satfinite(v0[2 * h], v0[2 * h + 1]);
-            hw1[h] = cvt_f16x2_satfinite(v1[2 * h], v1[2 * h + 1]);
-            const float2 f0 = __half22float2(*reinterpret_cast<const __half2*>(&hw0[h]));
-            const float2 f1 = __half22float2(*reinterpret_cast<const __half2*>(&hw1[h]));
-            const __half2 l0 = __floats2half2_rn((v0[2 * h] - f0.x) * tc::TC_LO_SCALE, (v0[2 * h + 1] - f0.y) * tc::TC_LO_SCALE);
-            const __half2 l1 = __floats2half2_rn((v1[2 * h] - f1.x) * tc::TC_LO_SCALE, (v1[2 * h + 1] - f1.y) * tc::TC_LO_SCALE);
-            lw0[h] = *reinterpret_cast<const uint32_t*>(&l0); lw1[h] = *reinterpret_cast<const uint32_t*>(&l1);
-          }
+          conv16_split(v0, hw0, lw0);
+          conv16_split(v1, hw1, lw1);
           *reinterpret_cast<uint2*>(hrow16 + p0 * CONV_O + o4) = make_uint2(hw0[0], hw0[1]);
           *reinterpret_cast<uint2*>(lrow16 + p0 * CONV_O + o4) = make_uint2(lw0[0], lw0[1]);
           *reinterpret_cast<uint2*>(hrow16 + p1 * CONV_O + o4) = make_uint2(hw1[0], hw1[1]);
@@ -1806,7 +1614,7 @@
   static_assert(M::MT * 16 * CONV_O <= SM::WARP_FLOATS * SM::WARPS, "dW reduction buffer aliases the warp slices");
   static_assert(Cfg::PW <= 32, "one packed observation word per lane");
   static_assert(SM::XP % 4 == 0 && SM::WB % 4 == 0, "16-byte aligned patch rows and weight fragments");
-  conv16_load_weights<C>(params + (int64_t)seed * P, L, wb, cb, sc, bi);
+  conv16_load_weights<C>(params + (int64_t)seed * P, L, wb, cb, sc, bi, threadIdx.x, blockDim.x);
   if (tid < 3 * CONV_O) s_red[tid] = 0.f;
   __syncthreads();
   float a_dsc[4] = {0.f, 0.f, 0.f, 0.f}, a_dbi[4] = {0.f, 0.f, 0.f, 0.f}, a_dcb[4] = {0.f, 0.f, 0.f, 0.f};
@@ -2494,6 +2302,24 @@
   ep.off_hw = L.head_w; ep.off_hb = L.head_b; ep.A = A; ep.rows = rows;
   ep.H = w.h2; ep.XHAT = w.xhat2; ep.RSTD = w.rstd2; ep.Q = q;
   return tc::launch_gemm16(0, 1, epi, t, gs, ep, st, epi == tc::EPI_LN_HEAD ? K_TC_FWD_HEAD : K_TC_FWD);
+}
+
+static int tc16_conv_dense_fwd(int epi, int C, const uint32_t* obs, int64_t obs_rows_per_seed, const int32_t* gather,
+                               const float* params, int64_t P, const pqn_net_layout_t& L, const Workspace& w,
+                               const Planes16& pl, int A, float* q, int S, int rows, cudaStream_t st) {
+  CUtensorMap t[2];
+  int rc;
+  if ((rc = tc::make_tmap16(&t[0], pl.w1_hi, HID_CNN, FLAT_CNN, S, HID_CNN, (uint64_t)FLAT_CNN * HID_CNN, 64))) return rc;
+  if ((rc = tc::make_tmap16(&t[1], pl.w1_lo, HID_CNN, FLAT_CNN, S, HID_CNN, (uint64_t)FLAT_CNN * HID_CNN, 64))) return rc;
+  tc::GemmShape gs = {};
+  gs.S = S; gs.M = rows; gs.m_tiles = (rows + 127) / 128; gs.n_tiles = 1; gs.k_blocks = FLAT_CNN / tc::TC_BK16;
+  tc::EpiParams ep = {};
+  ep.params = params; ep.P = P; ep.off_b = L.d0_b; ep.off_scale = L.ln1_scale; ep.off_bias = L.ln1_bias;
+  ep.off_hw = L.head_w; ep.off_hb = L.head_b; ep.A = A; ep.rows = rows;
+  ep.H = w.h2; ep.XHAT = w.xhat2; ep.RSTD = w.rstd2; ep.Q = q;
+  tc::ConvIn ci;
+  ci.obs = obs; ci.obs_rows_per_seed = obs_rows_per_seed; ci.gather = gather; ci.L = L;
+  return tc::launch_conv_gemm16(C, epi, t, gs, ep, ci, st, epi == tc::EPI_LN_HEAD ? K_TC_FWD_HEAD : K_TC_FWD);
 }
 
 static int tc16_wgrad(float* grads, int64_t P, const pqn_net_layout_t& L, const Planes16& pl, int S, int rows,
@@ -2883,6 +2709,12 @@
   return PQN_OK;
 }
 
+int pqn_set_conv_fusion(int on) {
+  if (on != 0 && on != 1) return set_error(PQN_E_UNSUPPORTED, "pqn_set_conv_fusion: no mode %d", on);
+  g_conv_fuse = on;
+  return PQN_OK;
+}
+
 int pqn_set_tensor_core_path(int on) {
   if (on < 0 || on > 2) return set_error(PQN_E_UNSUPPORTED, "pqn_set_tensor_core_path: no tensor-core path %d", on);
   g_use_tc = on;
@@ -2943,10 +2775,16 @@
     const bool f16 = use_tc && g_use_tc == 2;
     const Planes16 pl = planes16(w, S, rows);
     const bool conv16 = f16 && g_conv_mma == 1;
-    launch_conv_fwd<false>(d->in_c, dim3(cdiv(rows, 4), S), st, (const uint32_t*)obs, obs_rows_per_seed, gather, params,
-                           L.total, L, conv16 ? (float*)pl.h1_hi : w.h1, conv16 ? (float*)pl.h1_lo : nullptr, nullptr,
-                           (int)rows, nullptr, nullptr, nullptr, conv16);
-    if (f16) {
+    const bool fused = conv16 && g_conv_fuse;
+    if (!fused)
+      launch_conv_fwd<false>(d->in_c, dim3(cdiv(rows, 4), S), st, (const uint32_t*)obs, obs_rows_per_seed, gather, params,
+                             L.total, L, conv16 ? (float*)pl.h1_hi : w.h1, conv16 ? (float*)pl.h1_lo : nullptr, nullptr,
+                             (int)rows, nullptr, nullptr, nullptr, conv16);
+    if (fused) {
+      launch_split16_w1(params, L.total, L.d0_w, pl, S, st);
+      if ((rc = tc16_conv_dense_fwd(tc::EPI_LN_HEAD, d->in_c, (const uint32_t*)obs, obs_rows_per_seed, gather, params,
+                                    L.total, L, w, pl, A, q, S, (int)rows, st))) return rc;
+    } else if (f16) {
       if (!conv16) launch_split16_h1(w.h1, pl, (int64_t)S * rows * FLAT_CNN, st);
       launch_split16_w1(params, L.total, L.d0_w, pl, S, st);
       if ((rc = tc16_dense_fwd(tc::EPI_LN_HEAD, params, L.total, L, w, pl, A, q, S, (int)rows, st))) return rc;
diff --git a/purejaxql_b200/csrc/pqn_tc.cu b/purejaxql_b200/csrc/pqn_tc.cu
--- a/purejaxql_b200/csrc/pqn_tc.cu
+++ b/purejaxql_b200/csrc/pqn_tc.cu
@@ -5,6 +5,7 @@
 #include "../../include/pqn_b200.h"
 #include "api_common.h"
 #include "tc_common.cuh"
+#include "conv16.cuh"
 
 namespace pqn {
 namespace tc {
@@ -224,6 +225,48 @@
         o.y += corr[mi][ni][2 * h + 1];
         *p = make_float2(o.x * osc, o.y * osc);
       }
+}
+
+__device__ __forceinline__ void promote_main(float* tile_s, const float (&mainacc)[64], int fr, int fc, bool first) {
+#pragma unroll
+  for (int j = 0; j < 16; ++j)
+#pragma unroll
+    for (int h = 0; h < 2; ++h) {
+      float2* p = reinterpret_cast<float2*>(tile_s + (fr + 8 * h) * TC_ACC_LD + 8 * j + fc);
+      const float2 v = make_float2(mainacc[4 * j + 2 * h], mainacc[4 * j + 2 * h + 1]);
+      if (first) *p = v;
+      else { const float2 o = *p; *p = make_float2(o.x + v.x, o.y + v.y); }
+    }
+}
+
+__device__ __forceinline__ void finish_corr(float* tile_s, const float (&corr)[64], int fr, int fc, int kbn, float osc) {
+#pragma unroll
+  for (int j = 0; j < 16; ++j)
+#pragma unroll
+    for (int h = 0; h < 2; ++h) {
+      float2* p = reinterpret_cast<float2*>(tile_s + (fr + 8 * h) * TC_ACC_LD + 8 * j + fc);
+      float2 o = kbn > 0 ? *p : make_float2(0.f, 0.f);
+      if (kbn > 0) {
+        o.x = fmaf(corr[4 * j + 2 * h], TC_LO_INV, o.x);
+        o.y = fmaf(corr[4 * j + 2 * h + 1], TC_LO_INV, o.y);
+      }
+      *p = make_float2(o.x * osc, o.y * osc);
+    }
+}
+
+template <int EPI>
+__device__ __forceinline__ void ln_epilogue_tile(const EpiParams& ep, float* tile_s, float* sp_all, int t, int warp,
+                                                 int lane, int seed, int m0, int M) {
+  stage_epi_params<EPI>(ep, sp_all, seed, t);
+  float acc[128];
+  const float* row = tile_s + t * TC_ACC_LD;
+#pragma unroll
+  for (int j = 0; j < 32; ++j) {
+    const float4 v = *reinterpret_cast<const float4*>(row + 4 * j);
+    acc[4 * j] = v.x; acc[4 * j + 1] = v.y; acc[4 * j + 2] = v.z; acc[4 * j + 3] = v.w;
+  }
+  __syncwarp();
+  epilogue_ln_row<EPI>(ep, acc, tile_s + warp * 32 * TC_ACC_LD, sp_all, lane, seed, m0 + warp * 32, M);
 }
 
 template <int EPI, bool F16>
@@ -504,6 +547,220 @@
   }
 }
 
+constexpr int CV_STAGE_BYTES = 2 * TC_TILE_BYTES;
+constexpr int CV_B_HI = 0, CV_B_LO = TC_TILE_BYTES;
+constexpr int CV_WARPS = TC_CONSUMERS / 32;
+constexpr int CV_THREADS = TC_CONSUMERS + 128;
+constexpr int CV_PRODUCER_REGS = 40, CV_CONSUMER_REGS = 232;
+constexpr int CV_KB = FLAT_CNN / TC_BK16;
+
+template <int C>
+struct ConvGemm {
+  static constexpr int PW = ConvCfg<C>::PW;
+  static constexpr int OLD = PW + 4;
+  static constexpr int PB_PIX = 16 * Conv16<C>::ROW;
+  static constexpr int TILE = TC_STAGES * CV_STAGE_BYTES;
+  static constexpr int SP = TILE + 128 * TC_ACC_LD * 4;
+  static constexpr int WB = SP + TC_SP_FLOATS * 4;
+  static constexpr int CB = WB + Conv16<C>::KS * 2 * 32 * 16;
+  static constexpr int OBS = CB + 3 * CONV_O * 4;
+  static constexpr int PB = OBS + 2 * CV_WARPS * 16 * OLD * 4;
+  static constexpr int BAR = PB + CV_WARPS * 4 * PB_PIX * 4;
+  static constexpr int SMEM = BAR + 2 * TC_STAGES * 8 + 1024 ;
+  static_assert(WB % 16 == 0 && OBS % 16 == 0 && PB % 16 == 0 && BAR % 8 == 0, "aligned regions");
+  static_assert(SMEM <= 227 * 1024, "dynamic shared memory of the conv-fused GEMM exceeds the per-CTA limit");
+};
+
+__device__ __forceinline__ void cp_async16(uint32_t smem_dst, const void* gsrc) {
+  asm volatile("cp.async.cg.shared.global [%0], [%1], 16;" ::"r"(smem_dst), "l"(gsrc) : "memory");
+}
+__device__ __forceinline__ void cp_async_commit() { asm volatile("cp.async.commit_group;" ::: "memory"); }
+__device__ __forceinline__ void cp_async_wait_all() { asm volatile("cp.async.wait_group 0;" ::: "memory"); }
+__device__ __forceinline__ void fence_frag(uint32_t (&a)[4]) {
+#pragma unroll
+  for (int i = 0; i < 4; ++i) asm volatile("" : "+r"(a[i])::"memory");
+}
+
+__device__ __forceinline__ void quad_pairs(const uint32_t (&x)[2], int lane, uint32_t& lo, uint32_t& hi) {
+  const int t = lane & 3, base = lane & ~3;
+  const uint32_t sa = (t >> 1) ? x[1] : x[0], sb = (t >> 1) ? x[0] : x[1];
+  const uint32_t ra = __shfl_sync(0xffffffffu, sa, base | ((t & 1) << 1) | (t >> 1));
+  const uint32_t rb = __shfl_sync(0xffffffffu, sb, base | (((t & 1) ^ 1) << 1) | (t >> 1));
+  lo = (t & 1) ? rb : ra;
+  hi = (t & 1) ? ra : rb;
+}
+
+template <int C, int EPI>
+__global__ void __launch_bounds__(CV_THREADS, 1)
+    tc_conv_gemm_kernel(const __grid_constant__ CUtensorMap tm_b_hi, const __grid_constant__ CUtensorMap tm_b_lo,
+                        const GemmShape gs, const EpiParams ep, const ConvIn ci) {
+  using G = ConvGemm<C>;
+  using M = Conv16<C>;
+  extern __shared__ __align__(1024) uint8_t smem_raw[];
+  const uint32_t smem_base = (smem_u32(smem_raw) + 1023u) & ~1023u;
+  uint8_t* smem_al = smem_raw + (smem_base - smem_u32(smem_raw));
+  float* tile_s = reinterpret_cast<float*>(smem_al + G::TILE);
+  float* sp_all = reinterpret_cast<float*>(smem_al + G::SP);
+  uint4* wb = reinterpret_cast<uint4*>(smem_al + G::WB);
+  float* cb = reinterpret_cast<float*>(smem_al + G::CB);
+  float* sc = cb + CONV_O;
+  float* bi = sc + CONV_O;
+  uint32_t* obs_s = reinterpret_cast<uint32_t*>(smem_al + G::OBS);
+  uint32_t* pb_s = reinterpret_cast<uint32_t*>(smem_al + G::PB);
+  uint64_t* full = reinterpret_cast<uint64_t*>(smem_al + G::BAR);
+  uint64_t* empty = full + TC_STAGES;
+
+  const int warp = threadIdx.x >> 5, lane = threadIdx.x & 31;
+  if (warp == 8 && lane == 0) {
+    prefetch_tmap(&tm_b_hi); prefetch_tmap(&tm_b_lo);
+    for (int i = 0; i < TC_STAGES; ++i) { mbar_init(&full[i], 1); mbar_init(&empty[i], TC_CONSUMERS / 32); }
+    fence_barrier_init();
+  }
+  __syncthreads();
+  const int tiles_per_seed = gs.m_tiles;
+  const int num_tiles = tiles_per_seed * gs.S;
+
+  if (warp >= 8) {
+    asm volatile("setmaxnreg.dec.sync.aligned.u32 %0;" ::"n"(CV_PRODUCER_REGS));
+    if (warp == 8 && lane == 0) {
+      int stage = 0;
+      uint32_t phase = 0;
+      for (int tile = blockIdx.x; tile < num_tiles; tile += gridDim.x) {
+        const int seed = tile / tiles_per_seed;
+        for (int kb = 0; kb < CV_KB; ++kb) {
+          mbar_wait(&empty[stage], phase ^ 1u);
+          const uint32_t sb = smem_base + stage * CV_STAGE_BYTES;
+          mbar_expect_tx(&full[stage], 2 * TC_TILE_BYTES);
+#pragma unroll
+          for (int j = 0; j < 2; ++j) {
+            tma_load_3d(sb + CV_B_HI + j * 8192, &tm_b_hi, &full[stage], 64 * j, kb * TC_BK16, seed);
+            tma_load_3d(sb + CV_B_LO + j * 8192, &tm_b_lo, &full[stage], 64 * j, kb * TC_BK16, seed);
+          }
+          if (++stage == TC_STAGES) { stage = 0; phase ^= 1u; }
+        }
+      }
+    }
+    return;
+  }
+
+  asm volatile("setmaxnreg.inc.sync.aligned.u32 %0;" ::"n"(CV_CONSUMER_REGS));
+  const int t = threadIdx.x;
+  const int g = lane >> 2, tq = lane & 3;
+  const int fr = 16 * warp + g, fc = 2 * tq;
+  uint32_t* my_pb = pb_s + warp * 4 * G::PB_PIX;
+  for (int i = t; i < 2 * CV_WARPS * 16; i += TC_CONSUMERS)
+    for (int w = G::PW; w < G::OLD; ++w) obs_s[i * G::OLD + w] = 0u;
+  auto obs_src = [&](int tile) -> const uint32_t* {
+    const int seed = tile / tiles_per_seed;
+    int m = (tile - seed * tiles_per_seed) * 128 + 16 * warp + (lane & 15);
+    m = m < gs.M ? m : gs.M - 1;
+    const int64_t src = ci.gather ? __ldg(ci.gather + (int64_t)seed * gs.M + m) : m;
+    return ci.obs + ((int64_t)seed * ci.obs_rows_per_seed + src) * G::PW;
+  };
+  auto obs_copy = [&](const uint32_t* src, int buf) {
+    const uint32_t dst = smem_u32(obs_s + ((buf * CV_WARPS + warp) * 16 + (lane & 15)) * G::OLD);
+    for (int j = lane >> 4; j < G::PW / 4; j += 2) cp_async16(dst + 16 * j, src + 4 * j);
+    cp_async_commit();
+  };
+  if ((int)blockIdx.x < num_tiles) obs_copy(obs_src(blockIdx.x), 0);
+
+  int cur_seed = -1, buf = 0;
+  int stage = 0;
+  uint32_t phase = 0;
+  for (int tile = blockIdx.x; tile < num_tiles; tile += gridDim.x) {
+    const int seed = tile / tiles_per_seed, m0 = (tile - seed * tiles_per_seed) * 128;
+    const int next = tile + gridDim.x;
+    const uint32_t* next_src = next < num_tiles ? obs_src(next) : nullptr;
+    consumer_bar_sync();
+    if (seed != cur_seed) {
+      conv16_load_weights<C>(ep.params + (int64_t)seed * ep.P, ci.L, wb, cb, sc, bi, t, TC_CONSUMERS);
+      consumer_bar_sync();
+      cur_seed = seed;
+    }
+    cp_async_wait_all();
+    __syncwarp();
+    const uint32_t* my_obs = obs_s + (buf * CV_WARPS + warp) * 16 * G::OLD;
+
+    auto build_pair = [&](int kb, int half, uint32_t (&ah)[2][4], uint32_t (&al)[2][4]) {
+      if (half == 0) {
+        __syncwarp();
+        store_patch16<C>(my_obs + g * G::OLD, 4 * kb + tq, my_pb + tq * G::PB_PIX + g * M::ROW);
+        store_patch16<C>(my_obs + (g + 8) * G::OLD, 4 * kb + tq, my_pb + tq * G::PB_PIX + (g + 8) * M::ROW);
+        __syncwarp();
+      }
+      float z2[2][2][4];
+      conv16_blocks<C, 2>(my_pb, wb, cb, 2 * half, lane, z2);
+      const float4 s4 = *reinterpret_cast<const float4*>(sc + 4 * tq), b4 = *reinterpret_cast<const float4*>(bi + 4 * tq);
+      const float sc4[4] = {s4.x, s4.y, s4.z, s4.w}, bi4[4] = {b4.x, b4.y, b4.z, b4.w};
+#pragma unroll
+      for (int i = 0; i < 2; ++i) {
+        float v0[4], v1[4];
+        conv16_act(z2[i], sc4, bi4, v0, v1);
+        uint32_t hw0[2], lw0[2], hw1[2], lw1[2];
+        conv16_split(v0, hw0, lw0);
+        conv16_split(v1, hw1, lw1);
+        quad_pairs(hw0, lane, ah[i][0], ah[i][2]);
+        quad_pairs(hw1, lane, ah[i][1], ah[i][3]);
+        quad_pairs(lw0, lane, al[i][0], al[i][2]);
+        quad_pairs(lw1, lane, al[i][1], al[i][3]);
+      }
+    };
+
+    float mainacc[64], corr[64];
+#pragma unroll
+    for (int i = 0; i < 64; ++i) { mainacc[i] = 0.f; corr[i] = 0.f; }
+    uint32_t ahi[2][2][4], alo[2][2][4];
+    build_pair(0, 0, ahi[0], alo[0]);
+    int prev_stage = 0;
+    for (int kb = 0; kb < CV_KB; ++kb) {
+      mbar_wait(&full[stage], phase);
+      const uint32_t sb = smem_base + stage * CV_STAGE_BYTES;
+#pragma unroll
+      for (int half = 0; half < 2; ++half) {
+        const int nxt = half ^ 1;
+        wgmma_fence();
+#pragma unroll
+        for (int i = 0; i < 2; ++i) {
+          const int ks = 2 * half + i;
+          const uint64_t b_hi = make_gdesc16<1>(sb + CV_B_HI, ks), b_lo = make_gdesc16<1>(sb + CV_B_LO, ks);
+          wgmma_f16_m64n128_ra<1>(corr, alo[half][i], b_hi, (ks == 0 && kb == 0) ? 0u : 1u);
+          wgmma_f16_m64n128_ra<1>(corr, ahi[half][i], b_lo, 1u);
+          wgmma_f16_m64n128_ra<1>(mainacc, ahi[half][i], b_hi, (ks == 0 && kb % TC_PROMOTE == 0) ? 0u : 1u);
+        }
+        wgmma_commit();
+        wgmma_wait<1>();
+#pragma unroll
+        for (int i = 0; i < 2; ++i) { fence_frag(ahi[nxt][i]); fence_frag(alo[nxt][i]); }
+        if (half == 0 && kb > 0) {
+          __syncwarp();
+          if (lane == 0) mbar_arrive(&empty[prev_stage]);
+        }
+        if (half == 0 && kb == 0 && next_src) obs_copy(next_src, buf ^ 1);
+        if (half == 0) build_pair(kb, 1, ahi[1], alo[1]);
+        else if (kb + 1 < CV_KB) build_pair(kb + 1, 0, ahi[0], alo[0]);
+      }
+      prev_stage = stage;
+      if (++stage == TC_STAGES) { stage = 0; phase ^= 1u; }
+      if ((kb + 1) % TC_PROMOTE == 0) {
+        wgmma_wait<0>();
+        fence_operands(mainacc); fence_operands(corr);
+#pragma unroll
+        for (int i = 0; i < 2; ++i) { fence_frag(ahi[0][i]); fence_frag(alo[0][i]); }
+        promote_main(tile_s, mainacc, fr, fc, kb < TC_PROMOTE);
+      }
+    }
+#pragma unroll
+    for (int i = 0; i < 2; ++i) { fence_frag(ahi[1][i]); fence_frag(alo[1][i]); }
+    __syncwarp();
+    if (lane == 0) mbar_arrive(&empty[prev_stage]);
+    finish_corr(tile_s, corr, fr, fc, CV_KB, ep.out_scale != 0.f ? ep.out_scale : 1.0f);
+    consumer_bar_sync();
+    if (t < 128) ln_epilogue_tile<EPI>(ep, tile_s, sp_all, t, warp, lane, seed, m0, gs.M);
+    buf ^= 1;
+  }
+  cp_async_wait_all();
+}
+
 typedef CUresult (*EncodeTiledFn)(CUtensorMap*, CUtensorMapDataType, cuuint32_t, void*, const cuuint64_t*,
                                   const cuuint64_t*, const cuuint32_t*, const cuuint32_t*, CUtensorMapInterleave,
                                   CUtensorMapSwizzle, CUtensorMapL2promotion, CUtensorMapFloatOOBfill);
@@ -557,6 +814,36 @@
     kfn<<<grid, TC_THREADS, TC_SMEM_BYTES, st>>>(t[0], t[1], t[2], t[3], tm_out, gs, ep);
   }
   return check_launch("tc_gemm");
+}
+
+template <int C, int EPI>
+static int launch_conv_t(const CUtensorMap* tb, const GemmShape& gs, const EpiParams& ep, const ConvIn& ci,
+                         cudaStream_t st, int kid) {
+  auto kfn = tc_conv_gemm_kernel<C, EPI>;
+  constexpr int smem = ConvGemm<C>::SMEM;
+  if (cudaFuncSetAttribute(kfn, cudaFuncAttributeMaxDynamicSharedMemorySize, smem) != cudaSuccess)
+    return check_launch("tc_conv_gemm(cudaFuncSetAttribute)");
+  const int tiles = gs.m_tiles * gs.S;
+  const int grid = tiles < num_sms() ? tiles : num_sms();
+  {
+    LaunchScope _ls(kid, st);
+    kfn<<<grid, CV_THREADS, smem, st>>>(tb[0], tb[1], gs, ep, ci);
+  }
+  return check_launch("tc_conv_gemm");
+}
+
+int launch_conv_gemm16(int C, int epi, const CUtensorMap* tb, const GemmShape& gs, const EpiParams& ep, const ConvIn& ci,
+                       cudaStream_t st, int kernel_id) {
+  if (gs.n_tiles != 1 || gs.k_split > 1 || gs.k_blocks != CV_KB)
+    return set_error(PQN_E_INVALID, "tc_conv_gemm16: N = 128, K = 1024 and no split-K");
+#define PQN_CONV_CASE(CC) \
+  if (C == CC && epi == EPI_LN_HEAD) return launch_conv_t<CC, EPI_LN_HEAD>(tb, gs, ep, ci, st, kernel_id);
+  PQN_CONV_CASE(4)
+  PQN_CONV_CASE(6)
+  PQN_CONV_CASE(7)
+  PQN_CONV_CASE(10)
+#undef PQN_CONV_CASE
+  return set_error(PQN_E_UNSUPPORTED, "tc_conv_gemm16: combination C=%d epi=%d not instantiated", C, epi);
 }
 
 int launch_gemm(int a_mn, int b_mn, int epi, const CUtensorMap* t, const GemmShape& gs, const EpiParams& ep,
diff --git a/purejaxql_b200/csrc/tc_common.cuh b/purejaxql_b200/csrc/tc_common.cuh
--- a/purejaxql_b200/csrc/tc_common.cuh
+++ b/purejaxql_b200/csrc/tc_common.cuh
@@ -129,6 +129,28 @@
       : "l"(desc_a), "l"(desc_b), "r"(scale_d), "n"(TA), "n"(TB));
 }
 
+template <int TB>
+__device__ __forceinline__ void wgmma_f16_m64n128_ra(float (&d)[64], const uint32_t (&a)[4], uint64_t desc_b,
+                                                     uint32_t scale_d) {
+  asm volatile(
+      "{\n\t.reg .pred p;\n\t"
+      "setp.ne.b32 p, %69, 0;\n\t"
+      "wgmma.mma_async.sync.aligned.m64n128k16.f32.f16.f16 "
+      "{%0, %1, %2, %3, %4, %5, %6, %7, %8, %9, %10, %11, %12, %13, %14, %15, %16, %17, %18, %19, %20, %21, %22, %23, "
+      "%24, %25, %26, %27, %28, %29, %30, %31, %32, %33, %34, %35, %36, %37, %38, %39, %40, %41, %42, %43, %44, %45, "
+      "%46, %47, %48, %49, %50, %51, %52, %53, %54, %55, %56, %57, %58, %59, %60, %61, %62, %63}, "
+      "{%64, %65, %66, %67}, %68, p, 1, 1, %70;\n\t}"
+      : "+f"(d[0]), "+f"(d[1]), "+f"(d[2]), "+f"(d[3]), "+f"(d[4]), "+f"(d[5]), "+f"(d[6]), "+f"(d[7]), "+f"(d[8]),
+        "+f"(d[9]), "+f"(d[10]), "+f"(d[11]), "+f"(d[12]), "+f"(d[13]), "+f"(d[14]), "+f"(d[15]), "+f"(d[16]),
+        "+f"(d[17]), "+f"(d[18]), "+f"(d[19]), "+f"(d[20]), "+f"(d[21]), "+f"(d[22]), "+f"(d[23]), "+f"(d[24]),
+        "+f"(d[25]), "+f"(d[26]), "+f"(d[27]), "+f"(d[28]), "+f"(d[29]), "+f"(d[30]), "+f"(d[31]), "+f"(d[32]),
+        "+f"(d[33]), "+f"(d[34]), "+f"(d[35]), "+f"(d[36]), "+f"(d[37]), "+f"(d[38]), "+f"(d[39]), "+f"(d[40]),
+        "+f"(d[41]), "+f"(d[42]), "+f"(d[43]), "+f"(d[44]), "+f"(d[45]), "+f"(d[46]), "+f"(d[47]), "+f"(d[48]),
+        "+f"(d[49]), "+f"(d[50]), "+f"(d[51]), "+f"(d[52]), "+f"(d[53]), "+f"(d[54]), "+f"(d[55]), "+f"(d[56]),
+        "+f"(d[57]), "+f"(d[58]), "+f"(d[59]), "+f"(d[60]), "+f"(d[61]), "+f"(d[62]), "+f"(d[63])
+      : "r"(a[0]), "r"(a[1]), "r"(a[2]), "r"(a[3]), "l"(desc_b), "r"(scale_d), "n"(TB));
+}
+
 template <int MN>
 __device__ __forceinline__ uint64_t make_gdesc16(uint32_t tile_addr, int ks) {
   const uint32_t addr = MN ? tile_addr + ks * 2048 : tile_addr + ks * 32;
```

Measured after the change: 36.46 million (median of 6 runs). +3.2%, better.
